# zhouxian/act3d-chained-diffuser

Hardware: AMD Instinct MI355X
Metric: train samples/sec (Act3D keypose fwd+bwd+AdamW step) (higher is better)
Workload: dtype fp16 / bf16 MFMA on two-part operands (x = hi + lo; fp32 accumulate) in attention; fp32-accurate linears (f32 MFMA; bf16x3 MFMA from 4096 rows); bf16 frozen backbone + FPN; 1 GPU; Act3D keypose training step, 18-PerAct-task shapes: 4 cameras 256x256, 3 ghost-point levels, 1000 ghost points (333/level), E=60, frozen synthetic CLIP-RN50-shaped backbone + trainable FPN included in the step; per_gpu_batch_keyframes=64, global_batch=64, parallelism=dp1, hipgraph=True, backbone_prefetch=True

## Files before the change

### act3d-chained-diffuser_amd/csrc/a3d_common.h

```cpp
#pragma once
#include <hip/hip_runtime.h>
#include <stdint.h>
#include <math.h>

#define A3D_OK 0
#define A3D_ERR_ARG (-22)
#define A3D_ERR_LAUNCH (-5)
#define A3D_ERR_NOMEM (-12)

namespace a3d {

void set_error(const char* fmt, ...);
int check_launch(const char* what);
int zero_words(void* p, size_t bytes, hipStream_t s, const char* what);

typedef __attribute__((ext_vector_type(4))) float f32x4;
typedef __attribute__((ext_vector_type(8))) short s16x8;
typedef __attribute__((ext_vector_type(8))) __bf16 bf16x8;
typedef __attribute__((ext_vector_type(4))) short s16x4;

constexpr int HD = 15;
constexpr float LOG2E_F = 1.4426950408889634f;
constexpr int HDP = 16;

__device__ __forceinline__ unsigned short f2bf(float x) {
  unsigned int u = __float_as_uint(x);
  unsigned int r = u + 0x7FFFu + ((u >> 16) & 1u);
  return (unsigned short)(r >> 16);
}
__device__ __forceinline__ unsigned int pk_bf16(float a, float b) {
  typedef __bf16 bf16x2_t __attribute__((ext_vector_type(2)));
  typedef float f32x2_t __attribute__((ext_vector_type(2)));
  return __builtin_bit_cast(unsigned int, __builtin_convertvector(f32x2_t{a, b}, bf16x2_t));
}
__device__ __forceinline__ float bf2f(unsigned short h) {
  return __uint_as_float(((unsigned int)h) << 16);
}
__device__ __forceinline__ void split_bf16(float x, unsigned short& hi, unsigned short& lo) {
  hi = f2bf(x);
  lo = f2bf(x - bf2f(hi));
}

__device__ __forceinline__ void split_bf16_3(float x, unsigned short& hi, unsigned short& lo, unsigned short& lo2) {
  hi = f2bf(x);
  const float r1 = x - bf2f(hi);
  lo = f2bf(r1);
  lo2 = f2bf(r1 - bf2f(lo));
}
constexpr int QKW = 48;
constexpr int VRW = 32;
__device__ __forceinline__ int tile_off(int row, int seg) { return row * 32 + ((seg ^ ((0 - (row >> 3)) & 3)) << 3); }
__device__ __forceinline__ int plane_off(int row, int seg) { return row * 32 + ((seg ^ ((0 - (row >> 2)) & 3)) << 3); }

__device__ __forceinline__ float colmax4(float v) {
  typedef unsigned int u32x2_t __attribute__((ext_vector_type(2)));
  u32x2_t r = __builtin_amdgcn_permlane16_swap(__float_as_uint(v), __float_as_uint(v), false, false);
  v = fmaxf(__uint_as_float(r[0]), __uint_as_float(r[1]));
  r = __builtin_amdgcn_permlane32_swap(__float_as_uint(v), __float_as_uint(v), false, false);
  return fmaxf(__uint_as_float(r[0]), __uint_as_float(r[1]));
}

__device__ __forceinline__ double colsum4(double v) {
  typedef unsigned int u32x2_t __attribute__((ext_vector_type(2)));
  unsigned int lo = (unsigned int)(__double_as_longlong(v) & 0xFFFFFFFFll), hi = (unsigned int)(__double_as_longlong(v) >> 32);
  u32x2_t a = __builtin_amdgcn_permlane16_swap(lo, lo, false, false);
  u32x2_t b = __builtin_amdgcn_permlane16_swap(hi, hi, false, false);
  v = __longlong_as_double(((long long)b[0] << 32) | a[0]) + __longlong_as_double(((long long)b[1] << 32) | a[1]);
  lo = (unsigned int)(__double_as_longlong(v) & 0xFFFFFFFFll);
  hi = (unsigned int)(__double_as_longlong(v) >> 32);
  a = __builtin_amdgcn_permlane32_swap(lo, lo, false, false);
  b = __builtin_amdgcn_permlane32_swap(hi, hi, false, false);
  return __longlong_as_double(((long long)b[0] << 32) | a[0]) + __longlong_as_double(((long long)b[1] << 32) | a[1]);
}

__device__ __forceinline__ f32x4 mfma_bf16_16x16x32(s16x8 a, s16x8 b, f32x4 c) {
  return __builtin_amdgcn_mfma_f32_16x16x32_bf16(__builtin_bit_cast(bf16x8, a),
                                                 __builtin_bit_cast(bf16x8, b), c, 0, 0, 0);
}
__device__ __forceinline__ f32x4 mfma_f32_16x16x4(float a, float b, f32x4 c) {
  return __builtin_amdgcn_mfma_f32_16x16x4f32(a, b, c, 0, 0, 0);
}

__device__ __forceinline__ float wave_sum(float v) {
#pragma unroll
  for (int o = 32; o > 0; o >>= 1) v += __shfl_xor(v, o, 64);
  return v;
}
__device__ __forceinline__ float wave_max(float v) {
#pragma unroll
  for (int o = 32; o > 0; o >>= 1) v = fmaxf(v, __shfl_xor(v, o, 64));
  return v;
}

__device__ __forceinline__ float rope_freq(int k, int E) {
  return expf((float)(2 * k) * (-9.210340371976184f / (float)(E / 3)));
}

__host__ __device__ __forceinline__ void sincos_poly(float x, float* sn, float* cs) {
  const float kf = rintf(x * 0.636619772367581343f);
  float r = fmaf(-kf, 1.57079637050628662109375f, x);
  r = fmaf(-kf, -4.37113900018624283e-8f, r);
  const float z = r * r;
  const float ps = fmaf(fmaf(fmaf(-1.9515295891e-4f, z, 8.3321608736e-3f), z, -1.6666654611e-1f) * z, r, r);
  const float pc = fmaf(fmaf(fmaf(2.443315711809948e-5f, z, -1.388731625493765e-3f), z, 4.166664568298827e-2f), z * z,
                        fmaf(-0.5f, z, 1.0f));
  const int q = (int)kf;
  const float s0 = (q & 1) ? pc : ps, c0 = (q & 1) ? ps : pc;
  *sn = (q & 2) ? -s0 : s0;
  *cs = ((q + 1) & 2) ? -c0 : c0;
}
__host__ __device__ __forceinline__ void fast_sincos(float x, float* sn, float* cs) {
#if defined(A3D_LIBM_SINCOS) && defined(__HIP_DEVICE_COMPILE__)
  sincosf(x, sn, cs);
#else
  if (fabsf(x) >= 200.0f) {
    const double t = (double)x;
    const double k = rint(t * 0.15915494309189535);
    x = (float)fma(-k, 2.4492935982947064e-16, fma(-k, 6.283185307179586, t));
  }
  sincos_poly(x, sn, cs);
#endif
}

__device__ __forceinline__ float add_rn(float a, float b) {
#pragma clang fp contract(off)
  return a + b;
}
__device__ __forceinline__ float sub_rn(float a, float b) {
#pragma clang fp contract(off)
  return a - b;
}
__device__ __forceinline__ float mul_rn(float a, float b) {
#pragma clang fp contract(off)
  return a * b;
}
__device__ __forceinline__ float sqrt_rn(float a) { return __builtin_sqrtf(a); }

__host__ __device__ __forceinline__ void philox4x32_10(uint32_t c0, uint32_t c1, uint32_t c2, uint32_t c3,
                                                       uint32_t k0, uint32_t k1, uint32_t out[4]) {
  for (int r = 0; r < 10; ++r) {
    const uint64_t p0 = (uint64_t)0xD2511F53u * c0;
    const uint64_t p1 = (uint64_t)0xCD9E8D57u * c2;
    const uint32_t n0 = (uint32_t)(p1 >> 32) ^ c1 ^ k0;
    const uint32_t n1 = (uint32_t)p1;
    const uint32_t n2 = (uint32_t)(p0 >> 32) ^ c3 ^ k1;
    const uint32_t n3 = (uint32_t)p0;
    c0 = n0; c1 = n1; c2 = n2; c3 = n3;
    k0 += 0x9E3779B9u; k1 += 0xBB67AE85u;
  }
  out[0] = c0; out[1] = c1; out[2] = c2; out[3] = c3;
}

struct DropKey { uint32_t k0, k1; };
__device__ __forceinline__ DropKey drop_key(const unsigned long long* state) {
  const unsigned long long seed = state[0], offs = state[1];
  const unsigned long long key = seed + offs * 0x9E3779B97F4A7C15ull;
  DropKey k;
  k.k0 = (uint32_t)key;
  k.k1 = (uint32_t)(key >> 32);
  return k;
}
__device__ __forceinline__ uint32_t drop_keep8(DropKey k, uint32_t c0, uint32_t c1, uint32_t c2, uint32_t site,
                                               uint32_t thr16) {
  uint32_t r[4];
  philox4x32_10(c0, c1, c2, site, k.k0, k.k1, r);
  uint32_t bits = 0;
#pragma unroll
  for (int w = 0; w < 4; ++w) {
    bits |= ((r[w] & 0xFFFFu) >= thr16 ? 1u : 0u) << (2 * w);
    bits |= ((r[w] >> 16) >= thr16 ? 1u : 0u) << (2 * w + 1);
  }
  return bits;
}

__device__ __forceinline__ bool xcd_decode(int per_group, int ngroups, int& group, int& within) {
  const int id = blockIdx.x;
  const int xcd = id & 7, slot = id >> 3;
  group = (slot / per_group) * 8 + xcd;
  within = slot % per_group;
  return group < ngroups;
}
static inline int xcd_grid(int ngroups, int per_group) { return ((ngroups + 7) / 8) * 8 * per_group; }

static inline int cdiv(int a, int b) { return (a + b - 1) / b; }

bool conv1x1_deep_serves(int K, int N);
int conv1x1_deep_slabs(size_t M, int K, int N);
int conv1x1_deep_launch(const void* x, const void* w, const float* in_scale, const float* in_shift, int in_relu, void* y, float* partial,
                        size_t M, int K, int N, hipStream_t s);

}
```

### act3d-chained-diffuser_amd/csrc/conv1x1.hip

```cpp
#include "a3d_common.h"
#include "../../include/act3d_hip.h"

namespace a3d {

constexpr int C1_BK = 32;

__device__ __forceinline__ int c1_woff(int row, int seg) { return row * 32 + ((seg ^ (((row >> 1) & 1) | (((row >> 4) & 1) << 1))) << 3); }

struct C1Epilogue { const float* bias; int nbias; const unsigned short* top; int H, W; };
template <int WN, int KS, bool EP = false>
__global__ __launch_bounds__(256, 2) void conv1x1_stream_kernel(const unsigned short* __restrict__ x, const unsigned short* __restrict__ w,
                                                             const float* __restrict__ in_scale, const float* __restrict__ in_shift,
                                                             int in_relu, unsigned short* __restrict__ y, float* __restrict__ partial,
                                                             long long M, int N, C1Epilogue ep) {
  constexpr int WM = 4 / WN, BM = 64 * WM, BN = 64 * WN, K = KS * 32;
  constexpr int XL = BM * 4 / 256;
  constexpr int D = 8 / XL;
  extern __shared__ __attribute__((aligned(16))) unsigned short smem_c1[];
  unsigned short* Ws = smem_c1;
  unsigned short* Xs = Ws + KS * BN * 32;
  float* scS = reinterpret_cast<float*>(Xs + 2 * BM * 32);
  __shared__ float redS[4][64], redQ[4][64];
  const int t = threadIdx.x, lane = t & 63, wave = t >> 6;
  const int li = lane & 15, g = lane >> 4;
  const int wm = wave / WN, wn = wave % WN;
  const int n0 = blockIdx.y * BN;
  const long long mtiles = (M + BM - 1) / BM;
  for (int i = t; i < KS * BN * 4; i += 256) {
    const int ks = i / (BN * 4), rem = i - ks * (BN * 4), row = rem >> 2, seg = rem & 3;
    *reinterpret_cast<uint4*>(&Ws[ks * BN * 32 + c1_woff(row, seg)]) =
        *reinterpret_cast<const uint4*>(w + (size_t)(n0 + row) * K + ks * C1_BK + seg * 8);
  }
  if (in_scale)
    for (int i = t; i < K; i += 256) { scS[i] = in_scale[i]; scS[K + i] = in_shift[i]; }
  float ssum[4][4], ssq[4][4];
#pragma unroll
  for (int a = 0; a < 4; ++a)
#pragma unroll
    for (int r = 0; r < 4; ++r) { ssum[a][r] = 0.f; ssq[a][r] = 0.f; }
  float epb[16];
  if (EP) {
#pragma unroll
    for (int j = 0; j < 16; ++j) {
      const int c = n0 + wn * 64 + g * 16 + j;
      epb[j] = (ep.bias && c < ep.nbias) ? ep.bias[c] : 0.f;
    }
  }
  const long long my_tiles = blockIdx.x < mtiles ? (mtiles - blockIdx.x + gridDim.x - 1) / gridDim.x : 0;
  const long long total = my_tiles * KS;
  auto load = [&](long long s, uint4 (&r)[XL]) {
    const long long m0 = (blockIdx.x + (s / KS) * gridDim.x) * BM;
    const int ks = (int)(s % KS);
#pragma unroll
    for (int i = 0; i < XL; ++i) {
      const int idx = t + i * 256, row = idx >> 2, seg = idx & 3;
      const long long m = m0 + row < M ? m0 + row : M - 1;
      r[i] = *reinterpret_cast<const uint4*>(x + (size_t)m * K + ks * C1_BK + seg * 8);
    }
  };
  const float relu_lo = in_relu ? 0.f : -INFINITY;
  auto stage = [&](int buf, int ks, const uint4 (&r)[XL]) {
#pragma unroll
    for (int i = 0; i < XL; ++i) {
      const int idx = t + i * 256, row = idx >> 2, seg = idx & 3;
      uint4 v = r[i];
      if (in_scale) {
        const int k0 = ks * C1_BK + seg * 8;
        unsigned int u[4] = {v.x, v.y, v.z, v.w};
#pragma unroll
        for (int j = 0; j < 4; ++j) {
          float a = __uint_as_float(u[j] << 16) * scS[k0 + 2 * j] + scS[K + k0 + 2 * j];
          float b = __uint_as_float(u[j] & 0xFFFF0000u) * scS[k0 + 2 * j + 1] + scS[K + k0 + 2 * j + 1];
          a = fmaxf(a, relu_lo);
          b = fmaxf(b, relu_lo);
          u[j] = pk_bf16(a, b);
        }
        v = make_uint4(u[0], u[1], u[2], u[3]);
      }
      *reinterpret_cast<uint4*>(&Xs[buf * BM * 32 + plane_off(row, seg)]) = v;
    }
  };
  if (total > 0) {
    uint4 xr[D][XL];
#pragma unroll
    for (int j = 0; j < D; ++j) load(j < total ? j : total - 1, xr[j]);
    f32x4 acc[4][4];
#pragma unroll
    for (int a = 0; a < 4; ++a)
#pragma unroll
      for (int b = 0; b < 4; ++b) acc[a][b] = f32x4{0.f, 0.f, 0.f, 0.f};
    __syncthreads();
    for (long long s0 = 0; s0 < total; s0 += D) {
#pragma unroll
      for (int j = 0; j < D; ++j) {
        const long long s = s0 + j;
        if (s >= total) break;
        const int ks = (int)(s % KS), buf = (int)(s & 1);
        stage(buf, ks, xr[j]);
        load(s + D < total ? s + D : total - 1, xr[j]);
        __syncthreads();
        s16x8 xa[4], wb[4];
#pragma unroll
        for (int tm = 0; tm < 4; ++tm)
          xa[tm] = *reinterpret_cast<const s16x8*>(&Xs[buf * BM * 32 + plane_off(wm * 64 + tm * 16 + li, g)]);
#pragma unroll
        for (int tn = 0; tn < 4; ++tn)
          wb[tn] = *reinterpret_cast<const s16x8*>(&Ws[ks * BN * 32 + c1_woff(wn * 64 + (li >> 2) * 16 + tn * 4 + (li & 3), g)]);
        uint4 tv[4][2];
        if (EP && ks == KS - 1 && ep.top) {
          const long long m0 = (blockIdx.x + (s / KS) * gridDim.x) * BM;
#pragma unroll
          for (int tm = 0; tm < 4; ++tm) {
            const long long m = m0 + wm * 64 + tm * 16 + li;
            const unsigned int mm = (unsigned int)(m < M ? m : M - 1);
            const unsigned int hq = mm / (unsigned int)ep.W, w_ = mm - hq * (unsigned int)ep.W;
            const unsigned int n_ = hq / (unsigned int)ep.H, h_ = hq - n_ * (unsigned int)ep.H;
            const size_t tr = ((size_t)n_ * (ep.H >> 1) + (h_ >> 1)) * (ep.W >> 1) + (w_ >> 1);
            const uint4* src = reinterpret_cast<const uint4*>(ep.top + tr * N + n0 + wn * 64 + g * 16);
            tv[tm][0] = src[0];
            tv[tm][1] = src[1];
          }
        }
#pragma unroll
        for (int tn = 0; tn < 4; ++tn)
#pragma unroll
          for (int tm = 0; tm < 4; ++tm) acc[tn][tm] = mfma_bf16_16x16x32(wb[tn], xa[tm], acc[tn][tm]);
        if (ks == KS - 1) {
          const long long m0 = (blockIdx.x + (s / KS) * gridDim.x) * BM;
#pragma unroll
          for (int tm = 0; tm < 4; ++tm) {
            const long long m = m0 + wm * 64 + tm * 16 + li;
            const bool ok = m < M;
            unsigned int pk[8];
#pragma unroll
            for (int tn = 0; tn < 4; ++tn) {
#pragma unroll
              for (int r2 = 0; r2 < 2; ++r2) {
                float a0 = acc[tn][tm][2 * r2], a1 = acc[tn][tm][2 * r2 + 1];
                if (EP) {
                  a0 += epb[4 * tn + 2 * r2];
                  a1 += epb[4 * tn + 2 * r2 + 1];
                  if (ep.top) {
                    const uint4 q = tv[tm][tn >> 1];
                    const unsigned int tw = (tn & 1) ? (r2 ? q.w : q.z) : (r2 ? q.y : q.x);
                    a0 += __uint_as_float(tw << 16);
                    a1 += __uint_as_float(tw & 0xFFFF0000u);
                  }
                }
                const unsigned int u = pk_bf16(a0, a1);
                if (!EP && ok) {
                  const float v0 = __uint_as_float(u << 16), v1 = __uint_as_float(u & 0xFFFF0000u);
                  ssum[tn][2 * r2] += v0;
                  ssq[tn][2 * r2] += v0 * v0;
                  ssum[tn][2 * r2 + 1] += v1;
                  ssq[tn][2 * r2 + 1] += v1 * v1;
                }
                pk[2 * tn + r2] = u;
              }
              acc[tn][tm] = f32x4{0.f, 0.f, 0.f, 0.f};
            }
            if (ok) {
              uint4* dst = reinterpret_cast<uint4*>(y + (size_t)m * N + n0 + wn * 64 + g * 16);
              dst[0] = make_uint4(pk[0], pk[1], pk[2], pk[3]);
              dst[1] = make_uint4(pk[4], pk[5], pk[6], pk[7]);
            }
          }
        }
      }
    }
  }
  if (EP || !partial) return;
#pragma unroll
  for (int tn = 0; tn < 4; ++tn)
#pragma unroll
    for (int r = 0; r < 4; ++r) {
      float sv = ssum[tn][r], q = ssq[tn][r];
#pragma unroll
      for (int o = 1; o < 16; o <<= 1) { sv += __shfl_xor(sv, o, 64); q += __shfl_xor(q, o, 64); }
      if (li == 0) { redS[wave][g * 16 + tn * 4 + r] = sv; redQ[wave][g * 16 + tn * 4 + r] = q; }
    }
  __syncthreads();
  for (int i = t; i < BN; i += 256) {
    const int wn_i = i >> 6, c = i & 63;
    float sv = 0.f, q = 0.f;
#pragma unroll
    for (int j = 0; j < WM; ++j) { sv += redS[j * WN + wn_i][c]; q += redQ[j * WN + wn_i][c]; }
    float* p = partial + (size_t)blockIdx.x * 2 * N;
    p[n0 + i] = sv;
    p[N + n0 + i] = q;
  }
}

}

using namespace a3d;

static int c1_wn(int N) { return N >= 256 ? 4 : (N >= 128 ? 2 : 1); }
static size_t c1_stream_lds(int K, int N) {
  const int wn = c1_wn(N), bn = 64 * wn, bm = 64 * (4 / wn);
  return (size_t)(K / 32) * bn * 64 + (size_t)2 * bm * 64 + (size_t)2 * K * sizeof(float);
}
static bool c1_streams(int K, int N) {
  return (K == 64 || K == 128 || K == 256) && (N % 64) == 0 && (N < 256 || (N % 256) == 0) && c1_stream_lds(K, N) <= 96 * 1024;
}
static int c1_slabs(size_t M, int K, int N) {
  const int wn = c1_wn(N);
  const int bm = 64 * (4 / wn);
  const size_t mtiles = (M + bm - 1) / bm;
  const int ntiles = N / (64 * wn);
  const size_t lds = c1_stream_lds(K, N) + 2048;
  const int per_cu = (int)std::max<size_t>(1, std::min<size_t>(2, (160 * 1024) / lds));
  return (int)std::min<size_t>(mtiles, (size_t)std::max(1, 256 * per_cu / ntiles));
}

static int c1_deep_mode = getenv("A3D_CONV1X1_DEEP") ? atoi(getenv("A3D_CONV1X1_DEEP")) : 1;
extern "C" int a3d_conv1x1_deep_mode(int mode) {
  const int prev = c1_deep_mode;
  if (mode >= 0) c1_deep_mode = mode > 0 ? 1 : 0;
  return prev;
}
static bool c1_deep(int K, int N) { return c1_deep_mode != 0 && !c1_streams(K, N) && conv1x1_deep_serves(K, N); }

extern "C" int a3d_conv1x1_streams(int K, int N) { return (K > 0 && N > 0 && (c1_streams(K, N) || c1_deep(K, N))) ? 1 : 0; }

extern "C" int a3d_conv1x1_nslab(size_t M, int K, int N) {
  if (M == 0 || N <= 0 || K <= 0) return 0;
  if (c1_streams(K, N)) return c1_slabs(M, K, N);
  return c1_deep(K, N) ? conv1x1_deep_slabs(M, K, N) : 0;
}

extern "C" int a3d_conv1x1_bn_fwd(const void* x, const void* w, const float* in_scale, const float* in_shift, int in_relu,
                                  void* y, float* partial, size_t M, int K, int N, void* stream) {
  if (!x || !w || !y || M == 0 || K <= 0 || N <= 0 || !(c1_streams(K, N) || c1_deep(K, N)) || (in_scale && !in_shift) ||
      ((((uintptr_t)x | (uintptr_t)w | (uintptr_t)y) & 15) != 0)) {
    set_error("a3d_conv1x1_bn_fwd: bad argument (M=%zu K=%d N=%d; served shapes: K in {64, 128, 256}, N in {64, 128, 256 j}, weight block "
              "+ buffers within 96 KB of LDS (the resident-weight kernel), or K = 64 j in 128 .. 2048 and N = 128 j up to 2048 (the deep-layer "
              "GEMM) -- a3d_conv1x1_streams; 16-byte aligned operands)", M, K, N);
    return A3D_ERR_ARG;
  }
  hipStream_t s = (hipStream_t)stream;
  if (!c1_streams(K, N)) return conv1x1_deep_launch(x, w, in_scale, in_shift, in_relu, y, partial, M, K, N, s);
  const unsigned short* xs = (const unsigned short*)x;
  const unsigned short* ws = (const unsigned short*)w;
  unsigned short* ys = (unsigned short*)y;
  const int slabs = c1_slabs(M, K, N);
  const size_t lds = c1_stream_lds(K, N);
  const dim3 grid(slabs, N >= 256 ? N / 256 : 1);
#define A3D_C1S(WNV, KSV)                                                                                                         \
  do {                                                                                                                           \
    static bool once = false;                                                                                                    \
    if (!once) { (void)hipFuncSetAttribute((const void*)conv1x1_stream_kernel<WNV, KSV>, hipFuncAttributeMaxDynamicSharedMemorySize, 96 * 1024); once = true; } \
    hipLaunchKernelGGL((conv1x1_stream_kernel<WNV, KSV>), grid, dim3(256), lds, s, xs, ws, in_scale, in_shift, in_relu, ys, partial, (long long)M, N, C1Epilogue{nullptr, 0, nullptr, 0, 0}); \
  } while (0)
  const int wn = c1_wn(N), ks = K / 32;
  if (wn == 4 && ks == 2) A3D_C1S(4, 2);
  else if (wn == 4 && ks == 4) A3D_C1S(4, 4);
  else if (wn == 2 && ks == 2) A3D_C1S(2, 2);
  else if (wn == 2 && ks == 4) A3D_C1S(2, 4);
  else if (wn == 2 && ks == 8) A3D_C1S(2, 8);
  else if (wn == 1 && ks == 2) A3D_C1S(1, 2);
  else if (wn == 1 && ks == 4) A3D_C1S(1, 4);
  else if (wn == 1 && ks == 8) A3D_C1S(1, 8);
  else { set_error("a3d_conv1x1_bn_fwd: no streaming instance for K=%d N=%d", K, N); return A3D_ERR_ARG; }
#undef A3D_C1S
  return check_launch("a3d_conv1x1_bn_fwd");
}

extern "C" int a3d_conv1x1_topdown_serves(int K, int N) { return (c1_streams(K, N) && N <= 128) ? 1 : 0; }

extern "C" int a3d_conv1x1_topdown_fwd(const void* x, const void* w, const float* bias, int nbias, const void* top, void* y,
                                       size_t images, int H, int W, int K, int N, void* stream) {
  const size_t M = images * (size_t)H * (size_t)W;
  if (!x || !w || !y || images == 0 || H <= 0 || W <= 0 || K <= 0 || N <= 0 || !a3d_conv1x1_topdown_serves(K, N) || M > 0xFFFFFFFFull ||
      (top && ((H & 1) || (W & 1))) || (bias && (nbias <= 0 || nbias > N)) ||
      ((((uintptr_t)x | (uintptr_t)w | (uintptr_t)y | (uintptr_t)top) & 15) != 0)) {
    set_error("a3d_conv1x1_topdown_fwd: bad argument (images=%zu H=%d W=%d K=%d N=%d nbias=%d; served: K in {64, 128, 256}, N in {64, 128}, "
              "H and W even with a top map, at most 2^32 rows, 0 < nbias <= N with a bias, 16-byte aligned operands)", images, H, W, K, N, nbias);
    return A3D_ERR_ARG;
  }
  hipStream_t s = (hipStream_t)stream;
  const int slabs = c1_slabs(M, K, N);
  const size_t lds = c1_stream_lds(K, N);
  const dim3 grid(slabs, 1);
  const C1Epilogue ep{bias, bias ? nbias : 0, (const unsigned short*)top, H, W};
#define A3D_C1E(WNV, KSV)                                                                                                         \
  do {                                                                                                                           \
    static bool once = false;                                                                                                    \
    if (!once) { (void)hipFuncSetAttribute((const void*)conv1x1_stream_kernel<WNV, KSV, true>, hipFuncAttributeMaxDynamicSharedMemorySize, 96 * 1024); once = true; } \
    hipLaunchKernelGGL((conv1x1_stream_kernel<WNV, KSV, true>), grid, dim3(256), lds, s, (const unsigned short*)x, (const unsigned short*)w, \
                       (const float*)nullptr, (const float*)nullptr, 0, (unsigned short*)y, (float*)nullptr, (long long)M, N, ep);  \
  } while (0)
  const int wn = c1_wn(N), ks = K / 32;
  if (wn == 2 && ks == 2) A3D_C1E(2, 2);
  else if (wn == 2 && ks == 4) A3D_C1E(2, 4);
  else if (wn == 2 && ks == 8) A3D_C1E(2, 8);
  else if (wn == 1 && ks == 2) A3D_C1E(1, 2);
  else if (wn == 1 && ks == 4) A3D_C1E(1, 4);
  else if (wn == 1 && ks == 8) A3D_C1E(1, 8);
  else { set_error("a3d_conv1x1_topdown_fwd: no streaming instance for K=%d N=%d", K, N); return A3D_ERR_ARG; }
#undef A3D_C1E
  return check_launch("a3d_conv1x1_topdown_fwd");
}
```

### act3d-chained-diffuser_amd/csrc/conv1x1_deep.hip

```cpp
#include "a3d_common.h"
#include "../../include/act3d_hip.h"

namespace a3d {

constexpr int CD_BM = 128, CD_BN = 128, CD_BK = 64;

__device__ __forceinline__ int cd_xoff(int row, int seg) { return row * 64 + ((seg ^ ((row >> 1) & 7)) << 3); }
__device__ __forceinline__ int cd_woff(int row, int seg) { return row * 64 + ((seg ^ ((((row >> 4) & 3) << 1) | ((row >> 1) & 1))) << 3); }

__device__ __forceinline__ unsigned int cd_norm2(unsigned int u, const float* scS, int K, int k, float relu_lo) {
  float a = __uint_as_float(u << 16) * scS[k] + scS[K + k];
  float b = __uint_as_float(u & 0xFFFF0000u) * scS[k + 1] + scS[K + k + 1];
  return pk_bf16(fmaxf(a, relu_lo), fmaxf(b, relu_lo));
}

__device__ __forceinline__ void cd_compute(const unsigned short* Xb, const unsigned short* Wb, const int (&xo)[2][4], const int (&wo)[2][4],
                                           f32x4 (&acc)[4][4]) {
#pragma unroll
  for (int h = 0; h < 2; ++h) {
    s16x8 xa[4], wb[4];
#pragma unroll
    for (int i = 0; i < 4; ++i) {
      xa[i] = *reinterpret_cast<const s16x8*>(&Xb[xo[h][i]]);
      wb[i] = *reinterpret_cast<const s16x8*>(&Wb[wo[h][i]]);
    }
#pragma unroll
    for (int tn = 0; tn < 4; ++tn)
#pragma unroll
      for (int tm = 0; tm < 4; ++tm) acc[tn][tm] = mfma_bf16_16x16x32(wb[tn], xa[tm], acc[tn][tm]);
  }
}

__device__ __forceinline__ void cd_epilogue(f32x4 (&acc)[4][4], float (&ssum)[4][4], float (&ssq)[4][4], unsigned short* __restrict__ y,
                                            long long m0, long long M, int N, int n0, int wm, int wn, int li, int g) {
#pragma unroll
  for (int tm = 0; tm < 4; ++tm) {
    const long long m = m0 + wm * 64 + tm * 16 + li;
    const bool ok = m < M;
    unsigned int pk[8];
#pragma unroll
    for (int tn = 0; tn < 4; ++tn) {
#pragma unroll
      for (int r2 = 0; r2 < 2; ++r2) {
        const unsigned int u = pk_bf16(acc[tn][tm][2 * r2], acc[tn][tm][2 * r2 + 1]);
        const float v0 = ok ? __uint_as_float(u << 16) : 0.f, v1 = ok ? __uint_as_float(u & 0xFFFF0000u) : 0.f;
        ssum[tn][2 * r2] += v0;
        ssq[tn][2 * r2] += v0 * v0;
        ssum[tn][2 * r2 + 1] += v1;
        ssq[tn][2 * r2 + 1] += v1 * v1;
        pk[2 * tn + r2] = u;
      }
      acc[tn][tm] = f32x4{0.f, 0.f, 0.f, 0.f};
    }
    if (ok) {
      uint4* dst = reinterpret_cast<uint4*>(y + (size_t)m * N + n0 + wn * 64 + g * 16);
      dst[0] = make_uint4(pk[0], pk[1], pk[2], pk[3]);
      dst[1] = make_uint4(pk[4], pk[5], pk[6], pk[7]);
    }
  }
}

template <bool XFORM>
__global__ __launch_bounds__(256, 2) void conv1x1_deep_kernel(const unsigned short* __restrict__ x, const unsigned short* __restrict__ w,
                                                            const float* __restrict__ in_scale, const float* __restrict__ in_shift,
                                                            int in_relu, unsigned short* __restrict__ y, float* __restrict__ partial,
                                                            long long M, int N, int K) {
  extern __shared__ __attribute__((aligned(16))) unsigned short smem_cd[];
  unsigned short* Xs = smem_cd;
  unsigned short* Ws = Xs + 2 * CD_BM * CD_BK;
  float* scS = reinterpret_cast<float*>(Ws + 2 * CD_BN * CD_BK);
  const int t = threadIdx.x, lane = t & 63, wave = t >> 6;
  const int li = lane & 15, g = lane >> 4;
  const int wm = wave >> 1, wn = wave & 1;
  const int n0 = blockIdx.y * CD_BN;
  const int KS = K / CD_BK;
  const long long mtiles = (M + CD_BM - 1) / CD_BM;
  if (XFORM)
    for (int i = t; i < K; i += 256) { scS[i] = in_scale[i]; scS[K + i] = in_shift[i]; }
  float ssum[4][4], ssq[4][4];
#pragma unroll
  for (int a = 0; a < 4; ++a)
#pragma unroll
    for (int r = 0; r < 4; ++r) { ssum[a][r] = 0.f; ssq[a][r] = 0.f; }
  const long long my_tiles = blockIdx.x < mtiles ? (mtiles - blockIdx.x + gridDim.x - 1) / gridDim.x : 0;
  const long long total = my_tiles * KS;
  const int srow = t >> 3, sseg = t & 7;
  long long l_m0 = (long long)blockIdx.x * CD_BM;
  int l_ks = 0;
  const float relu_lo = in_relu ? 0.f : -INFINITY;
#define CD_LOAD1(P, i)                                                                                                \
  {                                                                                                                   \
    const long long m_ = l_m0 + srow + 32 * i < M ? l_m0 + srow + 32 * i : M - 1;    \
    P##x##i = *reinterpret_cast<const uint4*>(x + (size_t)m_ * K + l_ks * CD_BK + sseg * 8);                          \
    P##w##i = *reinterpret_cast<const uint4*>(w + (size_t)(n0 + srow + 32 * i) * K + l_ks * CD_BK + sseg * 8);        \
  }
#define CD_LOAD(P)                                                                                                    \
  do {                                                                                                                \
    CD_LOAD1(P, 0) CD_LOAD1(P, 1) CD_LOAD1(P, 2) CD_LOAD1(P, 3)                                                       \
    if (l_left > 1) { --l_left; if (++l_ks == KS) { l_ks = 0; l_m0 += (long long)gridDim.x * CD_BM; } }               \
  } while (0)
#define CD_STAGE1(P, i)                                                                                               \
  {                                                                                                                   \
    uint4 v = P##x##i;                                                                                                \
    if (XFORM) {                                                                                                      \
      const int k0 = ks * CD_BK + sseg * 8;                                                                           \
      unsigned int u0 = v.x, u1 = v.y, u2 = v.z, u3 = v.w;                                                            \
      u0 = cd_norm2(u0, scS, K, k0 + 0, relu_lo); u1 = cd_norm2(u1, scS, K, k0 + 2, relu_lo);                         \
      u2 = cd_norm2(u2, scS, K, k0 + 4, relu_lo); u3 = cd_norm2(u3, scS, K, k0 + 6, relu_lo);                         \
      v = make_uint4(u0, u1, u2, u3);                                                                                 \
    }                                                                                                                 \
    *reinterpret_cast<uint4*>(&Xs[buf * CD_BM * CD_BK + cd_xoff(srow + 32 * i, sseg)]) = v;                           \
    *reinterpret_cast<uint4*>(&Ws[buf * CD_BN * CD_BK + cd_woff(srow + 32 * i, sseg)]) = P##w##i;                     \
  }
#define CD_STAGE(P) CD_STAGE1(P, 0) CD_STAGE1(P, 1) CD_STAGE1(P, 2) CD_STAGE1(P, 3)
  int xo[2][4], wo[2][4];
#pragma unroll
  for (int h = 0; h < 2; ++h)
#pragma unroll
    for (int i = 0; i < 4; ++i) {
      xo[h][i] = cd_xoff(wm * 64 + i * 16 + li, h * 4 + g);
      wo[h][i] = cd_woff(wn * 64 + (li >> 2) * 16 + i * 4 + (li & 3), h * 4 + g);
    }
  if (total > 0) {
    uint4 ax0, ax1, ax2, ax3, aw0, aw1, aw2, aw3, bx0, bx1, bx2, bx3, bw0, bw1, bw2, bw3;
    long long l_left = total;
    CD_LOAD(a);
    CD_LOAD(b);
    long long c_m0 = (long long)blockIdx.x * CD_BM;
    int ks = 0;
    f32x4 acc[4][4];
#pragma unroll
    for (int a = 0; a < 4; ++a)
#pragma unroll
      for (int b = 0; b < 4; ++b) acc[a][b] = f32x4{0.f, 0.f, 0.f, 0.f};
    __syncthreads();
#define CD_STEP(P, BUF)                                                                                               \
    {                                                                                                                 \
      constexpr int buf = BUF;                                                                                        \
      CD_STAGE(P)                                                                                                     \
      CD_LOAD(P);                                                                                \
      __syncthreads();                                             \
      cd_compute(Xs + buf * CD_BM * CD_BK, Ws + buf * CD_BN * CD_BK, xo, wo, acc);                                    \
      if (ks == KS - 1) cd_epilogue(acc, ssum, ssq, y, c_m0, M, N, n0, wm, wn, li, g);                                \
      if (++ks == KS) { ks = 0; c_m0 += (long long)gridDim.x * CD_BM; }                                               \
    }
    for (long long s = 0; s < total; s += 2) {
      CD_STEP(a, 0)
      if (s + 1 < total) CD_STEP(b, 1)
    }
#undef CD_STEP
  }
  if (!partial) return;
  __syncthreads();
  float* redS = reinterpret_cast<float*>(Xs);
  float* redQ = redS + 4 * 64;
#pragma unroll
  for (int tn = 0; tn < 4; ++tn)
#pragma unroll
    for (int r = 0; r < 4; ++r) {
      float sv = ssum[tn][r], q = ssq[tn][r];
#pragma unroll
      for (int o = 1; o < 16; o <<= 1) { sv += __shfl_xor(sv, o, 64); q += __shfl_xor(q, o, 64); }
      if (li == 0) { redS[wave * 64 + g * 16 + tn * 4 + r] = sv; redQ[wave * 64 + g * 16 + tn * 4 + r] = q; }
    }
  __syncthreads();
  if (t < CD_BN) {
    const int wn_i = t >> 6, c = t & 63;
    const float sv = redS[(0 * 2 + wn_i) * 64 + c] + redS[(1 * 2 + wn_i) * 64 + c];
    const float q = redQ[(0 * 2 + wn_i) * 64 + c] + redQ[(1 * 2 + wn_i) * 64 + c];
    float* p = partial + (size_t)blockIdx.x * 2 * N;
    p[n0 + t] = sv;
    p[N + n0 + t] = q;
  }
}

#undef CD_LOAD
#undef CD_LOAD1
#undef CD_STAGE1
#undef CD_STAGE

}

using namespace a3d;

bool a3d::conv1x1_deep_serves(int K, int N) { return K >= 128 && K <= 2048 && (K % CD_BK) == 0 && N >= 128 && N <= 2048 && (N % CD_BN) == 0; }
static size_t cd_lds(int K, bool xform) { return (size_t)2 * (CD_BM + CD_BN) * CD_BK * 2 + (xform ? (size_t)2 * K * sizeof(float) : 0); }

int a3d::conv1x1_deep_slabs(size_t M, int K, int N) {
  (void)K;
  const size_t mtiles = (M + CD_BM - 1) / CD_BM;
  const int nblocks = N / CD_BN;
  return (int)std::min<size_t>(mtiles, (size_t)std::max(1, 512 / nblocks));
}

int a3d::conv1x1_deep_launch(const void* x, const void* w, const float* in_scale, const float* in_shift, int in_relu, void* y, float* partial,
                             size_t M, int K, int N, hipStream_t s) {
  if (in_scale && K > 1024) { set_error("a3d_conv1x1_bn_fwd: the folded BatchNorm-apply of the deep-layer kernel serves K <= 1024 (K=%d)", K); return A3D_ERR_ARG; }
  static bool once = false;
  if (!once) {
    (void)hipFuncSetAttribute((const void*)conv1x1_deep_kernel<false>, hipFuncAttributeMaxDynamicSharedMemorySize, 80 * 1024);
    (void)hipFuncSetAttribute((const void*)conv1x1_deep_kernel<true>, hipFuncAttributeMaxDynamicSharedMemorySize, 80 * 1024);
    once = true;
  }
  const dim3 grid(conv1x1_deep_slabs(M, K, N), N / CD_BN);
  if (in_scale)
    hipLaunchKernelGGL(conv1x1_deep_kernel<true>, grid, dim3(256), cd_lds(K, true), s, (const unsigned short*)x, (const unsigned short*)w,
                       in_scale, in_shift, in_relu, (unsigned short*)y, partial, (long long)M, N, K);
  else
    hipLaunchKernelGGL(conv1x1_deep_kernel<false>, grid, dim3(256), cd_lds(K, false), s, (const unsigned short*)x, (const unsigned short*)w,
                       in_scale, in_shift, in_relu, (unsigned short*)y, partial, (long long)M, N, K);
  return check_launch("a3d_conv1x1_bn_fwd(deep)");
}
```

### act3d-chained-diffuser_amd/csrc/vision.hip

```cpp
#include "a3d_common.h"
#include "../../include/act3d_hip.h"

namespace a3d {

__global__ __launch_bounds__(256) void bn_stats_kernel(const uint4* __restrict__ x, float* __restrict__ partial,
                                                       size_t rows, int C, int CG, int nslab) {
  __shared__ float red[256 * 16];
  const int tpr = CG >> 3;
  const int nsub = 256 / tpr;
  const int cp = threadIdx.x % tpr, rsub = threadIdx.x / tpr;
  const int C8 = C >> 3;
  const int cvec = blockIdx.y * tpr + cp;
  const size_t chunk_rows = (size_t)nsub * 8;
  const size_t nchunk = (rows + chunk_rows - 1) / chunk_rows;
  float s[8], q[8];
#pragma unroll
  for (int j = 0; j < 8; ++j) { s[j] = 0.f; q[j] = 0.f; }
  auto accum = [&](const uint4& v) {
    const unsigned int w[4] = {v.x, v.y, v.z, v.w};
#pragma unroll
    for (int j = 0; j < 4; ++j) {
      const float a = __uint_as_float(w[j] << 16), b = __uint_as_float(w[j] & 0xFFFF0000u);
      s[2 * j] += a; q[2 * j] += a * a;
      s[2 * j + 1] += b; q[2 * j + 1] += b * b;
    }
  };
  auto load = [&](size_t ch, uint4 (&v)[8]) {
    const size_t r = ch * chunk_rows + rsub;
#pragma unroll
    for (int u = 0; u < 8; ++u) {
      const size_t ru = r + (size_t)u * nsub;
      const uint4 t = x[(ru < rows ? ru : rows - 1) * C8 + cvec];
      v[u] = ru < rows ? t : make_uint4(0, 0, 0, 0);
    }
  };
  uint4 cur[8], nxt[8];
  size_t ch = blockIdx.x;
  if (ch < nchunk) load(ch, cur);
  while (ch < nchunk) {
    const size_t nch = ch + nslab;
    if (nch < nchunk) load(nch, nxt);
#pragma unroll
    for (int u = 0; u < 8; ++u) accum(cur[u]);
#pragma unroll
    for (int u = 0; u < 8; ++u) cur[u] = nxt[u];
    ch = nch;
  }
#pragma unroll
  for (int j = 0; j < 8; ++j) { red[threadIdx.x * 16 + j] = s[j]; red[threadIdx.x * 16 + 8 + j] = q[j]; }
  __syncthreads();
  for (int o = threadIdx.x; o < 2 * CG; o += 256) {
    const int which = o / CG, c = o - which * CG;
    const int tp = c >> 3, j = c & 7;
    float acc = 0.f;
    for (int u = 0; u < nsub; ++u) acc += red[(u * tpr + tp) * 16 + which * 8 + j];
    partial[(size_t)blockIdx.x * 2 * C + (size_t)which * C + blockIdx.y * CG + c] = acc;
  }
}

__global__ __launch_bounds__(1024) void bn_finalize_kernel(const float* __restrict__ partial, int nslab, double rows, int C,
                                                           float eps, float momentum, const float* __restrict__ gamma,
                                                           const float* __restrict__ beta, float* __restrict__ running_mean,
                                                           float* __restrict__ running_var, float* __restrict__ scale,
                                                           float* __restrict__ shift, int train) {
  __shared__ double rs[16][16], rq[16][16];
  const int cx = threadIdx.x & 15, sg = threadIdx.x >> 4, wave = threadIdx.x >> 6;
  const int c = blockIdx.x * 16 + cx;
  double s = 0.0, q = 0.0;
  if (train && c < C) {
    int i = sg;
    double s1 = 0.0, q1 = 0.0;
    for (; i + 64 < nslab; i += 128) {
      s += (double)partial[(size_t)i * 2 * C + c];
      q += (double)partial[(size_t)i * 2 * C + C + c];
      s1 += (double)partial[(size_t)(i + 64) * 2 * C + c];
      q1 += (double)partial[(size_t)(i + 64) * 2 * C + C + c];
    }
    if (i < nslab) {
      s += (double)partial[(size_t)i * 2 * C + c];
      q += (double)partial[(size_t)i * 2 * C + C + c];
    }
    s += s1;
    q += q1;
  }
  s = colsum4(s);
  q = colsum4(q);
  if ((threadIdx.x & 63) < 16) { rs[wave][cx] = s; rq[wave][cx] = q; }
  __syncthreads();
  if (sg != 0 || c >= C) return;
  double mean, var;
  if (train) {
    s = 0.0; q = 0.0;
#pragma unroll
    for (int u = 0; u < 16; ++u) { s += rs[u][cx]; q += rq[u][cx]; }
    mean = s / rows;
    var = q / rows - mean * mean;
    if (var < 0.0) var = 0.0;
    if (running_mean) {
      const double unb = rows > 1.0 ? var * rows / (rows - 1.0) : var;
      running_mean[c] = (float)((1.0 - momentum) * running_mean[c] + momentum * mean);
      running_var[c] = (float)((1.0 - momentum) * running_var[c] + momentum * unb);
    }
  } else {
    mean = running_mean[c];
    var = running_var[c];
  }
  const float inv = (float)(1.0 / sqrt(var + (double)eps));
  const float sc = (gamma ? gamma[c] : 1.f) * inv;
  scale[c] = sc;
  shift[c] = (beta ? beta[c] : 0.f) - (float)mean * sc;
}

__device__ __forceinline__ unsigned int pack2(float a, float b) {
  typedef __attribute__((ext_vector_type(2))) float f2;
  typedef __attribute__((ext_vector_type(2))) __bf16 b2;
  return __builtin_bit_cast(unsigned int, __builtin_convertvector((f2){a, b}, b2));
}

__global__ __launch_bounds__(256) void rgb_normalize_kernel(const float* __restrict__ x, const float* __restrict__ mean,
                                                            const float* __restrict__ stdv, unsigned short* __restrict__ y,
                                                            size_t N, size_t HW) {
  const size_t quads = N * HW / 4;
  const float m0 = mean[0], m1 = mean[1], m2 = mean[2], s0 = stdv[0], s1 = stdv[1], s2 = stdv[2];
  for (size_t i = (size_t)blockIdx.x * blockDim.x + threadIdx.x; i < quads; i += (size_t)gridDim.x * blockDim.x) {
    const size_t n = (i * 4) / HW, p = (i * 4) - n * HW;
    const float* base = x + n * 3 * HW + p;
    const float4 r = *reinterpret_cast<const float4*>(base);
    const float4 g = *reinterpret_cast<const float4*>(base + HW);
    const float4 b = *reinterpret_cast<const float4*>(base + 2 * HW);
    const float rr[4] = {r.x, r.y, r.z, r.w}, gg[4] = {g.x, g.y, g.z, g.w}, bb[4] = {b.x, b.y, b.z, b.w};
    unsigned short o[12];
#pragma unroll
    for (int j = 0; j < 4; ++j) {
      o[3 * j + 0] = f2bf((rr[j] - m0) / s0);
      o[3 * j + 1] = f2bf((gg[j] - m1) / s1);
      o[3 * j + 2] = f2bf((bb[j] - m2) / s2);
    }
    uint2* dst = reinterpret_cast<uint2*>(y + (n * HW + p) * 3);
    dst[0] = make_uint2(o[0] | ((unsigned)o[1] << 16), o[2] | ((unsigned)o[3] << 16));
    dst[1] = make_uint2(o[4] | ((unsigned)o[5] << 16), o[6] | ((unsigned)o[7] << 16));
    dst[2] = make_uint2(o[8] | ((unsigned)o[9] << 16), o[10] | ((unsigned)o[11] << 16));
  }
}

template <bool RBN>
__global__ __launch_bounds__(256) void bn_apply_kernel(const uint4* __restrict__ x, const uint4* __restrict__ res,
                                                       const float* __restrict__ scale, const float* __restrict__ shift,
                                                       const float* __restrict__ rscale, const float* __restrict__ rshift,
                                                       uint4* __restrict__ y, size_t nvec, int C8, int relu) {
  const bool pow2 = (C8 & (C8 - 1)) == 0;
  for (size_t i = (size_t)blockIdx.x * blockDim.x + threadIdx.x; i < nvec; i += (size_t)gridDim.x * blockDim.x) {
    const int c = (pow2 ? (int)((unsigned int)i & (unsigned int)(C8 - 1)) : (int)(i % C8)) * 8;
    const uint4 v = x[i];
    uint4 rv = make_uint4(0, 0, 0, 0);
    if (res) rv = res[i];
    const unsigned int vw[4] = {v.x, v.y, v.z, v.w};
    const unsigned int rw[4] = {rv.x, rv.y, rv.z, rv.w};
    unsigned int ow[4];
#pragma unroll
    for (int j = 0; j < 4; ++j) {
      float a = __uint_as_float(vw[j] << 16) * scale[c + 2 * j] + shift[c + 2 * j];
      float b = __uint_as_float(vw[j] & 0xFFFF0000u) * scale[c + 2 * j + 1] + shift[c + 2 * j + 1];
      if (res) {
        float ra = __uint_as_float(rw[j] << 16), rb = __uint_as_float(rw[j] & 0xFFFF0000u);
        if (RBN) {
          ra = ra * rscale[c + 2 * j] + rshift[c + 2 * j];
          rb = rb * rscale[c + 2 * j + 1] + rshift[c + 2 * j + 1];
        }
        a += ra;
        b += rb;
      }
      if (relu) { a = fmaxf(a, 0.f); b = fmaxf(b, 0.f); }
      ow[j] = pack2(a, b);
    }
    y[i] = make_uint4(ow[0], ow[1], ow[2], ow[3]);
  }
}

__global__ __launch_bounds__(256) void bn_apply_pool2_kernel(const uint4* __restrict__ x, const uint4* __restrict__ res,
                                                             const float* __restrict__ scale, const float* __restrict__ shift,
                                                             uint4* __restrict__ y_full, uint4* __restrict__ y_pool, int N,
                                                             int H, int W, int C8, int relu) {
  const int Ho = H >> 1, Wo = W >> 1;
  const size_t nout = (size_t)N * Ho * Wo * C8;
  const bool p2 = (C8 & (C8 - 1)) == 0 && (Wo & (Wo - 1)) == 0;
  const int c8_sh = 31 - __clz(C8), wo_sh = 31 - __clz(Wo);
  for (unsigned int i = blockIdx.x * blockDim.x + threadIdx.x; i < (unsigned int)nout; i += gridDim.x * blockDim.x) {
    int c8, wo;
    unsigned int pix;
    if (p2) {
      c8 = (int)(i & (unsigned int)(C8 - 1));
      pix = i >> c8_sh;
      wo = (int)(pix & (unsigned int)(Wo - 1));
      pix >>= wo_sh;
    } else {
      c8 = (int)(i % (unsigned int)C8);
      pix = i / (unsigned int)C8;
      wo = (int)(pix % (unsigned int)Wo);
      pix /= (unsigned int)Wo;
    }
    const int ho = (int)(pix % (unsigned int)Ho);
    const int n = (int)(pix / (unsigned int)Ho);
    const int c = c8 * 8;
    float sc[8], sh[8];
#pragma unroll
    for (int j = 0; j < 8; ++j) { sc[j] = scale ? scale[c + j] : 1.f; sh[j] = scale ? shift[c + j] : 0.f; }
    float acc[8];
#pragma unroll
    for (int j = 0; j < 8; ++j) acc[j] = 0.f;
#pragma unroll
    for (int dy = 0; dy < 2; ++dy) {
#pragma unroll
      for (int dx = 0; dx < 2; ++dx) {
        const size_t src = (((size_t)n * H + 2 * ho + dy) * W + 2 * wo + dx) * C8 + c8;
        const uint4 v = x[src];
        uint4 rv = make_uint4(0, 0, 0, 0);
        if (res) rv = res[src];
        const unsigned int vw[4] = {v.x, v.y, v.z, v.w};
        const unsigned int rw[4] = {rv.x, rv.y, rv.z, rv.w};
        unsigned int ow[4];
#pragma unroll
        for (int j = 0; j < 4; ++j) {
          float a = __uint_as_float(vw[j] << 16) * sc[2 * j] + sh[2 * j];
          float b = __uint_as_float(vw[j] & 0xFFFF0000u) * sc[2 * j + 1] + sh[2 * j + 1];
          if (res) {
            a += __uint_as_float(rw[j] << 16);
            b += __uint_as_float(rw[j] & 0xFFFF0000u);
          }
          if (relu) { a = fmaxf(a, 0.f); b = fmaxf(b, 0.f); }
          ow[j] = pack2(a, b);
          acc[2 * j] += __uint_as_float(ow[j] << 16);
          acc[2 * j + 1] += __uint_as_float(ow[j] & 0xFFFF0000u);
        }
        if (y_full) y_full[src] = make_uint4(ow[0], ow[1], ow[2], ow[3]);
      }
    }
    y_pool[i] = make_uint4(pack2(acc[0] * 0.25f, acc[1] * 0.25f), pack2(acc[2] * 0.25f, acc[3] * 0.25f),
                           pack2(acc[4] * 0.25f, acc[5] * 0.25f), pack2(acc[6] * 0.25f, acc[7] * 0.25f));
  }
}

__device__ __forceinline__ void bf16x4_to_f32(uint2 a, float (&o)[4]) {
  o[0] = __uint_as_float(a.x << 16); o[1] = __uint_as_float(a.x & 0xFFFF0000u);
  o[2] = __uint_as_float(a.y << 16); o[3] = __uint_as_float(a.y & 0xFFFF0000u);
}
__global__ __launch_bounds__(256) void upsample2_add_fwd_kernel(const uint2* __restrict__ lat, const uint2* __restrict__ top,
                                                                const float* __restrict__ bias, int nbias,
                                                                uint2* __restrict__ y, int N, int H, int W, int C4) {
  const size_t total = (size_t)N * H * W * C4;
  const int Ht = H >> 1, Wt = W >> 1;
  const bool p2 = (C4 & (C4 - 1)) == 0 && (W & (W - 1)) == 0 && (H & (H - 1)) == 0;
  const int c_sh = 31 - __clz(C4), w_sh = 31 - __clz(W), h_sh = 31 - __clz(H);
  for (size_t i = (size_t)blockIdx.x * blockDim.x + threadIdx.x; i < total; i += (size_t)gridDim.x * blockDim.x) {
    int c, w, h, n;
    if (p2) {
      c = (int)((unsigned int)i & (unsigned int)(C4 - 1));
      const size_t pix = i >> c_sh;
      w = (int)((unsigned int)pix & (unsigned int)(W - 1));
      h = (int)((unsigned int)(pix >> w_sh) & (unsigned int)(H - 1));
      n = (int)(pix >> (w_sh + h_sh));
    } else {
      c = (int)(i % C4);
      size_t pix = i / C4;
      w = (int)(pix % W);
      pix /= W;
      h = (int)(pix % H);
      n = (int)(pix / H);
    }
    float a[4], t[4] = {0.f, 0.f, 0.f, 0.f};
    bf16x4_to_f32(lat[i], a);
    if (top) bf16x4_to_f32(top[(((size_t)n * Ht + (h >> 1)) * Wt + (w >> 1)) * C4 + c], t);
    if (bias) {
#pragma unroll
      for (int j = 0; j < 4; ++j) a[j] += (c * 4 + j < nbias) ? bias[c * 4 + j] : 0.f;
    }
    y[i] = make_uint2(pack2(a[0] + t[0], a[1] + t[1]), pack2(a[2] + t[2], a[3] + t[3]));
  }
}
__global__ __launch_bounds__(256) void upsample2_add_bwd_kernel(const uint2* __restrict__ dy, uint2* __restrict__ dtop,
                                                                float* __restrict__ bias_partial, int N, int H, int W, int C4) {
  __shared__ float red[256 * 4];
  const int Ht = H >> 1, Wt = W >> 1;
  const size_t total = (size_t)N * Ht * Wt * C4;
  float cs[4] = {0.f, 0.f, 0.f, 0.f};
  const bool p2 = (C4 & (C4 - 1)) == 0 && (Wt & (Wt - 1)) == 0 && (Ht & (Ht - 1)) == 0;
  const int c_sh = 31 - __clz(C4), w_sh = 31 - __clz(Wt), h_sh = 31 - __clz(Ht);
  for (size_t i = (size_t)blockIdx.x * blockDim.x + threadIdx.x; i < total; i += (size_t)gridDim.x * blockDim.x) {
    int c, wt, ht, n;
    if (p2) {
      c = (int)((unsigned int)i & (unsigned int)(C4 - 1));
      const size_t pix = i >> c_sh;
      wt = (int)((unsigned int)pix & (unsigned int)(Wt - 1));
      ht = (int)((unsigned int)(pix >> w_sh) & (unsigned int)(Ht - 1));
      n = (int)(pix >> (w_sh + h_sh));
    } else {
      c = (int)(i % C4);
      size_t pix = i / C4;
      wt = (int)(pix % Wt);
      pix /= Wt;
      ht = (int)(pix % Ht);
      n = (int)(pix / Ht);
    }
    float acc[4] = {0.f, 0.f, 0.f, 0.f};
#pragma unroll
    for (int dyy = 0; dyy < 2; ++dyy)
#pragma unroll
      for (int dx = 0; dx < 2; ++dx) {
        float v[4];
        bf16x4_to_f32(dy[(((size_t)n * H + 2 * ht + dyy) * W + 2 * wt + dx) * C4 + c], v);
#pragma unroll
        for (int j = 0; j < 4; ++j) acc[j] += v[j];
      }
    if (dtop) dtop[i] = make_uint2(pack2(acc[0], acc[1]), pack2(acc[2], acc[3]));
#pragma unroll
    for (int j = 0; j < 4; ++j) cs[j] += acc[j];
  }
  if (bias_partial) {
#pragma unroll
    for (int j = 0; j < 4; ++j) red[threadIdx.x * 4 + j] = cs[j];
    __syncthreads();
    for (int o = threadIdx.x; o < 4 * C4; o += 256) {
      const int c = o >> 2, j = o & 3;
      float a = 0.f;
      for (int u = c; u < 256; u += C4) a += red[u * 4 + j];
      bias_partial[(size_t)blockIdx.x * 4 * C4 + o] = a;
    }
  }
}

__global__ __launch_bounds__(1024) void colsum_reduce_kernel(const float* __restrict__ partial, int nrow, int C, float* __restrict__ out,
                                                            int nout) {
  __shared__ float red[16][64];
  const int cl = threadIdx.x & 63, rg = threadIdx.x >> 6;
  const int c = blockIdx.x * 64 + cl;
  float a[8];
#pragma unroll
  for (int u = 0; u < 8; ++u) a[u] = 0.f;
  if (c < C) {
    int i = rg;
    for (; i + 7 * 16 < nrow; i += 8 * 16) {
#pragma unroll
      for (int u = 0; u < 8; ++u) a[u] += partial[(size_t)(i + u * 16) * C + c];
    }
    for (; i < nrow; i += 16) a[0] += partial[(size_t)i * C + c];
  }
  red[rg][cl] = ((a[0] + a[1]) + (a[2] + a[3])) + ((a[4] + a[5]) + (a[6] + a[7]));
  __syncthreads();
  if (rg == 0 && c < nout) {
    float s = 0.f;
#pragma unroll
    for (int u = 0; u < 16; ++u) s += red[u][cl];
    out[c] += s;
  }
}

__global__ __launch_bounds__(256) void colsum_rows_kernel(const float* __restrict__ src, int B, int S, int k, int ld, int C,
                                                          float* __restrict__ partial) {
  __shared__ float red[256];
  const int cl = threadIdx.x & 63, rg = threadIdx.x >> 6;
  const int c = blockIdx.y * 64 + cl;
  const size_t total = (size_t)B * k;
  float a = 0.f;
  if (c < C) {
    for (size_t r = (size_t)blockIdx.x * 4 + rg; r < total; r += (size_t)gridDim.x * 4) {
      const size_t b = r / k, s = r - b * k;
      a += src[(b * S + s) * ld + c];
    }
  }
  red[threadIdx.x] = a;
  __syncthreads();
  if (threadIdx.x < 64 && c < C)
    partial[(size_t)blockIdx.x * C + c] = (red[cl] + red[64 + cl]) + (red[128 + cl] + red[192 + cl]);
}

}

using namespace a3d;

static int bn_channel_group(int C) { return C < 256 ? C : 256; }

extern "C" int a3d_bn_nslab(size_t rows, int C) {
  if (C < 8) return 1;
  const int CG = bn_channel_group(C);
  const size_t chunk_rows = (size_t)(256 / (CG / 8)) * 8;
  size_t n = 2048 / (size_t)(C / CG);
  const size_t nchunk = (rows + chunk_rows - 1) / chunk_rows;
  if (n > nchunk) n = nchunk;
  if (n > 1024) n = 1024;
  if (n < 1) n = 1;
  return (int)n;
}

extern "C" int a3d_bn_stats(const void* x, float* partial, size_t rows, int C, int nslab, void* stream) {
  const int CG = bn_channel_group(C);
  if (!x || !partial || rows == 0 || C < 8 || (C % 8) != 0 || C > 2048 || (256 % (CG / 8)) != 0 || (C % CG) != 0 || nslab < 1 ||
      (((uintptr_t)x) & 15)) {
    set_error("a3d_bn_stats: bad argument (C=%d must be 8 * a divisor of 256 or a multiple of 256, nslab=%d)", C, nslab);
    return A3D_ERR_ARG;
  }
  hipLaunchKernelGGL(bn_stats_kernel, dim3(nslab, C / CG), dim3(256), 0, (hipStream_t)stream, (const uint4*)x, partial, rows, C, CG,
                     nslab);
  return check_launch("a3d_bn_stats");
}

extern "C" int a3d_bn_finalize(const float* partial, int nslab, size_t rows, int C, float eps, float momentum,
                               const float* gamma, const float* beta, float* running_mean, float* running_var,
                               float* scale, float* shift, int train, void* stream) {
  if (C <= 0 || !scale || !shift || (train && !partial) || (!train && (!running_mean || !running_var))) {
    set_error("a3d_bn_finalize: bad argument");
    return A3D_ERR_ARG;
  }
  hipLaunchKernelGGL(bn_finalize_kernel, dim3(cdiv(C, 16)), dim3(1024), 0, (hipStream_t)stream, partial, nslab, (double)rows,
                     C, eps, momentum, gamma, beta, running_mean, running_var, scale, shift, train);
  return check_launch("a3d_bn_finalize");
}

static int g_bn_grid_cap = getenv("A3D_BN_GRID") ? std::max(64, atoi(getenv("A3D_BN_GRID"))) : 16384;
static int bn_grid_cap() { return g_bn_grid_cap; }
extern "C" int a3d_bn_grid_cap(int cap) {
  const int prev = g_bn_grid_cap;
  if (cap > 0) g_bn_grid_cap = std::max(64, cap);
  return prev;
}

extern "C" int a3d_bn_apply(const void* x, const void* residual, const float* res_scale, const float* res_shift, const float* scale,
                            const float* shift, void* y, size_t rows, int C, int relu, void* stream) {
  if (!x || !scale || !shift || !y || rows == 0 || C <= 0 || (C % 8) != 0 || (res_scale && (!res_shift || !residual)) ||
      ((((uintptr_t)x) | ((uintptr_t)y) | ((uintptr_t)residual)) & 15)) {
    set_error("a3d_bn_apply: bad argument (C=%d must be a multiple of 8, pointers 16-byte aligned, res_scale needs res_shift and a residual)", C);
    return A3D_ERR_ARG;
  }
  const size_t nvec = rows * (size_t)(C / 8);
  const int grid = (int)std::min<size_t>((nvec + 255) / 256, (size_t)bn_grid_cap());
  if (res_scale)
    hipLaunchKernelGGL(bn_apply_kernel<true>, dim3(grid), dim3(256), 0, (hipStream_t)stream, (const uint4*)x, (const uint4*)residual,
                       scale, shift, res_scale, res_shift, (uint4*)y, nvec, C / 8, relu);
  else
    hipLaunchKernelGGL(bn_apply_kernel<false>, dim3(grid), dim3(256), 0, (hipStream_t)stream, (const uint4*)x, (const uint4*)residual,
                       scale, shift, (const float*)nullptr, (const float*)nullptr, (uint4*)y, nvec, C / 8, relu);
  return check_launch("a3d_bn_apply");
}

extern "C" int a3d_bn_apply_pool2(const void* x, const void* residual, const float* scale, const float* shift, void* y_full,
                                  void* y_pool, int N, int H, int W, int C, int relu, void* stream) {
  if (!x || !y_pool || (scale && !shift) || N <= 0 || H <= 0 || W <= 0 || (H & 1) || (W & 1) || C <= 0 || (C % 8) != 0 ||
      ((((uintptr_t)x) | ((uintptr_t)y_pool) | ((uintptr_t)y_full) | ((uintptr_t)residual)) & 15)) {
    set_error("a3d_bn_apply_pool2: bad argument (H=%d W=%d must be even, C=%d a multiple of 8, pointers 16-byte aligned)", H,
              W, C);
    return A3D_ERR_ARG;
  }
  const size_t nout = (size_t)N * (H / 2) * (W / 2) * (C / 8);
  if (nout >= ((size_t)1 << 31)) { set_error("a3d_bn_apply_pool2: map too large (%zu 16-byte outputs)", nout); return A3D_ERR_ARG; }
  const int grid = (int)std::min<size_t>((nout + 255) / 256, (size_t)bn_grid_cap());
  hipLaunchKernelGGL(bn_apply_pool2_kernel, dim3(grid), dim3(256), 0, (hipStream_t)stream, (const uint4*)x,
                     (const uint4*)residual, scale, shift, (uint4*)y_full, (uint4*)y_pool, N, H, W, C / 8, relu);
  return check_launch("a3d_bn_apply_pool2");
}

static int check_up2(const char* fn, const void* a, const void* b, const void* c , int N, int H, int W, int C) {
  if (!a || !b || N <= 0 || H <= 0 || W <= 0 || (H & 1) || (W & 1) || C <= 0 || (C % 4) != 0 ||
      ((((uintptr_t)a) | ((uintptr_t)b) | ((uintptr_t)c)) & 7)) {
    set_error("%s: bad argument (H=%d W=%d must be even, C=%d a multiple of 4, pointers 8-byte aligned)", fn, H, W, C);
    return A3D_ERR_ARG;
  }
  return A3D_OK;
}

extern "C" int a3d_upsample2_add_fwd(const void* lat, const void* top, const float* bias, int nbias, void* y, int N, int H, int W,
                                     int C, void* stream) {
  int rc = check_up2("a3d_upsample2_add_fwd", lat, y, top, N, H, W, C);
  if (rc) return rc;
  if (bias && (nbias <= 0 || nbias > C)) { set_error("a3d_upsample2_add_fwd: %d bias entries for %d channels", nbias, C); return A3D_ERR_ARG; }
  const size_t total = (size_t)N * H * W * (C / 4);
  const int grid = (int)std::min<size_t>((total + 255) / 256, 16384);
  hipLaunchKernelGGL(upsample2_add_fwd_kernel, dim3(grid), dim3(256), 0, (hipStream_t)stream, (const uint2*)lat,
                     (const uint2*)top, bias, nbias, (uint2*)y, N, H, W, C / 4);
  return check_launch("a3d_upsample2_add_fwd");
}

static int up2_bwd_grid(int N, int H, int W, int C) {
  const size_t total = (size_t)N * (H / 2) * (W / 2) * (C / 4);
  return (int)std::min<size_t>((total + 255) / 256, 2048);
}
extern "C" size_t a3d_upsample2_add_bwd_ws_floats(int N, int H, int W, int C) {
  if (N <= 0 || H <= 0 || W <= 0 || C <= 0) return 0;
  return (size_t)up2_bwd_grid(N, H, W, C) * C;
}

extern "C" int a3d_upsample2_add_bwd(const void* dy, void* dtop, float* dbias, int nbias, float* ws, int N, int H, int W, int C,
                                     void* stream) {
  int rc = check_up2("a3d_upsample2_add_bwd", dy, dy, dtop, N, H, W, C);
  if (rc) return rc;
  if (!dtop && !dbias) { set_error("a3d_upsample2_add_bwd: nothing to compute (dtop and dbias are both null)"); return A3D_ERR_ARG; }
  if (dbias && (!ws || (256 % (C / 4)) != 0 || nbias <= 0 || nbias > C)) {
    set_error("a3d_upsample2_add_bwd: the bias gradient needs a workspace, C / 4 = %d dividing 256 and 0 < nbias <= C", C / 4);
    return A3D_ERR_ARG;
  }
  const int grid = up2_bwd_grid(N, H, W, C);
  hipLaunchKernelGGL(upsample2_add_bwd_kernel, dim3(grid), dim3(256), 0, (hipStream_t)stream, (const uint2*)dy, (uint2*)dtop,
                     dbias ? ws : nullptr, N, H, W, C / 4);
  rc = check_launch("a3d_upsample2_add_bwd");
  if (rc || !dbias) return rc;
  hipLaunchKernelGGL(colsum_reduce_kernel, dim3(cdiv(C, 64)), dim3(1024), 0, (hipStream_t)stream, ws, grid, C, dbias, nbias);
  return check_launch("a3d_upsample2_add_bwd(bias)");
}

extern "C" size_t a3d_colsum_rows_ws_floats(int B, int k, int C) {
  if (B <= 0 || k <= 0 || C <= 0) return 0;
  const size_t nblk = std::min<size_t>(((size_t)B * k + 63) / 64, 1024);
  return nblk * C;
}

extern "C" int a3d_colsum_rows(const float* src, int B, int S, int k, int ld, int C, float* out, int nout, float* ws, void* stream) {
  if (!src || !out || !ws || B <= 0 || S <= 0 || k <= 0 || k > S || C <= 0 || ld < C || nout <= 0 || nout > C) {
    set_error("a3d_colsum_rows: bad argument (B=%d S=%d k=%d ld=%d C=%d nout=%d; k <= S, nout <= C <= ld)", B, S, k, ld, C, nout);
    return A3D_ERR_ARG;
  }
  const int nblk = (int)(a3d_colsum_rows_ws_floats(B, k, C) / C);
  hipLaunchKernelGGL(colsum_rows_kernel, dim3(nblk, cdiv(C, 64)), dim3(256), 0, (hipStream_t)stream, src, B, S, k, ld, C, ws);
  int rc = check_launch("a3d_colsum_rows");
  if (rc) return rc;
  hipLaunchKernelGGL(colsum_reduce_kernel, dim3(cdiv(C, 64)), dim3(1024), 0, (hipStream_t)stream, ws, nblk, C, out, nout);
  return check_launch("a3d_colsum_rows(reduce)");
}

extern "C" int a3d_rgb_normalize_nhwc_bf16(const float* x, const float* mean, const float* stdv, void* y, size_t N, int H, int W,
                                           void* stream) {
  const size_t HW = (size_t)H * W;
  if (!x || !mean || !stdv || !y || N == 0 || H <= 0 || W <= 0 || (HW % 4) != 0 || ((((uintptr_t)x) & 15) != 0) ||
      ((((uintptr_t)y) & 7) != 0)) {
    set_error("a3d_rgb_normalize_nhwc_bf16: bad argument (H * W must be a multiple of 4, x 16-byte aligned)");
    return A3D_ERR_ARG;
  }
  const size_t quads = N * HW / 4;
  hipLaunchKernelGGL(rgb_normalize_kernel, dim3((int)std::min<size_t>((quads + 255) / 256, 16384)), dim3(256), 0,
                     (hipStream_t)stream, x, mean, stdv, (unsigned short*)y, N, HW);
  return check_launch("a3d_rgb_normalize_nhwc_bf16");
}
```

### act3d-chained-diffuser_amd/engine.py

```python
import os

import torch
import torch.distributed as dist

from . import lib as L

NO_DECAY = ["bias", "LayerNorm.weight", "LayerNorm.bias"]


def _is_no_decay(name):
    return any(nd in name for nd in NO_DECAY)


def discover_active_parameters(model, run_fwd_bwd):
    for p in model.parameters():
        p.grad = None
    run_fwd_bwd()
    active = [n for n, p in model.named_parameters() if p.requires_grad and p.grad is not None]
    for p in model.parameters():
        p.grad = None
    return active


class FlatParams:

    def __init__(self, model, active_names=None, late_prefixes=("feature_pyramid",)):
        named = [(n, p) for n, p in model.named_parameters() if p.requires_grad]
        if active_names is not None:
            keep = set(active_names)
            named = [(n, p) for n, p in named if n in keep]
        is_late = lambda n: any(pre in n for pre in late_prefixes)
        segs = [[], [], [], []]
        for n, p in named:
            nd, late = _is_no_decay(n), is_late(n)
            segs[0 if (nd and not late) else 1 if (nd and late) else 2 if late else 3].append((n, p))
        self.order = [x for s in segs for x in s]
        every = [n for n, _ in model.named_parameters()]
        self.torch_groups = [[n for n in every if _is_no_decay(n)], [n for n in every if not _is_no_decay(n)]]
        self.torch_index = {n: i for i, n in enumerate(self.torch_groups[0] + self.torch_groups[1])}
        sizes = [sum(p.numel() for _, p in s) for s in segs]
        self.n = sum(sizes)
        self.n_nodecay = sizes[0] + sizes[1]
        self.late_range = (sizes[0], sizes[0] + sizes[1] + sizes[2])
        dev = self.order[0][1].device
        self.flat = torch.empty(self.n, device=dev, dtype=torch.float32)
        self.grad = torch.zeros(self.n, device=dev, dtype=torch.float32)
        self.slices = {}
        off = 0
        with torch.no_grad():
            for n, p in self.order:
                k = p.numel()
                self.flat[off:off + k].copy_(p.detach().reshape(-1))
                p.data = self.flat[off:off + k].view(p.shape)
                p.grad = self.grad[off:off + k].view(p.shape)
                self.slices[n] = (off, off + k)
                off += k

    def rebind_grads(self):
        for n, p in self.order:
            a, b = self.slices[n]
            p.grad = self.grad[a:b].view(p.shape)

    def zero_grad(self):
        self.grad.zero_()
        for n, p in self.order:
            if p.grad is None or p.grad.data_ptr() != self.grad.data_ptr() + self.slices[n][0] * 4:
                self.rebind_grads()
                break


class FlatAdamW:

    def __init__(self, flat, lr=1e-4, betas=(0.9, 0.999), eps=1e-8, weight_decay=5e-4):
        self.flat, self.betas, self.eps, self.weight_decay = flat, betas, eps, weight_decay
        self.exp_avg = torch.zeros_like(flat.flat)
        self.exp_avg_sq = torch.zeros_like(flat.flat)
        self.step_count = torch.zeros(1, device=flat.flat.device, dtype=torch.float32)
        self.seg_off = torch.tensor([flat.slices[n][0] for n, _ in flat.order] + [flat.n], dtype=torch.int64, device=flat.flat.device)
        self.seg_state = torch.zeros((len(flat.order), 4), device=flat.flat.device, dtype=torch.float32)
        self.param_groups = [{"lr": lr, "weight_decay": 0.0}, {"lr": lr, "weight_decay": weight_decay}]

    @property
    def lr(self):
        return self.param_groups[0]["lr"]

    @lr.setter
    def lr(self, value):
        for g in self.param_groups:
            g["lr"] = float(value)

    def zero_grad(self, set_to_none=False):
        self.flat.zero_grad()

    def step(self, grad_scale=1.0):
        f = self.flat
        L.call("a3d_adamw_step", f.flat.data_ptr(), f.grad.data_ptr(), self.exp_avg.data_ptr(),
               self.exp_avg_sq.data_ptr(), self.step_count.data_ptr(), self.seg_off.data_ptr(), self.seg_state.data_ptr(),
               len(f.order), f.n, f.n_nodecay, float(self.lr),
               self.betas[0], self.betas[1], self.eps, 0.0, float(self.weight_decay), float(grad_scale), L.stream())

    @property
    def param_steps(self):
        return self.seg_state[:, 0]

    def reset_state(self):
        self.exp_avg.zero_(); self.exp_avg_sq.zero_(); self.step_count.zero_(); self.seg_state.zero_()

    def state_dict(self):
        f = self.flat
        state = {}
        steps = self.param_steps.detach().cpu()
        for (n, p), st in zip(f.order, steps):
            if float(st) <= 0:
                continue
            a, b = f.slices[n]
            state[f.torch_index[n]] = {"step": st.clone().reshape(()), "exp_avg": self.exp_avg[a:b].detach().clone().view(p.shape),
                                       "exp_avg_sq": self.exp_avg_sq[a:b].detach().clone().view(p.shape)}
        groups, off = [], 0
        for names, wd in zip(f.torch_groups, (0.0, self.weight_decay)):
            groups.append({"lr": self.lr, "betas": tuple(self.betas), "eps": self.eps, "weight_decay": wd,
                           "amsgrad": False, "maximize": False, "foreach": None, "capturable": False,
                           "differentiable": False, "fused": None, "decoupled_weight_decay": True,
                           "params": list(range(off, off + len(names)))})
            off += len(names)
        return {"state": state, "param_groups": groups}

    def load_state_dict(self, sd):
        f = self.flat
        if not isinstance(sd, dict) or "state" not in sd or "param_groups" not in sd:
            raise ValueError("optimizer state: expected torch.optim.AdamW's {'state', 'param_groups'} layout")
        sizes = [len(g["params"]) for g in sd["param_groups"]]
        if sizes != [len(g) for g in f.torch_groups]:
            raise ValueError("optimizer state: parameter groups of sizes %s do not match this model's %s "
                             "(reference grouping, engine.py:89-102)" % (sizes, [len(g) for g in f.torch_groups]))
        by_index = {i: n for n, i in f.torch_index.items()}
        seg_of = {n: i for i, (n, _) in enumerate(f.order)}
        steps = torch.zeros(len(f.order), dtype=torch.float32)
        loaded = []
        for idx, st in sd["state"].items():
            n = by_index.get(int(idx))
            if n is None:
                raise ValueError("optimizer state: index %r is not a parameter of this model" % (idx,))
            if n not in f.slices:
                continue
            a, b = f.slices[n]
            if st["exp_avg"].numel() != b - a:
                raise ValueError("optimizer state of %s has %d elements, the parameter %d" % (n, st["exp_avg"].numel(), b - a))
            loaded.append((a, b, st))
            steps[seg_of[n]] = float(st["step"])
        self.reset_state()
        for a, b, st in loaded:
            self.exp_avg[a:b].copy_(st["exp_avg"].reshape(-1))
            self.exp_avg_sq[a:b].copy_(st["exp_avg_sq"].reshape(-1))
        self.seg_state[:, 0].copy_(steps)
        self.step_count.fill_(float(steps.max()) if len(loaded) else 0.0)
        self.lr = sd["param_groups"][0].get("lr", self.lr)


def get_optimizer(model, lr=1e-4, active_names=None):
    flat = FlatParams(model, active_names)
    return flat, FlatAdamW(flat, lr=lr)


DP_ONESHOT = os.environ.get("A3D_DP_ONESHOT", "0") == "1"


class FlatDataParallel:

    def __init__(self, flat, process_group=None, overlap=True, model=None):
        self.flat = flat
        self.model = model
        self.pg = process_group
        self.world = dist.get_world_size(process_group) if dist.is_initialized() else 1
        self.overlap = overlap and flat.flat.is_cuda and not DP_ONESHOT
        self._pending = []
        self._side = torch.cuda.Stream() if self.overlap else None
        self._early_done = False
        self._begun = False
        self._armed = True

    def broadcast_parameters(self, src=0):
        if self.world == 1:
            return
        dist.broadcast(self.flat.flat, src=src, group=self.pg)
        if self.model is not None:
            flat_ptrs = {p.data_ptr() for _, p in self.flat.order}
            for name, t in self.model.state_dict().items():
                if t.data_ptr() in flat_ptrs:
                    continue
                if t.is_contiguous():
                    dist.broadcast(t, src=src, group=self.pg)
                else:
                    c = t.contiguous()
                    dist.broadcast(c, src=src, group=self.pg)
                    t.copy_(c)

    def _segments(self):
        a, b = self.flat.late_range
        return [(0, a), (b, self.flat.n)], (a, b)

    def arm(self, on=True):
        self._armed = bool(on)

    def hot_path_done(self):
        if self.world == 1 or not self.overlap or not self._armed or self._early_done:
            return
        hot, _ = self._segments()
        ev = torch.cuda.Event()
        ev.record(torch.cuda.current_stream())
        self._side.wait_event(ev)
        with torch.cuda.stream(self._side):
            for a, b in hot:
                if b > a:
                    self._pending.append(dist.all_reduce(self.flat.grad[a:b], op=dist.ReduceOp.SUM, group=self.pg,
                                                         async_op=True))
        self._early_done = True

    def begin_sync(self):
        if self.world == 1 or self._begun:
            return
        hot, late = self._segments()
        todo = [late] if self._early_done else [(0, self.flat.n)]
        if self._side is not None:
            ev = torch.cuda.Event()
            ev.record(torch.cuda.current_stream())
            self._side.wait_event(ev)
            with torch.cuda.stream(self._side):
                for a, b in todo:
                    if b > a:
                        self._pending.append(dist.all_reduce(self.flat.grad[a:b], op=dist.ReduceOp.SUM, group=self.pg, async_op=True))
        else:
            for a, b in todo:
                if b > a:
                    dist.all_reduce(self.flat.grad[a:b], op=dist.ReduceOp.SUM, group=self.pg)
        self._begun = True

    def finish_sync(self):
        if self.world == 1:
            return 1.0
        for w in self._pending:
            w.wait()
        if self._side is not None:
            torch.cuda.current_stream().wait_stream(self._side)
        self._pending, self._early_done, self._begun = [], False, False
        return 1.0 / self.world

    def sync_gradients(self):
        if self.world == 1:
            return 1.0
        self.begin_sync()
        return self.finish_sync()


def _split_backward(tokens, run_hot, on_hot_done):
    from .ops import TokenMap
    uniq, leaves = {}, []
    for t in tokens:
        tm = TokenMap.of(t)
        if id(tm.tokens) not in uniq:
            uniq[id(tm.tokens)] = (tm.tokens, tm.leaf())
        leaf = uniq[id(tm.tokens)][1]
        leaves.append(leaf if isinstance(t, TokenMap) else leaf.tokens)
    loss = run_hot(leaves)
    loss.backward()
    if on_hot_done is not None:
        on_hot_done()
    pairs = [(t, l.tokens.grad) for t, l in uniq.values() if t.requires_grad and l.tokens.grad is not None]
    if pairs:
        torch.autograd.backward([t for t, _ in pairs], [g for _, g in pairs])
    return loss.detach()


def fwd_bwd_keypose(model, criterion, sample, use_gt_sampling=True, on_hot_done=None):
    maps = sample.get("backbone_maps")
    tokens = model.compute_visual_tokens(sample["rgbs"]) if maps is None else model.compute_visual_tokens(sample["rgbs"], maps=maps)

    def hot(leaves):
        out = model(sample["rgbs"], sample["pcds"], sample["instr"], sample["curr_gripper"],
                    gt_action=sample["action"] if use_gt_sampling else None, visual_features=leaves)
        return sum(criterion.compute_loss(out, sample).values())

    return _split_backward(tokens, hot, on_hot_done)


def fwd_bwd_trajectory(model, criterion, sample, on_hot_done=None):
    maps = sample.get("backbone_maps")
    head = model.prediction_head
    tokens = head.encode_images(sample["rgbs"], None) if maps is None else head.encode_images(sample["rgbs"], None, maps=maps)
    multi = isinstance(tokens, (list, tuple))

    kw = {k: sample[k] for k in ("noise", "timesteps") if k in sample}

    def hot(leaves):
        return criterion.compute_loss(model(sample["trajectory"], sample["trajectory_mask"], sample["rgbs"], sample["pcds"],
                                            sample["instr"], sample["curr_gripper"], sample["action"],
                                            visual_tokens=list(leaves) if multi else leaves[0], **kw))

    return _split_backward(list(tokens) if multi else [tokens], hot, on_hot_done)


def _finish_step(optimizer, ddp, step_id, accumulate_grad_batches):
    if step_id % accumulate_grad_batches == accumulate_grad_batches - 1:
        scale = ddp.sync_gradients() if ddp is not None else 1.0
        optimizer.step(grad_scale=scale) if isinstance(optimizer, FlatAdamW) else optimizer.step()


def train_one_step(model, criterion, optimizer, step_id, sample, ddp=None, accumulate_grad_batches=1,
                   use_ground_truth_position_for_sampling_train=True):
    if step_id % accumulate_grad_batches == 0:
        optimizer.zero_grad()
    last = step_id % accumulate_grad_batches == accumulate_grad_batches - 1
    if ddp is not None:
        ddp.arm(last)
    loss = fwd_bwd_keypose(model, criterion, sample, use_ground_truth_position_for_sampling_train,
                           None if ddp is None else ddp.hot_path_done)
    _finish_step(optimizer, ddp, step_id, accumulate_grad_batches)
    return loss


def train_one_step_trajectory(model, criterion, optimizer, step_id, sample, ddp=None, accumulate_grad_batches=1):
    if step_id % accumulate_grad_batches == 0:
        optimizer.zero_grad()
    last = step_id % accumulate_grad_batches == accumulate_grad_batches - 1
    if ddp is not None:
        ddp.arm(last)
    loss = fwd_bwd_trajectory(model, criterion, sample, None if ddp is None else ddp.hot_path_done)
    _finish_step(optimizer, ddp, step_id, accumulate_grad_batches)
    return loss


class JointStep:

    def __init__(self, kp_model, kp_criterion, kp_optimizer, tr_model, tr_criterion, tr_optimizer, kp_ddp=None, tr_ddp=None,
                 use_ground_truth_position_for_sampling_train=True):
        self.kp = (kp_model, kp_criterion, kp_optimizer, kp_ddp)
        self.tr = (tr_model, tr_criterion, tr_optimizer, tr_ddp)
        self.use_gt = use_ground_truth_position_for_sampling_train

    def __call__(self, kp_sample, tr_sample):
        km, kc, ko, kd = self.kp
        tm, tc, to, td = self.tr
        ko.zero_grad()
        to.zero_grad()
        if kd is not None:
            kd.arm(True)
        loss_k = fwd_bwd_keypose(km, kc, kp_sample, self.use_gt, None if kd is None else kd.hot_path_done)
        if kd is not None:
            kd.begin_sync()
        if td is not None:
            td.arm(True)
        loss_t = fwd_bwd_trajectory(tm, tc, tr_sample, None if td is None else td.hot_path_done)
        if td is not None:
            td.begin_sync()
        ko.step(grad_scale=kd.finish_sync() if kd is not None else 1.0)
        to.step(grad_scale=td.finish_sync() if td is not None else 1.0)
        return loss_k, loss_t


def save_checkpoint(path, model, optimizer, step_id, best_loss=None):
    weight = {"module." + k: v.detach().clone() for k, v in model.state_dict().items()}
    torch.save({"weight": weight, "optimizer": optimizer.state_dict(), "iter": step_id + 1, "best_loss": best_loss}, path)


def load_checkpoint(path, model, optimizer=None, strict=True):
    d = torch.load(path, map_location="cpu", weights_only=False)
    weight = {(k[7:] if k.startswith("module.") else k): v for k, v in d["weight"].items()}
    res = model.load_state_dict(weight, strict=False)
    if strict and (res.missing_keys or res.unexpected_keys):
        raise RuntimeError("checkpoint %s does not match the model: missing %s, unexpected %s" %
                           (path, res.missing_keys[:5], res.unexpected_keys[:5]))
    if optimizer is not None:
        if "optimizer" not in d:
            raise RuntimeError("checkpoint %s holds no optimizer state" % path)
        optimizer.load_state_dict(d["optimizer"])
    return d.get("iter", 0), d.get("best_loss", None)


PREFETCH_HIPRIO = os.environ.get("A3D_PREFETCH_HIPRIO", "0")
PREFETCH_BN_GRID = int(os.environ.get("A3D_PREFETCH_BN_GRID", "256"))
PREFETCH_CHECK = os.environ.get("A3D_PREFETCH_CHECK", "0") == "1"


class GraphedStep:

    def __init__(self, step_fwd_bwd, optimizer, static_inputs, ddp=None, warmup=3, prefetch=None):
        self.static_inputs = static_inputs
        self.optimizer = optimizer
        self.ddp = ddp
        self.world = ddp.world if ddp is not None else 1
        self.prefetch = prefetch
        split = self.world > 1
        self.parity = 0
        self._primed = False
        sets = 1
        gkw = {}
        if prefetch is not None:
            sets = 2
            self.next_rgbs = static_inputs["rgbs"].clone()
            with torch.no_grad():
                m0 = prefetch(static_inputs["rgbs"])
            self.maps = [m0, {k: torch.empty_like(v) for k, v in m0.items()}]
            self._pf_stream = torch.cuda.Stream(priority=-1) if PREFETCH_HIPRIO == "side" else torch.cuda.Stream()
            if PREFETCH_HIPRIO in ("1", "main"):
                gkw["stream"] = torch.cuda.Stream(priority=-1)
        inputs = [dict(static_inputs) for _ in range(sets)]
        if prefetch is not None:
            for p_ in range(sets):
                inputs[p_]["backbone_maps"] = self.maps[p_]
        call = (lambda p_, cb: step_fwd_bwd(inputs[p_], cb)) if split else (lambda p_, cb: step_fwd_bwd(inputs[p_]))
        s = torch.cuda.Stream()
        s.wait_stream(torch.cuda.current_stream())
        with torch.cuda.stream(s):
            for _ in range(warmup):
                optimizer.zero_grad()
                call(0, ddp.hot_path_done if split else None)
                scale = ddp.sync_gradients() if ddp is not None else 1.0
                optimizer.step(grad_scale=scale)
        torch.cuda.current_stream().wait_stream(s)
        torch.cuda.synchronize()

        def fork(p_):
            if prefetch is None:
                return
            self._pf_stream.wait_stream(torch.cuda.current_stream())
            lib = L.load()
            prev = lib.a3d_bn_grid_cap(PREFETCH_BN_GRID) if PREFETCH_BN_GRID > 0 else 0
            try:
                with torch.cuda.stream(self._pf_stream), torch.no_grad():
                    prefetch(self.next_rgbs, out=self.maps[1 - p_])
            finally:
                if PREFETCH_BN_GRID > 0:
                    lib.a3d_bn_grid_cap(prev)

        def join():
            if prefetch is not None:
                torch.cuda.current_stream().wait_stream(self._pf_stream)

        self.g_fb, self.g_late, self.loss = [], [], []
        self.g_opt = None
        pool = None
        for p_ in range(sets):
            g = torch.cuda.CUDAGraph()
            self.g_fb.append(g)
            if not split:
                with (torch.cuda.graph(g, **gkw) if pool is None else torch.cuda.graph(g, pool=pool, **gkw)):
                    fork(p_)
                    optimizer.zero_grad()
                    self.loss.append(call(p_, None))
                    optimizer.step(grad_scale=1.0)
                    join()
                pool = g.pool()
                continue
            g2 = torch.cuda.CUDAGraph()
            self.g_late.append(g2)
            ctx = {}

            def switch_graphs():
                join()
                ctx["first"].__exit__(None, None, None)
                ctx["second"] = torch.cuda.graph(g2, pool=g.pool() if pool is None else pool, **gkw)
                ctx["second"].__enter__()

            ctx["first"] = torch.cuda.graph(g, **gkw) if pool is None else torch.cuda.graph(g, pool=pool, **gkw)
            ctx["first"].__enter__()
            try:
                fork(p_)
                optimizer.zero_grad()
                self.loss.append(call(p_, switch_graphs))
            finally:
                if "second" not in ctx:
                    join()
                (ctx.get("second") or ctx["first"]).__exit__(None, None, None)
            pool = g.pool()
        if split:
            self.g_opt = torch.cuda.CUDAGraph()
            with torch.cuda.graph(self.g_opt, pool=pool, **gkw):
                optimizer.step(grad_scale=1.0 / self.world)
        self._last = 0

    def launch(self, inputs=None, next_rgbs=None):
        if inputs is not None:
            for k, v in inputs.items():
                if torch.is_tensor(v) and k in self.static_inputs and v.data_ptr() != self.static_inputs[k].data_ptr():
                    self.static_inputs[k].copy_(v, non_blocking=True)
        p_ = 0
        if self.prefetch is not None:
            p_ = self.parity
            if self._primed and PREFETCH_CHECK and not torch.equal(self.static_inputs["rgbs"], self.next_rgbs):
                raise RuntimeError("GraphedStep(prefetch): this launch's images are not the next_rgbs the previous launch was given -- "
                                   "the maps prefetched for it belong to another batch")
            if not self._primed:
                with torch.no_grad():
                    self.prefetch(self.static_inputs["rgbs"], out=self.maps[p_])
                self._primed = True
            src = next_rgbs if next_rgbs is not None else self.static_inputs["rgbs"]
            if src.data_ptr() != self.next_rgbs.data_ptr():
                self.next_rgbs.copy_(src, non_blocking=True)
            self.parity ^= 1
        self._last = p_
        self.g_fb[p_].replay()
        if self.world > 1:
            self.ddp.arm(True)
            self.ddp.hot_path_done()
            self.g_late[p_].replay()
            self.ddp.begin_sync()

    def finish(self):
        if self.world > 1:
            self.ddp.finish_sync()
            self.g_opt.replay()
        return self.loss[self._last]

    def __call__(self, inputs=None, next_rgbs=None):
        self.launch(inputs, next_rgbs)
        return self.finish()


class GraphedJointStep:

    def __init__(self, keypose_step, trajectory_step):
        self.kp, self.tr = keypose_step, trajectory_step

    def __call__(self, kp_sample=None, tr_sample=None):
        self.kp.launch(kp_sample)
        self.tr.launch(tr_sample)
        return self.kp.finish(), self.tr.finish()
```

### act3d-chained-diffuser_amd/lib.py

```python
import ctypes as C
import os

import torch

_PKG_DIR = os.path.dirname(os.path.abspath(__file__))
LIB_PATH = os.path.join(_PKG_DIR, os.path.basename(os.environ.get("A3D_LIB", "libact3d_hip.so")))

_p = C.c_void_p
_i = C.c_int
_f = C.c_float
_z = C.c_size_t
_u64 = C.c_ulonglong



def _struct(name, fields):
    return type(name, (C.Structure,), {"_fields_": [(f, t) for f, t in fields]})


DnHeadParams = _struct("DnHeadParams", [(n, _p) for n in ("enc_w0", "enc_b0", "enc_w1", "enc_b1", "sem", "lang_kv")] +
                       [("S_lang", _i)] + [(n, _p) for n in ("q_w", "q_b", "out_w", "out_b", "ln_g", "ln_b")])
DnCrossParams = _struct("DnCrossParams", [(n, _p) for n in ("sem", "mod", "q_w", "q_b", "freq", "Kf", "Vt")])
DnRestParams = _struct("DnRestParams", [(n, _p) for n in (
    "c_out_w", "c_out_b", "c_ln_g", "c_ln_b", "sem", "s_mod", "s_in_w", "s_in_b", "s_out_w", "s_out_b", "s_ln_g", "s_ln_b", "freq",
    "kmask", "f_mod", "f_w1", "f_b1", "f_w2", "f_b2", "f_ln_g", "f_ln_b")] + [("F", _i)])
DnLayerParams = _struct("DnLayerParams", [("cross", DnCrossParams), ("rest", DnRestParams)])
DnTailParams = _struct("DnTailParams", [(n, _p) for n in (
    "pos_w0", "pos_b0", "pos_w1", "pos_b1", "rot_w0", "rot_b0", "rot_w1", "rot_b1", "noise", "cond_data", "cond_mask", "coef_pos",
    "coef_rot")])

QsParams = _struct("QsParams", [(n, _p) for n in ("wv", "bv", "wo", "bo", "g1", "b1", "w1", "c1", "w2", "c2", "g2", "b2")])
QsGrads = _struct("QsGrads", [(n, _p) for n in ("dwv", "dbv", "dwo", "dbo", "dg1", "db1", "dw1", "dc1", "dw2", "dc2", "dg2", "db2")])

SIGNATURES = {
    "a3d_version": (_i, []),
    "a3d_last_error_string": (C.c_char_p, []),
    "a3d_linear_fwd": (_i, [_p, _i, _p, _i, _p, _p, _i, _p, _i, _i, _i, _i, _i, _i, _p]),
    "a3d_linear_wgrad": (_i, [_p, _i, _p, _i, _p, _i, _p, _i, _i, _i, _p]),
    "a3d_linear_wgrad_ws": (_i, [_p, _i, _p, _i, _p, _i, _p, _i, _i, _i, _p, _z, _p]),
    "a3d_linear_wgrad_ws_bytes": (_z, [_i, _i, _i, _i]),
    "a3d_add_layernorm_fwd": (_i, [_p, _p, _p, _p, _p, _p, _p, _i, _i, _f, _p]),
    "a3d_add_layernorm_bwd": (_i, [_p, _p, _p, _p, _p, _p, _p, _p, _p, _i, _i, _p]),
    "a3d_rope_split_qk": (_i, [_p, _i, _p, _p, _f, _p, _i, _i, _i, _i, _i, _p]),
    "a3d_split_vt": (_i, [_p, _i, _p, _i, _i, _i, _i, _i, _p]),
    "a3d_proj_rope_split": (_i, [_p, _i, _p, _i, _p, _i, _p, _f, _p, _i, _p, _p, _f, _p, _i, _p, _p, _i, _i, _i, _i, _i, _p]),
    "a3d_rope_split": (_i, [_p, _i, _p, _p, _f, _p, _i, _p, _i, _i, _i, _i, _i, _p]),
    "a3d_rope_merge_bwd": (_i, [_p, _i, _p, _p, _f, _p, _i, _i, _i, _i, _i, _i, _p]),
    "a3d_attn_fwd": (_i, [_p, _p, _p, _p, _p, _p, _p, _i, _i, _i, _i, _i, _i, _i, _p]),
    "a3d_attn_fwd_ws_floats": (_z, [_i, _i, _i, _i]),
    "a3d_attn_bwd_bf16": (_i, [_p] * 15 + [_i] * 7 + [_p]),
    "a3d_rope_split16": (_i, [_p, _i, _p, _p, _f, _p, _p, _i, _i, _i, _i, _i, _i, _p]),
    "a3d_proj_rope_split16": (_i, [_p, _i, _p, _i, _p, _i, _p, _f, _p, _p, _i, _p, _f, _p, _p, _i, _p, _i, _i, _i, _i, _i, _p]),
    "a3d_attn16_fwd": (_i, [_p] * 7 + [_i] * 7 + [_p, C.c_uint, _f, _p]),
    "a3d_attn16_fwd_rows": (_i, [_p] * 7 + [_i] * 7 + [_p, C.c_uint, _f, _i, _p]),
    "a3d_conv3x3_tile_count": (_z, [_z, _i, _i]),
    "a3d_conv3x3_dgrad_tiles_ws_ints": (_z, [_z, _i, _i]),
    "a3d_conv3x3_mark_tiles": (_i, [_p, _i, _i, _i, _i, _i, _p, _p]),
    "a3d_conv3x3_dgrad_tiles": (_i, [_p, _p, _p, _p, _p, _z, _i, _i, _p]),
    "a3d_conv3x3_wgrad_tokens_ws_floats": (_z, []),
    "a3d_conv3x3_wgrad_tokens": (_i, [_p, _p, _p, _i, _i, _p, _p, _i, _i, _i, _i, _i, _i, _p]),
    "a3d_attn16_bwd_pack_bytes": (_z, [_i, _i, _i]),
    "a3d_dbg_dn_prof": (_i, [_p]),
    "a3d_attn8_operand_bytes": (_z, [_i, _i, _i]),
    "a3d_attn8_fwd": (_i, [_p] * 8 + [_i] * 7 + [_p]),
    "a3d_attn16_bwd": (_i, [_p] * 16 + [_i] * 7 + [_p, C.c_uint, _f, _p]),
    "a3d_pose_to_signal": (_i, [_p, _p, _p, _i, _i, _p]),
    "a3d_signal_to_pose": (_i, [_p, _p, _p, _i, _i, _p]),
    "a3d_traj_errors": (_i, [_p, _p, _p, _i, _i, _i, _p]),
    "a3d_keypose_errors": (_i, [_p, _p, _p, _p, _i, _p, _i, _i, _i, _p]),
    "a3d_sym_quat_loss": (_i, [_p, _p, _i, _f, _p, _p, _i, _p]),
    "a3d_sq_fwd_ws_floats": (_z, [_i, _i, _i, _i]),
    "a3d_sq_attn_fwd": (_i, [_p, _p, _p, _i, _p, _p, _i, _p, _p, _p, _p, _p, _p, _p, _i, _i, _i, _i, _i, _p]),
    "a3d_sq_bwd_ws_floats": (_z, [_i, _i, _i, _i]),
    "a3d_sq_attn_bwd": (_i, [_p, _p, _p, _i, _p, _p, _i, _p, _p, _p, _p, _p, _p, _p, _p, _p, _i, _p, _p, _i, _p, _i, _i, _i, _i,
                             _i, _p]),
    "a3d_sq_attn_bwd_acc": (_i, [_p, _p, _p, _i, _p, _p, _i, _p, _p, _p, _p, _p, _p, _p, _p, _p, _i, _p, _p, _i, _p, _i, _i, _i, _i,
                                 _i, _i, _p]),
    "a3d_qs_pre_fwd": (_i, [_p, _p, _p, _p, _p, _f, _p, _i, _i, _i, _p]),
    "a3d_qs_pre_bwd": (_i, [_p, _i, _p, _p, _f, _p, _p, _p, _p, _p, _i, _i, _i, _p]),
    "a3d_qs_save_floats": (_z, [_i, _i]),
    "a3d_qs_post_fwd": (_i, [_p, _p, _p, _p, _p, _i, _i, _i, _p]),
    "a3d_qs_post_bwd": (_i, [_p, _p, _p, _p, _p, _p, _p, _p, _p, _i, _i, _i, _p]),
    "a3d_sq_wgrad_reduce": (_i, [_p, _i, _p, _i, _p, _i, _p]),
    "a3d_dn_head": (_i, [_p, _i, _p, _p, _i, _i, _i, _i, _p]),
    "a3d_dn_cross_ws_floats": (_z, [_i, _i, _i]),
    "a3d_dn_cross": (_i, [_p, _p, _i, _p, _p, _i, _i, _i, _i, _i, _i, _i, _p]),
    "a3d_dn_rest": (_i, [_p, _p, _i, _p, _p, _p, _i, _i, _i, _i, _i, _p]),
    "a3d_dn_tail": (_i, [_p, _p, _p, _i, _p, _p, _i, _i, _i, _i, _p]),
    "a3d_dn_persist_splits": (_i, [_i, _i]),
    "a3d_dn_persist_sync_ints": (_z, [_i, _i, _i, _i]),
    "a3d_dn_persist_kvx_floats": (_z, [_i, _i, _i]),
    "a3d_dn_persist_prof": (_i, [_p, _i, _i, _i, _i, _p]),
    "a3d_dn_persist_xbuf_floats": (_z, [_i, _i]),
    "a3d_dn_persist": (_i, [_p, _i, _i, _i, _p, _p, _p, _p, _p, _p, _p, _p] + [_i] * 10 + [_p]),
    "a3d_rope_rows_f32": (_i, [_p, _i, _p, _p, _f, _p, _i, _i, _i, _i, _i, _p]),
    "a3d_dropout": (_i, [_p, _p, _z, _p, C.c_uint, _f, _p]),
    "a3d_dropout_mask": (_i, [_p, _z, _p, C.c_uint, C.c_uint, C.c_uint, _f, _p]),
    "a3d_linear_fwd_drop": (_i, [_p, _i, _p, _i, _p, _p, _i, _p, _i, _i, _i, _i, _i, _i, _p, C.c_uint, _f, _p]),
    "a3d_add_layernorm_bwd_drop": (_i, [_p] * 10 + [_i, _i, _p, C.c_uint, _f, _p]),
    "a3d_attn_fwd_dropout": (_i, [_p, _p, _p, _p, _p, _p, _p, _i, _i, _i, _i, _i, _i, _i, _p, C.c_uint, _f, _p]),
    "a3d_attn_bwd_bf16_dropout": (_i, [_p] * 15 + [_i] * 7 + [_p, C.c_uint, _f, _p]),
    "a3d_pcd_downsample": (_i, [_p, _p, _i, _i, _i, _i, _i, _p]),
    "a3d_knn_topk_ws_bytes": (_z, [_i, _i]),
    "a3d_knn_topk": (_i, [_p, _p, _p, _p, _p, _i, _i, _i, _p]),
    "a3d_traj_nn_topk": (_i, [_p, _i, _p, _p, _p, _p, _i, _i, _i, _p]),
    "a3d_build_context": (_i, [_p, _p, _p, _p, _i, _i, _i, _i, _i, _p]),
    "a3d_build_context_bwd": (_i, [_p, _p, _p, _p, _i, _i, _i, _i, _i, _i, _p]),
    "a3d_build_context_bf16": (_i, [_p, _i, _p, _p, _p, _p, _i, _i, _i, _i, _i, _p]),
    "a3d_colsum_rows_ws_floats": (_z, [_i, _i, _i]),
    "a3d_colsum_rows": (_i, [_p, _i, _i, _i, _i, _i, _p, _i, _p, _p]),
    "a3d_build_context_bwd_bf16": (_i, [_p, _p, _p, _i, _p, _i, _i, _i, _i, _i, _i, _p]),
    "a3d_mask_logits_fwd": (_i, [_p, _p, _p, _i, _i, _i, _p]),
    "a3d_mask_logits_bwd": (_i, [_p, _p, _p, _p, _p, _i, _i, _i, _i, _p]),
    "a3d_argmax_gather": (_i, [_p, _p, _p, _p, _i, _i, _p]),
    "a3d_soft_ce_loss": (_i, [_p, _p, _p, _p, _p, _p, _i, _i, _f, _f, _f, _p]),
    "a3d_elem_loss": (_i, [_p, _p, _i, _i, _f, _p, _p, _p]),
    "a3d_scale_by_scalar": (_i, [_p, _p, _p, _z, _p]),
    "a3d_quat_sigmoid_fwd": (_i, [_p, _p, _p, _i, _p]),
    "a3d_quat_sigmoid_bwd": (_i, [_p, _p, _p, _p, _i, _p]),
    "a3d_ortho6d_sigmoid_fwd": (_i, [_p, _p, _p, _i, _p]),
    "a3d_ortho6d_sigmoid_bwd": (_i, [_p, _p, _p, _p, _i, _p]),
    "a3d_select_row_fwd": (_i, [_p, _p, _p, _i, _i, _i, _p]),
    "a3d_select_row_bwd": (_i, [_p, _p, _p, _i, _i, _i, _p]),
    "a3d_sample_ghost_points": (_i, [_p, _p, _p, _f, _p, _i, _i, _i, _i, _p]),
    "a3d_rng_advance": (_i, [_p, _u64, _p]),
    "a3d_philox4x32_10_host": (None, [_p, _p, _p]),
    "a3d_sincos_host": (None, [_p, _p, _p, _z]),
    "a3d_adamw_step": (_i, [_p, _p, _p, _p, _p, _p, _p, _i, _z, _z, _f, _f, _f, _f, _f, _f, _f, _p]),
    "a3d_dbg_mfma_bf16": (_i, [_p, _p, _p, _p]),
    "a3d_dbg_mfma_f32": (_i, [_p, _p, _p, _p]),
    "a3d_dbg_cvt_pk_bf16": (_i, [_p, _p, _i, _p]),
    "a3d_bn_nslab": (_i, [_z, _i]),
    "a3d_bn_grid_cap": (_i, [_i]),
    "a3d_conv1x1_streams": (_i, [_i, _i]),
    "a3d_conv1x1_nslab": (_i, [_z, _i, _i]),
    "a3d_conv1x1_bn_fwd": (_i, [_p, _p, _p, _p, _i, _p, _p, _z, _i, _i, _p]),
    "a3d_conv1x1_topdown_serves": (_i, [_i, _i]),
    "a3d_conv1x1_topdown_fwd": (_i, [_p, _p, _p, _i, _p, _p, _z, _i, _i, _i, _i, _p]),
    "a3d_conv3x3_serves": (_i, [_i, _i, _i, _i]),
    "a3d_conv1x1_deep_mode": (_i, [_i]),
    "a3d_stem_conv_nslab": (_i, [_z, _i, _i]),
    "a3d_stem_conv_bn_fwd": (_i, [_p, _p, _p, _p, _p, _p, _z, _i, _i, _p]),
    "a3d_conv3x3_nslab": (_i, [_z, _i, _i, _i, _i]),
    "a3d_conv3x3_bn_fwd": (_i, [_p, _p, _p, _p, _i, _p, _p, _z, _i, _i, _i, _i, _p]),
    "a3d_bn_stats": (_i, [_p, _p, _z, _i, _i, _p]),
    "a3d_bn_finalize": (_i, [_p, _i, _z, _i, _f, _f, _p, _p, _p, _p, _p, _p, _i, _p]),
    "a3d_bn_apply": (_i, [_p, _p, _p, _p, _p, _p, _p, _z, _i, _i, _p]),
    "a3d_bn_apply_pool2": (_i, [_p, _p, _p, _p, _p, _p, _i, _i, _i, _i, _i, _p]),
    "a3d_rgb_normalize_nhwc_bf16": (_i, [_p, _p, _p, _p, _z, _i, _i, _p]),
    "a3d_upsample2_add_fwd": (_i, [_p, _p, _p, _i, _p, _i, _i, _i, _i, _p]),
    "a3d_upsample2_add_bwd_ws_floats": (_z, [_i, _i, _i, _i]),
    "a3d_upsample2_add_bwd": (_i, [_p, _p, _p, _i, _p, _i, _i, _i, _i, _p]),
    "a3d_ddpm_add_noise": (_i, [_p, _p, _p, _p, _p, _p, _i, _i, _i, _i, _p]),
    "a3d_ddpm_step": (_i, [_p, _p, _p, _p, _p, _p, _p, _p, _i, _i, _i, _i, _p]),
    "a3d_adaln_fwd": (_i, [_p, _p, _p, _i, _i, _i, _p]),
    "a3d_adaln_bwd": (_i, [_p, _p, _p, _p, _p, _i, _i, _i, _p]),
    "a3d_sinusoidal_emb": (_i, [_p, _p, _i, _i, _p]),
    "a3d_silu_fwd": (_i, [_p, _p, _z, _p]),
    "a3d_silu_bwd": (_i, [_p, _p, _p, _z, _p]),
    "a3d_add_rows": (_i, [_p, _p, _p, _i, _i, _i, _p]),
    "a3d_add_rows_bwd": (_i, [_p, _p, _i, _i, _i, _p]),
    "a3d_resize_crop": (_i, [_p, _p, _p, _i, _i, _i, _i, _f, _f, _p]),
    "a3d_traj_update": (_i, [_p, _p, _p, _i, _i, _i, _p]),
}

_lib = None


def load():
    global _lib
    if _lib is not None:
        return _lib
    if not os.path.exists(LIB_PATH):
        raise RuntimeError(
            "libact3d_hip.so is missing (%s). Build it with `python -c 'import __graft_entry__ as g; g.build()'` "
            "(needs hipcc); there is no CPU fallback." % LIB_PATH)
    lib = C.CDLL(LIB_PATH)
    for name, (res, args) in SIGNATURES.items():
        try:
            fn = getattr(lib, name)
        except AttributeError as e:
            raise RuntimeError("libact3d_hip.so does not export %s (stale build?)" % name) from e
        fn.restype = res
        fn.argtypes = args
    _lib = lib
    return lib


def exported_symbols():
    return list(SIGNATURES.keys())


def last_error():
    s = load().a3d_last_error_string()
    return s.decode() if s else ""


def check(rc, what=""):
    if rc != 0:
        raise RuntimeError("libact3d_hip %s failed with code %d: %s" % (what, rc, last_error()))


def ptr(t):
    if t is None:
        return None
    assert t.is_contiguous(), "libact3d_hip needs contiguous tensors"
    return t.data_ptr()


def stream():
    return torch.cuda.current_stream().cuda_stream


def require_gpu(*tensors):
    for t in tensors:
        if t is not None and not t.is_cuda:
            raise RuntimeError("act3d_amd ops run on an MI355X device tensor; got a %s tensor "
                               "(there is no CPU fallback)" % t.device)


def call(name, *args):
    lib = load()
    rc = getattr(lib, name)(*args)
    if rc != 0:
        raise RuntimeError("%s failed with code %d: %s" % (name, rc, last_error()))
```

### act3d-chained-diffuser_amd/nn.py

```python
import math
import os

import torch
import torch.nn as nn
import torch.nn.functional as F

from . import ops as O


class MultiheadCustomAttention(nn.Module):

    def __init__(self, embed_dim, num_heads, dropout=0.0):
        super().__init__()
        assert embed_dim % num_heads == 0 and embed_dim // num_heads == 15, \
            "the HIP attention kernels are specialised for head_dim 15 (60/4, 120/8), as in both reference models"
        self.embed_dim, self.num_heads, self.dropout = embed_dim, num_heads, dropout
        self.in_proj_weight = nn.Parameter(torch.empty(3 * embed_dim, embed_dim))
        self.in_proj_bias = nn.Parameter(torch.zeros(3 * embed_dim))
        self.out_proj = nn.Linear(embed_dim, embed_dim)
        nn.init.xavier_uniform_(self.in_proj_weight)
        nn.init.constant_(self.out_proj.bias, 0.0)


class RelativeCrossAttentionLayer(nn.Module):
    def __init__(self, embedding_dim, num_heads, dropout=0.0):
        super().__init__()
        self.multihead_attn = MultiheadCustomAttention(embedding_dim, num_heads, dropout=dropout)
        self.norm = nn.LayerNorm(embedding_dim)
        self.num_heads = num_heads

    def forward(self, query, value, query_xyz=None, value_xyz=None, pad_mask=None, sink=None):
        return O.attn_block(query, value, value, query, query_xyz, value_xyz, pad_mask, self.multihead_attn, self.norm,
                            self.num_heads, sink=sink)


class FeedforwardLayer(nn.Module):
    def __init__(self, embedding_dim, hidden_dim, dropout=0.0):
        super().__init__()
        self.linear1 = nn.Linear(embedding_dim, hidden_dim)
        self.linear2 = nn.Linear(hidden_dim, embedding_dim)
        self.norm = nn.LayerNorm(embedding_dim)
        for p in self.parameters():
            if p.dim() > 1:
                nn.init.xavier_uniform_(p)

    def forward(self, x):
        return O.mlp(x, self.linear1, self.linear2, self.norm)


class RelativeCrossAttentionModule(nn.Module):
    def __init__(self, embedding_dim, num_attn_heads, num_layers):
        super().__init__()
        self.attn_layers = nn.ModuleList(
            [RelativeCrossAttentionLayer(embedding_dim, num_attn_heads) for _ in range(num_layers)])
        self.ffw_layers = nn.ModuleList([FeedforwardLayer(embedding_dim, embedding_dim) for _ in range(num_layers)])

    def forward(self, query, value, query_xyz=None, value_xyz=None):
        output = []
        sink = getattr(value, "_a3d_sink", None)
        for attn, ffw in zip(self.attn_layers, self.ffw_layers):
            mha = attn.multihead_attn
            if O.query_layer_applicable(query, value, mha.embed_dim, attn.num_heads, ffw.linear1.out_features):
                query = O.QueryLayerFn.apply(query, value, query_xyz, value_xyz, mha.in_proj_weight, mha.in_proj_bias,
                                             mha.out_proj.weight, mha.out_proj.bias, attn.norm.weight, attn.norm.bias,
                                             ffw.linear1.weight, ffw.linear1.bias, ffw.linear2.weight, ffw.linear2.bias,
                                             ffw.norm.weight, ffw.norm.bias, attn.num_heads, sink)
            else:
                query = ffw(attn(query, value, query_xyz, value_xyz, sink=sink))
            output.append(query)
        return output


class AdaLN(nn.Module):
    def __init__(self, embedding_dim):
        super().__init__()
        self.modulation = nn.Sequential(nn.SiLU(), nn.Linear(embedding_dim, 2 * embedding_dim, bias=True))
        nn.init.constant_(self.modulation[-1].weight, 0)
        nn.init.constant_(self.modulation[-1].bias, 0)

    def forward(self, x, silu_t):
        return O.AdaLNFn.apply(x, O.linear(silu_t, self.modulation[1]))


class ParallelAttentionLayer(nn.Module):

    def __init__(self, d_model=256, dropout=0.1, n_heads=8, pre_norm=False, self_attention1=True,
                 self_attention2=False, cross_attention1=True, cross_attention2=False, apply_ffn=True,
                 slot_attention12=False, slot_attention21=False, rotary_pe=False, use_adaln=False):
        super().__init__()
        if pre_norm or self_attention2 or cross_attention2 or slot_attention12 or slot_attention21 or not cross_attention1:
            raise NotImplementedError("only the seq1 / post-norm configuration of ParallelAttentionLayer is on the hot "
                                      "path (SURVEY §8a-12); other options are not implemented")
        self.self_attention1, self.apply_ffn, self.rotary_pe = self_attention1, apply_ffn, rotary_pe
        self.n_heads, self.dropout_p = n_heads, dropout
        self.site_base = O.site_id("parallel_attention_layer")
        if self_attention1:
            self.adaln_1 = AdaLN(d_model) if use_adaln else None
            self.sa1 = MultiheadCustomAttention(d_model, n_heads, dropout=dropout)
            self.norm_1 = nn.LayerNorm(d_model)
        self.adaln_12 = AdaLN(d_model) if use_adaln else None
        self.cross_12 = MultiheadCustomAttention(d_model, n_heads, dropout=dropout)
        self.norm_12 = nn.LayerNorm(d_model)
        self.adaln_ff1 = AdaLN(d_model) if use_adaln else None
        self.ffn_12 = nn.Sequential(nn.Linear(d_model, 4 * d_model), nn.ReLU(), nn.Dropout(dropout),
                                    nn.Linear(4 * d_model, d_model), nn.Dropout(dropout))
        self.norm_122 = nn.LayerNorm(d_model)

    def forward(self, seq1, seq1_key_padding_mask, seq2, seq1_xyz=None, seq2_xyz=None, seq1_sem_pos=None, silu_t=None,
                drop=None):
        if self.training and self.dropout_p > 0 and drop is None:
            raise RuntimeError("ParallelAttentionLayer in training mode with dropout=%g needs the forward pass's DropCtx "
                               "(DiffusionHead.begin_dropout())" % self.dropout_p)
        if drop is not None and (not self.training or self.dropout_p <= 0):
            drop = None
        sb = self.site_base
        rope = self.rotary_pe
        q1 = seq1 if seq1_sem_pos is None else O.AddRowsFn.apply(seq1, seq1_sem_pos)
        qa = self.adaln_12(q1, silu_t) if (self.adaln_12 is not None and silu_t is not None) else q1
        seq1 = O.attn_block(qa, seq2, seq2, seq1, seq1_xyz if rope else None, seq2_xyz if rope else None, None,
                            self.cross_12, self.norm_12, self.n_heads, drop=drop, site=sb, sink=getattr(seq2, "_a3d_sink", None))
        if self.self_attention1:
            q1 = seq1 if seq1_sem_pos is None else O.AddRowsFn.apply(seq1, seq1_sem_pos)
            if self.adaln_1 is not None and silu_t is not None:
                qk, vv = self.adaln_1(q1, silu_t), self.adaln_1(seq1, silu_t)
            else:
                qk, vv = q1, seq1
            seq1 = O.attn_block(qk, qk, vv, seq1, seq1_xyz if rope else None, seq1_xyz if rope else None,
                                seq1_key_padding_mask, self.sa1, self.norm_1, self.n_heads, drop=drop, site=sb + 2)
        if self.apply_ffn:
            y = self.adaln_ff1(seq1, silu_t) if (self.adaln_ff1 is not None and silu_t is not None) else seq1
            seq1 = O.mlp(y, self.ffn_12[0], self.ffn_12[3], self.norm_122, drop=drop, site_hidden=sb + 4, site_out=sb + 5)
        return seq1


class ParallelAttention(nn.Module):
    def __init__(self, num_layers=1, **kw):
        super().__init__()
        self.layers = nn.ModuleList([ParallelAttentionLayer(**kw) for _ in range(num_layers)])

    def forward(self, seq1, seq1_key_padding_mask, seq2, **kw):
        for layer in self.layers:
            seq1 = layer(seq1, seq1_key_padding_mask, seq2, **kw)
        return seq1


class _Upsample2AddFn(torch.autograd.Function):

    @staticmethod
    def forward(ctx, lat, top, bias):
        N, C, H, W = lat.shape
        y = torch.empty_like(lat)
        O.L.call("a3d_upsample2_add_fwd", lat.data_ptr(), None if top is None else top.data_ptr(),
                 None if bias is None else bias.data_ptr(), 0 if bias is None else bias.numel(), y.data_ptr(), N, H, W, C,
                 O.L.stream())
        ctx.bias = bias
        ctx.has_top = top is not None
        return y

    @staticmethod
    def backward(ctx, dy):
        dy, dtop = _top_down_backward(dy, ctx.bias, ctx.has_top and ctx.needs_input_grad[1])
        return (dy if ctx.needs_input_grad[0] else None), dtop, None


def _top_down_backward(dy, bias, want_top):
    N, C, H, W = dy.shape
    want_bias = bias is not None and bias.requires_grad
    dtop = None
    if want_top or want_bias:
        dy = dy.contiguous(memory_format=torch.channels_last)
        if want_top:
            dtop = torch.empty((N, C, H // 2, W // 2), device=dy.device, dtype=dy.dtype, memory_format=torch.channels_last)
        ws = gb = None
        if want_bias:
            ws = torch.empty((O.L.load().a3d_upsample2_add_bwd_ws_floats(N, H, W, C),), device=dy.device, dtype=torch.float32)
            gb = O.grad_buf(bias)
        O.L.call("a3d_upsample2_add_bwd", dy.data_ptr(), None if dtop is None else dtop.data_ptr(),
                 None if gb is None else gb.data_ptr(), 0 if gb is None else gb.numel(), None if ws is None else ws.data_ptr(),
                 N, H, W, C, O.L.stream())
    return dy, dtop


FUSED_FPN_LATERAL = os.environ.get("A3D_FPN_LATERAL", "1") not in ("0", "", "off")
FUSED_FPN_OUT3X3 = os.environ.get("A3D_FPN_OUT3X3", "1") not in ("0", "", "off")


class _LateralTopDownFn(torch.autograd.Function):

    @staticmethod
    def forward(ctx, x, w, bias, top):
        N, K, H, W = x.shape
        Co = w.shape[0]
        w16 = w.detach().to(torch.bfloat16).reshape(Co, K).contiguous()
        y = torch.empty((N, Co, H, W), device=x.device, dtype=torch.bfloat16, memory_format=torch.channels_last)
        O.L.call("a3d_conv1x1_topdown_fwd", x.data_ptr(), w16.data_ptr(), None if bias is None else bias.data_ptr(),
                 0 if bias is None else bias.numel(), None if top is None else top.data_ptr(), y.data_ptr(), N, H, W, K, Co, O.L.stream())
        ctx.save_for_backward(x, w16)
        ctx.bias = bias
        ctx.has_top = top is not None
        return y

    @staticmethod
    def backward(ctx, dy):
        x, w16 = ctx.saved_tensors
        dy, dtop = _top_down_backward(dy, ctx.bias, ctx.has_top and ctx.needs_input_grad[3])
        need_x, need_w = ctx.needs_input_grad[0], ctx.needs_input_grad[1]
        dx = dw = None
        if need_x or need_w:
            dy = dy.contiguous(memory_format=torch.channels_last)
            w4 = w16.view(w16.shape[0], w16.shape[1], 1, 1)
            dx, dw, _ = torch.ops.aten.convolution_backward(dy, x, w4, None, (1, 1), (0, 0), (1, 1), False, (0, 0), 1, (need_x, need_w, False))
        return dx, (None if dw is None else dw.float()), None, dtop


def _fused_lateral_ok(x, Co, last):
    cl = torch.channels_last
    return bool(FUSED_FPN_LATERAL and x.is_cuda and x.dtype == torch.bfloat16 and x.dim() == 4 and x.is_contiguous(memory_format=cl)
                and O.L.load().a3d_conv1x1_topdown_serves(x.shape[1], Co)
                and (last is None or (last.dtype == torch.bfloat16 and last.is_contiguous(memory_format=cl) and last.shape[1] == Co
                                      and x.shape[-2] == 2 * last.shape[-2] and x.shape[-1] == 2 * last.shape[-1])))


def _fused_top_down_ok(lat, last, with_bias=False):
    cl = torch.channels_last
    ok = (lat.is_cuda and lat.dtype == torch.bfloat16 and lat.shape[1] % 4 == 0 and lat.shape[-2] % 2 == 0 and lat.shape[-1] % 2 == 0
          and lat.is_contiguous(memory_format=cl))
    if last is not None:
        ok = ok and (last.dtype == torch.bfloat16 and lat.shape[-2] == 2 * last.shape[-2] and lat.shape[-1] == 2 * last.shape[-1]
                     and last.is_contiguous(memory_format=cl))
    if with_bias:
        ok = ok and 256 % (lat.shape[1] // 4) == 0
    return ok


def fpn_top_down(lat, last, bias=None):
    if _fused_top_down_ok(lat, last, bias is not None):
        return _Upsample2AddFn.apply(lat, last, bias)
    if bias is not None:
        lat = lat + F.pad(bias, (0, lat.shape[1] - bias.numel())).to(lat.dtype).view(1, -1, 1, 1)
    return lat if last is None else lat + F.interpolate(last, size=lat.shape[-2:], mode="nearest")


class _LayerConv3x3Fn(torch.autograd.Function):

    @staticmethod
    def forward(ctx, x, w, cc):
        w16 = w.to(x.dtype)
        if (FUSED_FPN_OUT3X3 and x.is_cuda and x.dtype == torch.bfloat16 and x.is_contiguous(memory_format=torch.channels_last)
                and O.L.load().a3d_conv3x3_serves(x.shape[1], w16.shape[0], x.shape[2], x.shape[3])):
            w16 = w16.contiguous(memory_format=torch.channels_last)
            y = torch.empty((x.shape[0], w16.shape[0], x.shape[2], x.shape[3]), device=x.device, dtype=torch.bfloat16,
                            memory_format=torch.channels_last)
            O.L.call("a3d_conv3x3_bn_fwd", x.data_ptr(), w16.data_ptr(), None, None, 0, y.data_ptr(), None, x.shape[0], x.shape[2], x.shape[3],
                     x.shape[1], w16.shape[0], O.L.stream())
        else:
            y = F.conv2d(x, w16, None, padding=1)
        ctx.save_for_backward(x, w16)
        ctx.cc = cc
        cc.x, cc.dw, cc.dense = x, None, False
        cc.mask, cc.ntok = None, 0
        if O.SPARSE_FPN_DGRAD and ctx.needs_input_grad[0] and O.L.load().a3d_conv3x3_tile_count(x.shape[0], x.shape[2], x.shape[3]) > 0 \
                and x.shape[2] // 8 <= 255 and x.shape[3] // 32 <= 255:
            cc.mask = torch.zeros((O.L.load().a3d_conv3x3_tile_count(x.shape[0], x.shape[2], x.shape[3]),), device=x.device, dtype=torch.uint8)
        return y

    @staticmethod
    def backward(ctx, dy):
        x, w16 = ctx.saved_tensors
        cc = ctx.cc
        sparse = cc.dw is not None and not cc.dense
        need_x, need_w = ctx.needs_input_grad[0], ctx.needs_input_grad[1]
        dx = dw = None
        N, _, H, W = x.shape
        sparse_x = (need_x and sparse and cc.mask is not None and 0 < cc.ntok <= O.SPARSE_FPN_DGRAD_MAX * N * H * W and dy.dtype == torch.bfloat16)
        if sparse_x:
            dy = dy.contiguous(memory_format=torch.channels_last)
            wt = w16.flip(2, 3).permute(1, 2, 3, 0).contiguous()
            dx = torch.empty_like(x, memory_format=torch.channels_last)
            ws = torch.empty((O.L.load().a3d_conv3x3_dgrad_tiles_ws_ints(N, H, W),), device=x.device, dtype=torch.int32)
            O.L.call("a3d_conv3x3_dgrad_tiles", dy.data_ptr(), wt.data_ptr(), cc.mask.data_ptr(), ws.data_ptr(), dx.data_ptr(), N, H, W, O.L.stream())
            need_x = False
        if need_x or (need_w and not sparse):
            dy = dy.contiguous(memory_format=torch.channels_last)
            dxl, dw, _ = torch.ops.aten.convolution_backward(dy, x, w16, None, (1, 1), (1, 1), (1, 1), False, (0, 0), 1,
                                                             (need_x, need_w and not sparse, False))
            if need_x:
                dx = dxl
        if need_w and sparse:
            dw = cc.dw.permute(2, 3, 0, 1).contiguous()
        cc.dw, cc.mask = None, None
        return dx, (None if dw is None else dw.float()), None


class FeaturePyramidNetwork(nn.Module):

    def __init__(self, in_channels_list, out_channels):
        super().__init__()
        self.inner_blocks = nn.ModuleList([nn.Sequential(nn.Conv2d(c, out_channels, 1)) for c in in_channels_list])
        self.layer_blocks = nn.ModuleList(
            [nn.Sequential(nn.Conv2d(out_channels, out_channels, 3, padding=1)) for _ in in_channels_list])
        for m in self.modules():
            if isinstance(m, nn.Conv2d):
                nn.init.kaiming_uniform_(m.weight, a=1)
                nn.init.constant_(m.bias, 0)

    def forward(self, feats, needed=None, pad_to=None, defer_output_bias=None, sparse_ncam=None):
        names = list(feats.keys())
        xs = list(feats.values())
        C = self.inner_blocks[0][0].out_channels
        pad = 0 if pad_to is None else max(0, pad_to - C)

        def conv(m, x, wpad, with_bias, **kw):
            w = F.pad(m.weight, wpad) if pad else m.weight
            b = None
            if with_bias:
                b = F.pad(m.bias, (0, pad)) if pad else m.bias
            return F.conv2d(x, w, b, **kw)

        def inner(i, x, last):
            m = self.inner_blocks[i][0]
            wpad = (0, 0, 0, 0, 0, 0, 0, pad)
            Co = C + pad
            bf16 = x.dtype == torch.bfloat16 or (torch.is_autocast_enabled() and torch.get_autocast_gpu_dtype() == torch.bfloat16)
            fuse = (x.is_cuda and bf16 and Co % 4 == 0 and 256 % (Co // 4) == 0 and x.shape[-1] % 2 == 0 and x.shape[-2] % 2 == 0
                    and (last is None or (x.shape[-2] == 2 * last.shape[-2] and x.shape[-1] == 2 * last.shape[-1])))
            if not fuse:
                lat = conv(m, x, wpad, True)
                return lat if last is None else fpn_top_down(lat, last)
            if _fused_lateral_ok(x, Co, last):
                return _LateralTopDownFn.apply(x, F.pad(m.weight, wpad) if pad else m.weight, m.bias, last)
            return fpn_top_down(conv(m, x, wpad, False), last, m.bias)

        out_bias, out_ctx = {}, {}

        def layer(i, x):
            m = self.layer_blocks[i][0]
            defer = defer_output_bias and x.is_cuda
            if defer:
                out_bias[names[i]] = m.bias
            if (defer and sparse_ncam and O.SPARSE_FPN_WGRAD and C + pad == 64 and x.dtype == torch.bfloat16 and x.shape[1] == 64
                    and x.is_contiguous(memory_format=torch.channels_last) and x.shape[0] % sparse_ncam == 0):
                cc = O.SparseConvCtx(sparse_ncam)
                out_ctx[names[i]] = cc
                w = F.pad(m.weight, (0, 0, 0, 0, 0, pad, 0, pad)) if pad else m.weight
                return _LayerConv3x3Fn.apply(x, w, cc)
            return conv(m, x, (0, 0, 0, 0, 0, pad, 0, pad), not defer, padding=1)

        last = inner(len(xs) - 1, xs[-1], None)
        out = {}
        lowest = min(names.index(n) for n in needed) if needed is not None else 0
        if needed is None or names[-1] in needed:
            out[names[-1]] = layer(len(xs) - 1, last)
        for i in range(len(xs) - 2, lowest - 1, -1):
            last = inner(i, xs[i], last)
            if needed is None or names[i] in needed:
                out[names[i]] = layer(i, last)
        if defer_output_bias is None:
            return out
        return (out, out_bias, out_ctx) if sparse_ncam else (out, out_bias)


class _Bottleneck(nn.Module):
    expansion = 4

    def __init__(self, inplanes, planes, stride=1):
        super().__init__()
        self.conv1 = nn.Conv2d(inplanes, planes, 1, bias=False)
        self.bn1 = nn.BatchNorm2d(planes)
        self.conv2 = nn.Conv2d(planes, planes, 3, padding=1, bias=False)
        self.bn2 = nn.BatchNorm2d(planes)
        self.avgpool = nn.AvgPool2d(stride) if stride > 1 else nn.Identity()
        self.conv3 = nn.Conv2d(planes, planes * 4, 1, bias=False)
        self.bn3 = nn.BatchNorm2d(planes * 4)
        self.downsample = None
        if stride > 1 or inplanes != planes * 4:
            self.downsample = nn.Sequential(nn.AvgPool2d(stride), nn.Conv2d(inplanes, planes * 4, 1, bias=False),
                                            nn.BatchNorm2d(planes * 4))

    def forward(self, x):
        out = F.relu(self.bn1(self.conv1(x)))
        out = F.relu(self.bn2(self.conv2(out)))
        out = self.bn3(self.conv3(self.avgpool(out)))
        return F.relu(out + (x if self.downsample is None else self.downsample(x)))


class SyntheticCLIPResNet50(nn.Module):

    def __init__(self, width=64, layers=(3, 4, 6, 3)):
        super().__init__()
        self.conv1 = nn.Conv2d(3, width // 2, 3, stride=2, padding=1, bias=False)
        self.bn1 = nn.BatchNorm2d(width // 2)
        self.conv2 = nn.Conv2d(width // 2, width // 2, 3, padding=1, bias=False)
        self.bn2 = nn.BatchNorm2d(width // 2)
        self.conv3 = nn.Conv2d(width // 2, width, 3, padding=1, bias=False)
        self.bn3 = nn.BatchNorm2d(width)
        self.avgpool = nn.AvgPool2d(2)
        self._inplanes = width
        self.layer1 = self._make_layer(width, layers[0])
        self.layer2 = self._make_layer(width * 2, layers[1], stride=2)
        self.layer3 = self._make_layer(width * 4, layers[2], stride=2)
        self.layer4 = self._make_layer(width * 8, layers[3], stride=2)

    def _make_layer(self, planes, blocks, stride=1):
        layers = [_Bottleneck(self._inplanes, planes, stride)]
        self._inplanes = planes * 4
        for _ in range(1, blocks):
            layers.append(_Bottleneck(self._inplanes, planes))
        return nn.Sequential(*layers)

    def forward(self, x):
        x = F.relu(self.bn1(self.conv1(x)))
        x = F.relu(self.bn2(self.conv2(x)))
        x0 = F.relu(self.bn3(self.conv3(x)))
        x1 = self.layer1(self.avgpool(x0))
        x2 = self.layer2(x1)
        x3 = self.layer3(x2)
        x4 = self.layer4(x3)
        return {"res1": x0, "res2": x1, "res3": x2, "res4": x3, "res5": x4}


class ClipNormalize(nn.Module):

    def __init__(self):
        super().__init__()
        self.register_buffer("mean", torch.tensor([0.48145466, 0.4578275, 0.40821073]).view(1, 3, 1, 1), persistent=False)
        self.register_buffer("std", torch.tensor([0.26862954, 0.26130258, 0.27577711]).view(1, 3, 1, 1), persistent=False)

    def forward(self, x):
        return (x - self.mean) / self.std


def load_synthetic_clip():
    return SyntheticCLIPResNet50(), ClipNormalize()


def bn_scale_shift(x, bn, partial=None):
    N, C, H, W = x.shape
    rows = N * H * W
    dev = x.device
    st = O.L.stream()
    scale = torch.empty((2, C), device=dev, dtype=torch.float32)
    train = 1 if bn.training else 0
    nslab = 1
    if train and partial is None:
        nslab = O.L.load().a3d_bn_nslab(rows, C)
        partial = torch.empty((nslab, 2, C), device=dev, dtype=torch.float32)
        O.L.call("a3d_bn_stats", x.data_ptr(), partial.data_ptr(), rows, C, nslab, st)
    elif train:
        nslab = partial.shape[0]
    O.L.call("a3d_bn_finalize", None if not train else partial.data_ptr(), nslab, rows, C, float(bn.eps),
             float(bn.momentum if bn.momentum is not None else 0.1), bn.weight.data_ptr(), bn.bias.data_ptr(),
             bn.running_mean.data_ptr(), bn.running_var.data_ptr(), scale[0].data_ptr(), scale[1].data_ptr(), train, st)
    return scale


def conv1x1_bn(x, conv, in_scale=None, in_relu=False, want_stats=True):
    N, K, H, W = x.shape
    Cout = conv.weight.shape[0]
    assert x.dtype == torch.bfloat16 and x.is_contiguous(memory_format=torch.channels_last)
    assert conv.kernel_size == (1, 1) and conv.stride == (1, 1) and conv.bias is None and conv.weight.dtype == torch.bfloat16
    M = N * H * W
    w2 = conv.weight.reshape(Cout, K)
    assert w2.is_contiguous()
    y = torch.empty((N, Cout, H, W), device=x.device, dtype=torch.bfloat16, memory_format=torch.channels_last)
    partial = None
    if want_stats:
        partial = torch.empty((O.L.load().a3d_conv1x1_nslab(M, K, Cout), 2, Cout), device=x.device, dtype=torch.float32)
    O.L.call("a3d_conv1x1_bn_fwd", x.data_ptr(), w2.data_ptr(), None if in_scale is None else in_scale[0].data_ptr(),
             None if in_scale is None else in_scale[1].data_ptr(), 1 if in_relu else 0, y.data_ptr(),
             None if partial is None else partial.data_ptr(), M, K, Cout, O.L.stream())
    return y, partial


def conv3x3_serves(x, conv):
    return bool(conv.kernel_size == (3, 3) and conv.stride == (1, 1) and conv.padding == (1, 1) and conv.dilation == (1, 1) and
                conv.groups == 1 and conv.bias is None and conv.weight.dtype == torch.bfloat16 and x.dtype == torch.bfloat16 and
                O.L.load().a3d_conv3x3_serves(x.shape[1], conv.weight.shape[0], x.shape[2], x.shape[3]))


def conv3x3_bn(x, conv, in_scale=None, in_relu=False, want_stats=True):
    N, Cin, H, W = x.shape
    Cout = conv.weight.shape[0]
    assert x.is_contiguous(memory_format=torch.channels_last) and conv3x3_serves(x, conv)
    wt = conv.weight
    assert wt.is_contiguous(memory_format=torch.channels_last)
    y = torch.empty((N, Cout, H, W), device=x.device, dtype=torch.bfloat16, memory_format=torch.channels_last)
    partial = None
    if want_stats:
        partial = torch.empty((O.L.load().a3d_conv3x3_nslab(N, H, W, Cin, Cout), 2, Cout), device=x.device, dtype=torch.float32)
    O.L.call("a3d_conv3x3_bn_fwd", x.data_ptr(), wt.data_ptr(), None if in_scale is None else in_scale[0].data_ptr(),
             None if in_scale is None else in_scale[1].data_ptr(), 1 if in_relu else 0, y.data_ptr(),
             None if partial is None else partial.data_ptr(), N, H, W, Cin, Cout, O.L.stream())
    return y, partial


FUSED_STEM = os.environ.get("A3D_FUSED_STEM", "1") == "1"


def stem_serves(x, conv, normalize):
    return bool(FUSED_STEM and x.is_cuda and x.dtype == torch.float32 and x.dim() == 4 and x.shape[1] == 3 and x.is_contiguous() and
                isinstance(normalize, ClipNormalize) and isinstance(conv, nn.Conv2d) and conv.in_channels == 3 and conv.out_channels == 32 and
                conv.kernel_size == (3, 3) and conv.stride == (2, 2) and conv.padding == (1, 1) and conv.bias is None and
                conv.weight.dtype == torch.bfloat16 and O.L.load().a3d_stem_conv_nslab(x.shape[0], x.shape[2], x.shape[3]) > 0)


def stem_conv_bn(x, conv, normalize, want_stats=True):
    N, _, H, W = x.shape
    w2 = conv.weight.reshape(32, 27)
    if not w2.is_contiguous():
        w2 = conv.weight.contiguous().reshape(32, 27)
    y = torch.empty((N, 32, H // 2, W // 2), device=x.device, dtype=torch.bfloat16, memory_format=torch.channels_last)
    partial = None
    if want_stats:
        partial = torch.empty((O.L.load().a3d_stem_conv_nslab(N, H, W), 2, 32), device=x.device, dtype=torch.float32)
    O.L.call("a3d_stem_conv_bn_fwd", x.data_ptr(), normalize.mean.reshape(-1).contiguous().data_ptr(),
             normalize.std.reshape(-1).contiguous().data_ptr(), w2.data_ptr(), y.data_ptr(), None if partial is None else partial.data_ptr(),
             N, H, W, O.L.stream())
    return y, partial


def bn_act(x, bn, relu=True, residual=None, pool=False, keep_full=True, partial=None, residual_scale=None, out=None):
    N, C, H, W = x.shape
    if out is not None:
        assert out.shape == x.shape and out.dtype == x.dtype and out.is_contiguous(memory_format=torch.channels_last)
    assert x.dtype == torch.bfloat16 and x.is_contiguous(memory_format=torch.channels_last)
    if residual is not None:
        assert residual.shape == x.shape and residual.dtype == x.dtype and \
            residual.is_contiguous(memory_format=torch.channels_last)
    rows = N * H * W
    dev = x.device
    st = O.L.stream()
    sc_ptr = sh_ptr = None
    if bn is not None:
        scale = bn_scale_shift(x, bn, partial)
        sc_ptr, sh_ptr = scale[0].data_ptr(), scale[1].data_ptr()
    res_ptr = None if residual is None else residual.data_ptr()
    if not pool:
        y = out if out is not None else torch.empty_like(x)
        O.L.call("a3d_bn_apply", x.data_ptr(), res_ptr, None if residual_scale is None else residual_scale[0].data_ptr(),
                 None if residual_scale is None else residual_scale[1].data_ptr(), sc_ptr, sh_ptr, y.data_ptr(), rows, C,
                 1 if relu else 0, st)
        return y
    assert residual_scale is None, "the pooled apply takes a materialised residual"
    y = (out if out is not None else torch.empty_like(x)) if keep_full else None
    yp = torch.empty((N, C, H // 2, W // 2), device=dev, dtype=x.dtype, memory_format=torch.channels_last)
    O.L.call("a3d_bn_apply_pool2", x.data_ptr(), res_ptr, sc_ptr, sh_ptr, None if y is None else y.data_ptr(), yp.data_ptr(),
             N, H, W, C, 1 if relu else 0, st)
    return y, yp


def _pool2_ok(m, t):
    return isinstance(m, nn.AvgPool2d) and m.kernel_size in (2, (2, 2)) and t.shape[-1] % 2 == 0 and t.shape[-2] % 2 == 0


def fused_frozen_backbone_forward(bb, x, stem=None, out=None):
    conv = lambda m, t: F.conv2d(t, m.weight, None, m.stride, m.padding)
    fuse3 = FUSED_CONV3X3
    o_ = (lambda k: None) if out is None else (lambda k, _maps=out: _maps[k])

    def conv3(m, t, bn_in, p_in, want_stats):
        if fuse3 and conv3x3_serves(t, m):
            return conv3x3_bn(t, m, in_scale=bn_scale_shift(t, bn_in, p_in), in_relu=True, want_stats=want_stats)
        return conv(m, bn_act(t, bn_in, partial=p_in)), None

    c1, p1 = stem if stem is not None else (conv(bb.conv1, x), None)
    c2, p2 = conv3(bb.conv2, c1, bb.bn1, p1, bb.bn2.training)
    c3, p3 = conv3(bb.conv3, c2, bb.bn2, p2, bb.bn3.training)
    if _pool2_ok(bb.avgpool, c3):
        x0, x = bn_act(c3, bb.bn3, pool=True, partial=p3, out=o_("res1"))
    else:
        x0 = bn_act(c3, bb.bn3, partial=p3, out=o_("res1"))
        x = bb.avgpool(x0)
    outs = [x0]
    bns = [bb.bn1, bb.bn2, bb.bn3]
    blocks = [blk for layer in (bb.layer1, bb.layer2, bb.layer3, bb.layer4) for blk in layer]
    last_of_layer = {id(layer[-1]) for layer in (bb.layer1, bb.layer2, bb.layer3, bb.layer4)}
    x_pooled = None
    fuse = FUSED_CONV1X1

    def fused_ok(m, t):
        return bool(fuse and m.kernel_size == (1, 1) and m.stride == (1, 1) and
                    O.L.load().a3d_conv1x1_streams(t.shape[1], m.weight.shape[0]))

    def conv1(m, t, **kw):
        if fused_ok(m, t):
            return conv1x1_bn(t, m, **kw)
        return conv(m, t), None

    for bi, blk in enumerate(blocks):
        c1, p1 = conv1(blk.conv1, x, want_stats=blk.bn1.training)
        c2, p2 = conv3(blk.conv2, c1, blk.bn1, p1, blk.bn2.training)
        no_pool = isinstance(blk.avgpool, nn.Identity) or (isinstance(blk.avgpool, nn.AvgPool2d) and blk.avgpool.kernel_size in (1, (1, 1)))
        if no_pool and fused_ok(blk.conv3, c2):
            o3, p3 = conv1x1_bn(c2, blk.conv3, in_scale=bn_scale_shift(c2, blk.bn2, p2), in_relu=True, want_stats=blk.bn3.training)
        else:
            if _pool2_ok(blk.avgpool, c2):
                out = bn_act(c2, blk.bn2, pool=True, keep_full=False, partial=p2)[1]
            else:
                out = blk.avgpool(bn_act(c2, blk.bn2, partial=p2))
            o3, p3 = conv1(blk.conv3, out, want_stats=blk.bn3.training)
        if blk.downsample is not None:
            dpool = blk.downsample[0]
            if x_pooled is not None:
                xin = x_pooled
            elif _pool2_ok(dpool, x):
                xin = bn_act(x, None, relu=False, pool=True, keep_full=False)[1]
            elif isinstance(dpool, nn.AvgPool2d) and dpool.kernel_size in (1, (1, 1)):
                xin = x
            else:
                xin = dpool(x)
            cd, pd = conv1(blk.downsample[1], xin, want_stats=blk.downsample[2].training)
            bns.append(blk.downsample[2])
        nxt = blocks[bi + 1] if bi + 1 < len(blocks) else None
        want_pooled = nxt is not None and nxt.downsample is not None and _pool2_ok(nxt.downsample[0], o3)
        idn_scale = None
        if blk.downsample is None:
            idn = x
        elif FOLD_DOWNSAMPLE_BN and not want_pooled:
            idn, idn_scale = cd, bn_scale_shift(cd, blk.downsample[2], pd)
        else:
            idn = bn_act(cd, blk.downsample[2], relu=False, partial=pd)
        o_x = o_("res%d" % (len(outs) + 1)) if id(blk) in last_of_layer else None
        if want_pooled:
            x, x_pooled = bn_act(o3, blk.bn3, relu=True, residual=idn, pool=True, partial=p3, out=o_x)
        else:
            x, x_pooled = bn_act(o3, blk.bn3, relu=True, residual=idn, partial=p3, residual_scale=idn_scale, out=o_x), None
        bns += [blk.bn1, blk.bn2, blk.bn3]
        if id(blk) in last_of_layer:
            outs.append(x)
    if bb.training:
        torch._foreach_add_([b.num_batches_tracked for b in bns], 1)
    return dict(zip(["res1", "res2", "res3", "res4", "res5"], outs))


FUSED_BN = os.environ.get("A3D_FUSED_BN", "1") == "1"
FOLD_DOWNSAMPLE_BN = os.environ.get("A3D_FOLD_DS_BN", "1") not in ("0", "", "off")
FUSED_CONV1X1 = os.environ.get("A3D_FUSED_CONV1X1", "1") not in ("0", "", "off")
FUSED_CONV3X3 = os.environ.get("A3D_FUSED_CONV3X3", "1") not in ("0", "", "off")


def normalize_to_nhwc_bf16(x, normalize):
    x = x.float().contiguous()
    N, _, H, W = x.shape
    y = torch.empty((N, 3, H, W), device=x.device, dtype=torch.bfloat16, memory_format=torch.channels_last)
    O.L.call("a3d_rgb_normalize_nhwc_bf16", x.data_ptr(), normalize.mean.data_ptr(), normalize.std.data_ptr(), y.data_ptr(), N, H, W,
             O.L.stream())
    return y


def run_frozen_backbone(backbone, x, dtype, keep_dtype=False, normalize=None, out=None):
    def deliver(feats):
        if out is None:
            return feats
        for k, v in feats.items():
            if v.data_ptr() != out[k].data_ptr():
                out[k].copy_(v)
        return out
    fused = FUSED_BN and x.is_cuda and dtype == torch.bfloat16 and isinstance(backbone, SyntheticCLIPResNet50)
    if normalize is not None and not (fused and isinstance(normalize, ClipNormalize) and (x.shape[-1] * x.shape[-2]) % 4 == 0):
        x = normalize(x).contiguous(memory_format=torch.channels_last)
        normalize = None
    if dtype == torch.float32:
        return deliver(backbone(x))
    if getattr(backbone, "_conv_dtype", None) != dtype:
        for m in backbone.modules():
            if isinstance(m, nn.Conv2d):
                m.to(dtype)
                m.weight.data = m.weight.data.contiguous(memory_format=torch.channels_last)
        backbone._conv_dtype = dtype
    if fused:
        if normalize is not None and stem_serves(x, backbone.conv1, normalize):
            feats = fused_frozen_backbone_forward(backbone, None, stem=stem_conv_bn(x, backbone.conv1, normalize, want_stats=backbone.bn1.training),
                                                  out=out if keep_dtype else None)
        else:
            xb = normalize_to_nhwc_bf16(x, normalize) if normalize is not None else x.to(dtype).contiguous(memory_format=torch.channels_last)
            feats = fused_frozen_backbone_forward(backbone, xb, out=out if keep_dtype else None)
    else:
        feats = backbone(x.to(dtype))
    return deliver(feats if keep_dtype else {k: v.float() for k, v in feats.items()})
```

### include/act3d_hip.h

```cpp
#ifndef ACT3D_HIP_H
#define ACT3D_HIP_H
#include <stddef.h>
#include <stdint.h>
#ifdef __cplusplus
extern "C" {
#endif

int a3d_version(void);
const char* a3d_last_error_string(void);

int a3d_linear_fwd(const float* X, int ldx, const float* W, int ldw, const float* bias, float* Y, int ldy,
                   const float* mask, int ldm, int M, int N, int K, int act, int w_transposed, void* stream);
int a3d_linear_wgrad(const float* dY, int lddy, const float* X, int ldx, float* dW, int lddw, float* db, int M,
                     int N, int K, void* stream);
size_t a3d_linear_wgrad_ws_bytes(int M, int N, int K, int has_bias);
int a3d_linear_wgrad_ws(const float* dY, int lddy, const float* X, int ldx, float* dW, int lddw, float* db, int M,
                        int N, int K, float* ws, size_t ws_bytes, void* stream);
int a3d_add_layernorm_fwd(const float* A, const float* R, const float* gamma, const float* beta, float* Y,
                          float* mean, float* rstd, int M, int E, float eps, void* stream);
int a3d_add_layernorm_bwd(const float* A, const float* R, const float* gamma, const float* mean, const float* rstd,
                          const float* dY, float* dS, float* dgamma, float* dbeta, int M, int E, void* stream);

int a3d_rope_split_qk(const float* Y, int ldy, const float* xyz, const float* freq, float scale, void* dst, int B,
                      int N, int Npad, int E, int H, void* stream);
int a3d_split_vt(const float* Y, int ldy, void* dst, int B, int N, int Npad, int E, int H, void* stream);
int a3d_rope_split(const float* Y, int ldy, const float* xyz, const float* freq, float scale, void* rows_out,
                   int rows_width, void* planes_out, int B, int N, int Npad, int E, int H, void* stream);
int a3d_proj_rope_split(const float* X, int ldx, const float* W, int ldw, const float* bias, int K, const float* xyz0,
                        float scale0, void* rows0, int rows0_width, void* planes0, const float* xyz1, float scale1,
                        void* rows1, int rows1_width, void* planes1, const float* freq, int B, int N, int Npad, int E,
                        int H, void* stream);
int a3d_rope_merge_bwd(const float* dR, int nsplit, const float* xyz, const float* freq, float scale, float* dY,
                       int ldy, int B, int N, int Npad, int E, int H, void* stream);

int a3d_attn_fwd(const void* Qs, const void* Ks, const void* Vt, const unsigned char* kmask, float* O, float* LSE,
                 float* ws, int B, int H, int Lq, int Lqp, int S, int Sp, int nsplit, void* stream);
size_t a3d_attn_fwd_ws_floats(int B, int H, int Lqp, int nsplit);
int a3d_attn_bwd_bf16(const void* Qs, const void* Qt, const void* Ks, const void* Kt, const void* Vs,
                      const unsigned char* kmask, const float* O, const float* dO, const float* LSE, void* dOs,
                      void* dOt, float* D, float* dQp, float* dK, float* dV, int B, int H, int Lq, int Lqp, int S,
                      int Sp, int nsplit, void* stream);

int a3d_dropout(const float* x, float* y, size_t n, const unsigned long long* drop_state, unsigned int site, float p,
                void* stream);
int a3d_linear_fwd_drop(const float* X, int ldx, const float* W, int ldw, const float* bias, float* Y, int ldy,
                        const float* mask, int ldm, int M, int N, int K, int act, int w_transposed,
                        const unsigned long long* drop_state, unsigned int site, float p, void* stream);
int a3d_add_layernorm_bwd_drop(const float* A, const float* R, const float* gamma, const float* mean, const float* rstd,
                               const float* dY, float* dS, float* dS_drop, float* dgamma, float* dbeta, int M, int E,
                               const unsigned long long* drop_state, unsigned int site, float p, void* stream);
int a3d_dropout_mask(unsigned char* out, size_t n, const unsigned long long* drop_state, unsigned int c2, unsigned int c1,
                     unsigned int site, float p, void* stream);
int a3d_rope_split16(const float* Y, int ldy, const float* xyz, const float* freq, float scale, void* rows_out,
                     void* planes_out, int plane_parts, int B, int N, int Npad, int E, int H, void* stream);
int a3d_proj_rope_split16(const float* X, int ldx, const float* W, int ldw, const float* bias, int K, const float* xyz0,
                          float scale0, void* rows0, void* planes0, int parts0, const float* xyz1, float scale1, void* rows1,
                          void* planes1, int parts1, const float* freq, int B, int N, int Npad, int E, int H, void* stream);
int a3d_attn16_fwd(const void* Qr, const void* Kr, const void* Vp, const unsigned char* kmask, float* O, float* LSE2,
                   float* ws, int B, int H, int Lq, int Lqp, int S, int Sp, int nsplit,
                   const unsigned long long* drop_state, unsigned int drop_site, float drop_p, void* stream);
int a3d_attn16_fwd_rows(const void* Qr, const void* Kr, const void* Vr, const unsigned char* kmask, float* O, float* LSE2,
                        float* ws, int B, int H, int Lq, int Lqp, int S, int Sp, int nsplit,
                        const unsigned long long* drop_state, unsigned int drop_site, float drop_p, int nograd, void* stream);
size_t a3d_attn16_bwd_pack_bytes(int B, int H, int Lqp);
int a3d_attn16_bwd(const void* Qr, const void* Qp, const void* Kr, const void* Kp, const void* Vr,
                   const unsigned char* kmask, const float* O, const float* dO, const float* LSE2, void* dOr, void* pack,
                   float* D, int* rexp, float* dQp, float* dK, float* dV, int B, int H, int Lq, int Lqp, int S, int Sp,
                   int nsplit, const unsigned long long* drop_state, unsigned int drop_site, float drop_p, void* stream);

size_t a3d_attn8_operand_bytes(int B, int H, int Sp);
int a3d_attn8_fwd(const void* Qr, const void* Kr, const void* Vp, void* ops8, const unsigned char* kmask, float* O,
                  float* LSE2, float* ws, int B, int H, int Lq, int Lqp, int S, int Sp, int nsplit, void* stream);

int a3d_attn_fwd_dropout(const void* Qs, const void* Ks, const void* Vt, const unsigned char* kmask, float* O, float* LSE,
                         float* ws, int B, int H, int Lq, int Lqp, int S, int Sp, int nsplit,
                         const unsigned long long* drop_state, unsigned int site, float p, void* stream);
int a3d_attn_bwd_bf16_dropout(const void* Qs, const void* Qt, const void* Ks, const void* Kt, const void* Vs,
                              const unsigned char* kmask, const float* O, const float* dO, const float* LSE, void* dOs,
                              void* dOt, float* D, float* dQp, float* dK, float* dV, int B, int H, int Lq, int Lqp, int S,
                              int Sp, int nsplit, const unsigned long long* drop_state, unsigned int site, float p,
                              void* stream);

size_t a3d_sq_fwd_ws_floats(int B, int H, int E, int nsplit);
int a3d_sq_attn_fwd(const float* X, const float* xyz, const float* Wk, int ldw, const float* bk, const float* Wv, int ldwv,
                    const float* bv, const float* qrot, const float* freq, float* ws, float* xbar, float* lse, float* o, int B,
                    int S, int E, int H, int nsplit, void* stream);
size_t a3d_sq_bwd_ws_floats(int B, int H, int E, int nsplit);
int a3d_sq_attn_bwd(const float* X, const float* xyz, const float* Wk, int ldw, const float* bk, const float* Wv, int ldwv,
                    const float* qrot, const float* freq, const float* xbar, const float* lse, const float* dO, float* ws,
                    float* dX, float* dqp, float* dWk, int lddwk, float* dbk, float* dWv, int lddwv, float* dbv, int B, int S,
                    int E, int H, int nsplit, void* stream);
int a3d_sq_attn_bwd_acc(const float* X, const float* xyz, const float* Wk, int ldw, const float* bk, const float* Wv, int ldwv,
                        const float* qrot, const float* freq, const float* xbar, const float* lse, const float* dO, float* ws,
                        float* dX, float* dqp, float* dWk, int lddwk, float* dbk, float* dWv, int lddwv, float* dbv, int B, int S,
                        int E, int H, int nsplit, int accumulate_dX, void* stream);
int a3d_sq_wgrad_reduce(const float* partial, int nsplit, float* dW, int lddw, float* db, int E, void* stream);

int a3d_pcd_downsample(const float* pcd, float* out_xyz, int B, int C, int Hin, int Win, int factor, void* stream);
size_t a3d_knn_topk_ws_bytes(int B, int N);
int a3d_knn_topk(const float* pos, const float* xyz, void* ws, long long* idx_out, float* dist_out, int B, int N,
                 int k, void* stream);
int a3d_traj_nn_topk(const float* traj_xyz, int L, const float* xyz, void* ws, long long* idx_out, float* dist_out, int B,
                     int N, int k, void* stream);
int a3d_build_context(const float* feat, const long long* idx, const float* extra, float* ctx, int B, int Npts,
                      int k, int X, int W, void* stream);
int a3d_build_context_bwd(const float* dctx, const long long* idx, float* dfeat, float* dextra, int B, int Npts,
                          int k, int X, int W, int accumulate, void* stream);

int a3d_build_context_bf16(const void* feat, int ldf, const long long* idx, const float* extra, const float* bias, float* ctx,
                           int B, int Npts, int k, int X, int W, void* stream);
int a3d_build_context_bwd_bf16(const float* dctx, const long long* idx, void* dfeat, int ldf, float* dextra, int B,
                               int Npts, int k, int X, int W, int accumulate, void* stream);
size_t a3d_conv3x3_wgrad_tokens_ws_floats(void);
int a3d_conv3x3_wgrad_tokens(const void* X, const long long* idx, const float* G, int g_rows, int E, float* ws, float* dW,
                             int accumulate, int B, int k, int ncam, int H, int W, void* stream);
size_t a3d_conv3x3_tile_count(size_t images, int H, int W);
size_t a3d_conv3x3_dgrad_tiles_ws_ints(size_t images, int H, int W);
int a3d_conv3x3_mark_tiles(const long long* idx, int B, int k, int ncam, int H, int W, unsigned char* mask, void* stream);
int a3d_conv3x3_dgrad_tiles(const void* dy, const void* wt, const unsigned char* mask, int* ws, void* dx, size_t images, int H, int W,
                            void* stream);
size_t a3d_colsum_rows_ws_floats(int B, int k, int C);
int a3d_colsum_rows(const float* src, int B, int S, int k, int ld, int C, float* out, int nout, float* ws, void* stream);

int a3d_mask_logits_fwd(const float* q, const float* F, float* out, int B, int Ng, int E, void* stream);
int a3d_mask_logits_bwd(const float* q, const float* F, const float* dlog, float* dF, float* dq, int B, int Ng,
                        int E, int accumulate_dF, void* stream);
int a3d_argmax_gather(const float* logits, const float* ghost, long long* top_idx, float* pos, int B, int Ng,
                      void* stream);
int a3d_soft_ce_loss(const float* ghost, const float* gt, const float* logits, float* loss_b, float* loss,
                     float* dlogits, int B, int Ng, float spread, float label_smoothing, float coeff, void* stream);
int a3d_elem_loss(const float* pred, const float* target, int n, int kind, float coeff, float* loss, float* grad,
                  void* stream);
int a3d_scale_by_scalar(const float* x, const float* scalar, float* y, size_t n, void* stream);
int a3d_quat_sigmoid_fwd(const float* pred, float* rot, float* grip, int B, void* stream);
int a3d_quat_sigmoid_bwd(const float* pred, const float* drot, const float* dgrip, float* dpred, int B, void* stream);
int a3d_ortho6d_sigmoid_fwd(const float* pred, float* rot, float* grip, int B, void* stream);
int a3d_ortho6d_sigmoid_bwd(const float* pred, const float* drot, const float* dgrip, float* dpred, int B, void* stream);
int a3d_select_row_fwd(const float* x, const long long* idx, float* y, int B, int N, int W, void* stream);
int a3d_select_row_bwd(const float* dy, const long long* idx, float* dx, int B, int N, int W, void* stream);
int a3d_sample_ghost_points(const unsigned long long* state, const float* bounds, const float* anchor, float radius,
                            float* out, int B, int Ng, int level, int max_attempts, void* stream);
int a3d_rng_advance(unsigned long long* state, unsigned long long n, void* stream);
void a3d_philox4x32_10_host(const uint32_t ctr[4], const uint32_t key[2], uint32_t out[4]);
void a3d_sincos_host(const float* x, float* sn, float* cs, size_t n);
int a3d_adamw_step(float* p, const float* g, float* m, float* v, float* step, const long long* seg_off, float* seg_state,
                   int nseg, size_t n, size_t n_nodecay, float lr, float beta1, float beta2, float eps, float wd_nodecay,
                   float wd_decay, float grad_scale, void* stream);

typedef struct {
  const float *wv, *bv;
  const float *wo, *bo;
  const float *g1, *b1;
  const float *w1, *c1, *w2, *c2;
  const float *g2, *b2;
} a3d_qs_params;
typedef struct {
  float *dwv, *dbv, *dwo, *dbo, *dg1, *db1, *dw1, *dc1, *dw2, *dc2, *dg2, *db2;
} a3d_qs_grads;
int a3d_qs_pre_fwd(const float* x, const float* wq, const float* bq, const float* xyz, const float* freq, float scale, float* qrot,
                   int B, int E, int H, void* stream);
int a3d_qs_pre_bwd(const float* dqp, int nsplit, const float* xyz, const float* freq, float scale, const float* x, const float* wq,
                   float* dwq, float* dbq, float* dx, int B, int E, int H, void* stream);
size_t a3d_qs_save_floats(int B, int E);
int a3d_qs_post_fwd(const float* xbar, const float* resid, const a3d_qs_params* p, float* save, float* y, int B, int E, int H,
                    void* stream);
int a3d_qs_post_bwd(const float* dy, const float* resid, const float* xbar, const float* save, const a3d_qs_params* p,
                    const a3d_qs_grads* gr, float* dxbar, float* cD, float* dresid, int B, int E, int H, void* stream);

int a3d_ddpm_add_noise(const float* x0, const float* noise, const long long* t, const float* acp_pos,
                       const float* acp_rot, float* out, int B, int L, int D, int npos, void* stream);
int a3d_ddpm_step(const float* model_out, const float* sample, const float* noise, const float* cond_data,
                  const unsigned char* cond_mask, const float* coef_pos, const float* coef_rot, float* out, int rows,
                  int D, int npos, int t, void* stream);
int a3d_adaln_fwd(const float* x, const float* mod, float* y, int B, int L, int E, void* stream);
int a3d_adaln_bwd(const float* x, const float* mod, const float* dy, float* dx, float* dmod, int B, int L, int E,
                  void* stream);
int a3d_sinusoidal_emb(const float* x, float* out, int n, int E, void* stream);
int a3d_silu_fwd(const float* x, float* y, size_t n, void* stream);
int a3d_silu_bwd(const float* x, const float* dy, float* dx, size_t n, void* stream);
int a3d_add_rows(const float* x, const float* r, float* y, int B, int L, int E, void* stream);
int a3d_add_rows_bwd(const float* dy, float* dr, int B, int L, int E, void* stream);
int a3d_traj_update(const float* traj, const float* upd, float* out, int rows, int D, int npos, void* stream);

int a3d_pose_to_signal(const float* pose, const float* bounds, float* out, int n, int extra, void* stream);
int a3d_signal_to_pose(const float* signal, const float* bounds, float* out, int n, int extra, void* stream);
int a3d_traj_errors(const float* pred, const float* gt, float* cols, int B, int L, int D, void* stream);
int a3d_keypose_errors(const float* pos, const float* rot, const float* grip, const float* gt, int ldgt, float* cols, int B,
                       int nlev, int symmetric, void* stream);
int a3d_sym_quat_loss(const float* q, const float* gt, int ldgt, float coeff, float* loss, float* grad, int B, void* stream);

typedef struct {
  const float *enc_w0, *enc_b0, *enc_w1, *enc_b1;
  const float* sem;
  const float* lang_kv;
  int S_lang;
  const float *q_w, *q_b, *out_w, *out_b, *ln_g, *ln_b;
} a3d_dn_head_params;
typedef struct {
  const float* sem;
  const float* mod;
  const float *q_w, *q_b;
  const float* freq;
  const void* Kf;
  const unsigned short* Vt;
} a3d_dn_cross_params;
typedef struct {
  const float *c_out_w, *c_out_b, *c_ln_g, *c_ln_b;
  const float* sem;
  const float *s_mod, *s_in_w, *s_in_b, *s_out_w, *s_out_b, *s_ln_g, *s_ln_b;
  const float* freq;
  const unsigned char* kmask;
  const float *f_mod, *f_w1, *f_b1, *f_w2, *f_b2, *f_ln_g, *f_ln_b;
  int F;
} a3d_dn_rest_params;
typedef struct {
  const float *pos_w0, *pos_b0, *pos_w1, *pos_b1, *rot_w0, *rot_b0, *rot_w1, *rot_b1;
  const float *noise, *cond_data;
  const unsigned char* cond_mask;
  const float *coef_pos, *coef_rot;
} a3d_dn_tail_params;
int a3d_dn_head(const float* traj, int D, const a3d_dn_head_params* p, float* x_out, int B, int L, int E, int H, void* stream);
size_t a3d_dn_cross_ws_floats(int B, int H, int nsplit);
int a3d_dn_cross(const float* x, const float* traj, int D, const a3d_dn_cross_params* p, float* ws, int B, int L, int E,
                 int H, int S, int Sp, int nsplit, void* stream);
int a3d_dn_rest(const float* x_in, const float* traj, int D, const float* ws, const a3d_dn_rest_params* p, float* x_out,
                int B, int L, int E, int H, int nsplit, void* stream);
int a3d_dn_tail(const float* pos_feats, const float* rot_feats, const float* traj, int D, const a3d_dn_tail_params* p,
                float* traj_out, int B, int L, int E, int t_step, void* stream);
typedef struct {
  a3d_dn_cross_params cross;
  a3d_dn_rest_params rest;
} a3d_dn_layer_params;
int a3d_dn_persist_splits(int H, int nsplit);
size_t a3d_dn_persist_kvx_floats(int B, int L, int E);
size_t a3d_dn_persist_xbuf_floats(int B, int L);
int a3d_dn_persist_prof(const int* sync, int B, int L, int n_layers, int nsteps, long long* out256);
size_t a3d_dn_persist_sync_ints(int B, int L, int n_layers, int nsteps);
int a3d_dn_persist(const a3d_dn_layer_params* layers_dev, int n_traj, int n_pos, int n_rot, const a3d_dn_head_params* head,
                   const a3d_dn_tail_params* tail, float* traj, float* qbuf, float* part, float* kvx, float* xbuf, int* sync, int B,
                   int L, int D, int E, int H, int S, int Sp, int nsplit, int t_first, int nsteps, void* stream);
int a3d_dbg_dn_prof(long long* out18);
int a3d_rope_rows_f32(const float* Y, int ldy, const float* xyz, const float* freq, float scale, float* out, int B, int N,
                      int Npad, int E, int H, void* stream);

int a3d_bn_nslab(size_t rows, int C);
int a3d_bn_stats(const void* x, float* partial , size_t rows, int C, int nslab, void* stream);
int a3d_bn_finalize(const float* partial, int nslab, size_t rows, int C, float eps, float momentum, const float* gamma,
                    const float* beta, float* running_mean, float* running_var, float* scale, float* shift, int train,
                    void* stream);
int a3d_bn_apply(const void* x, const void* residual, const float* res_scale, const float* res_shift, const float* scale,
                 const float* shift, void* y, size_t rows, int C, int relu, void* stream);
int a3d_bn_apply_pool2(const void* x, const void* residual, const float* scale, const float* shift, void* y_full,
                       void* y_pool, int N, int H, int W, int C, int relu, void* stream);
int a3d_bn_grid_cap(int cap);
int a3d_upsample2_add_fwd(const void* lat, const void* top, const float* bias, int nbias, void* y, int N, int H, int W, int C,
                          void* stream);
size_t a3d_upsample2_add_bwd_ws_floats(int N, int H, int W, int C);
int a3d_upsample2_add_bwd(const void* dy, void* dtop, float* dbias, int nbias, float* ws, int N, int H, int W, int C,
                          void* stream);

int a3d_rgb_normalize_nhwc_bf16(const float* x, const float* mean, const float* stdv, void* y, size_t N, int H, int W,
                                void* stream);

int a3d_dbg_mfma_bf16(const void* A16x32, const void* B32x16, float* D16x16, void* stream);
int a3d_dbg_mfma_f32(const float* A16x4, const float* B4x16, float* D16x16, void* stream);
int a3d_dbg_cvt_pk_bf16(const float* in, void* out, int npairs, void* stream);

int a3d_conv1x1_streams(int K, int N);
int a3d_conv1x1_nslab(size_t M, int K, int N);
int a3d_conv1x1_bn_fwd(const void* x, const void* w, const float* in_scale, const float* in_shift, int in_relu, void* y,
                       float* partial, size_t M, int K, int N, void* stream);
int a3d_conv1x1_topdown_serves(int K, int N);
int a3d_conv1x1_topdown_fwd(const void* x, const void* w, const float* bias, int nbias, const void* top, void* y, size_t images,
                            int H, int W, int K, int N, void* stream);
int a3d_conv1x1_deep_mode(int mode);
int a3d_stem_conv_nslab(size_t images, int H, int W);
int a3d_stem_conv_bn_fwd(const float* rgb, const float* mean, const float* stdv, const void* w, void* y, float* partial, size_t images,
                         int H, int W, void* stream);

int a3d_conv3x3_serves(int Cin, int Cout, int H, int W);
int a3d_conv3x3_nslab(size_t images, int H, int W, int Cin, int Cout);
int a3d_conv3x3_bn_fwd(const void* x, const void* w, const float* in_scale, const float* in_shift, int in_relu, void* y,
                       float* partial, size_t images, int H, int W, int Cin, int Cout, void* stream);

int a3d_resize_crop(const float* src, float* dst, const int* params, int frames, int planes, int H, int W, float scale,
                    float shift, void* stream);

#ifdef __cplusplus
}
#endif
#endif
```

Before: 3494 samples/s.

## Fuse bottleneck block output BN+residual+ReLU into next block's conv1x1 load

Adds a conv1x1 variant that reads the raw conv3 output and the residual, applies BN scale/shift, adds the optionally BN-folded residual, applies ReLU while staging into LDS, and writes the activated block output once from the blockIdx.y==0 column. The separate bn_act pass over each block output in the ResNet backbone is skipped whenever the next block's conv1 shape is served (256->64 or 512->128 via the deep kernel). This is meant to cut one read-write pass and one kernel launch per block. It costs extra residual loads and registers inside the GEMM staging loop. Prefetch runs keep the unfused path by default, and the prefetch BN grid cap now defaults to the CU count instead of 256.

```diff
diff --git a/act3d-chained-diffuser_amd/csrc/a3d_common.h b/act3d-chained-diffuser_amd/csrc/a3d_common.h
--- a/act3d-chained-diffuser_amd/csrc/a3d_common.h
+++ b/act3d-chained-diffuser_amd/csrc/a3d_common.h
@@ -32,6 +32,22 @@
   typedef __bf16 bf16x2_t __attribute__((ext_vector_type(2)));
   typedef float f32x2_t __attribute__((ext_vector_type(2)));
   return __builtin_bit_cast(unsigned int, __builtin_convertvector(f32x2_t{a, b}, bf16x2_t));
+}
+__device__ __forceinline__ unsigned int bn_res_act2(unsigned int v, unsigned int r, float s0, float s1, float h0, float h1, bool has_res,
+                                                    bool res_bn, float rs0, float rs1, float rh0, float rh1, bool relu) {
+  float a = fmaf(__uint_as_float(v << 16), s0, h0);
+  float b = fmaf(__uint_as_float(v & 0xFFFF0000u), s1, h1);
+  if (has_res) {
+    float ra = __uint_as_float(r << 16), rb = __uint_as_float(r & 0xFFFF0000u);
+    if (res_bn) {
+      ra = fmaf(ra, rs0, rh0);
+      rb = fmaf(rb, rs1, rh1);
+    }
+    a += ra;
+    b += rb;
+  }
+  if (relu) { a = fmaxf(a, 0.f); b = fmaxf(b, 0.f); }
+  return pk_bf16(a, b);
 }
 __device__ __forceinline__ float bf2f(unsigned short h) {
   return __uint_as_float(((unsigned int)h) << 16);
@@ -188,5 +204,10 @@
 int conv1x1_deep_slabs(size_t M, int K, int N);
 int conv1x1_deep_launch(const void* x, const void* w, const float* in_scale, const float* in_shift, int in_relu, void* y, float* partial,
                         size_t M, int K, int N, hipStream_t s);
-
-}
+struct C1Residual { const unsigned short* res; const float* rscale; const float* rshift; unsigned short* x_out; };
+bool conv1x1_deep_res_serves(int K, int N);
+int conv1x1_deep_res_launch(const void* x_raw, const float* scale, const float* shift, const void* residual, const float* res_scale,
+                            const float* res_shift, int relu, const void* w, void* x_act_out, void* y, float* partial, size_t M, int K, int N,
+                            hipStream_t s);
+
+}
diff --git a/act3d-chained-diffuser_amd/csrc/conv1x1.hip b/act3d-chained-diffuser_amd/csrc/conv1x1.hip
--- a/act3d-chained-diffuser_amd/csrc/conv1x1.hip
+++ b/act3d-chained-diffuser_amd/csrc/conv1x1.hip
@@ -8,11 +8,11 @@
 __device__ __forceinline__ int c1_woff(int row, int seg) { return row * 32 + ((seg ^ (((row >> 1) & 1) | (((row >> 4) & 1) << 1))) << 3); }
 
 struct C1Epilogue { const float* bias; int nbias; const unsigned short* top; int H, W; };
-template <int WN, int KS, bool EP = false>
+template <int WN, int KS, bool EP = false, int RES = 0>
 __global__ __launch_bounds__(256, 2) void conv1x1_stream_kernel(const unsigned short* __restrict__ x, const unsigned short* __restrict__ w,
                                                              const float* __restrict__ in_scale, const float* __restrict__ in_shift,
                                                              int in_relu, unsigned short* __restrict__ y, float* __restrict__ partial,
-                                                             long long M, int N, C1Epilogue ep) {
+                                                             long long M, int N, C1Epilogue ep, C1Residual rz) {
   constexpr int WM = 4 / WN, BM = 64 * WM, BN = 64 * WN, K = KS * 32;
   constexpr int XL = BM * 4 / 256;
   constexpr int D = 8 / XL;
@@ -33,6 +33,9 @@
   }
   if (in_scale)
     for (int i = t; i < K; i += 256) { scS[i] = in_scale[i]; scS[K + i] = in_shift[i]; }
+  constexpr bool res_bn = RES == 2;
+  if (res_bn)
+    for (int i = t; i < K; i += 256) { scS[2 * K + i] = rz.rscale[i]; scS[3 * K + i] = rz.rshift[i]; }
   float ssum[4][4], ssq[4][4];
 #pragma unroll
   for (int a = 0; a < 4; ++a)
@@ -48,7 +51,7 @@
   }
   const long long my_tiles = blockIdx.x < mtiles ? (mtiles - blockIdx.x + gridDim.x - 1) / gridDim.x : 0;
   const long long total = my_tiles * KS;
-  auto load = [&](long long s, uint4 (&r)[XL]) {
+  auto load = [&](long long s, uint4 (&r)[XL], uint4 (&q)[XL]) {
     const long long m0 = (blockIdx.x + (s / KS) * gridDim.x) * BM;
     const int ks = (int)(s % KS);
 #pragma unroll
@@ -56,15 +59,30 @@
       const int idx = t + i * 256, row = idx >> 2, seg = idx & 3;
       const long long m = m0 + row < M ? m0 + row : M - 1;
       r[i] = *reinterpret_cast<const uint4*>(x + (size_t)m * K + ks * C1_BK + seg * 8);
+      if (RES) q[i] = *reinterpret_cast<const uint4*>(rz.res + (size_t)m * K + ks * C1_BK + seg * 8);
     }
   };
   const float relu_lo = in_relu ? 0.f : -INFINITY;
-  auto stage = [&](int buf, int ks, const uint4 (&r)[XL]) {
+  auto stage = [&](int buf, long long s, int ks, const uint4 (&r)[XL], const uint4 (&q)[XL]) {
 #pragma unroll
     for (int i = 0; i < XL; ++i) {
       const int idx = t + i * 256, row = idx >> 2, seg = idx & 3;
       uint4 v = r[i];
-      if (in_scale) {
+      if (RES) {
+        const int k0 = ks * C1_BK + seg * 8;
+        const unsigned int u[4] = {v.x, v.y, v.z, v.w}, qw[4] = {q[i].x, q[i].y, q[i].z, q[i].w};
+        unsigned int o[4];
+#pragma unroll
+        for (int j = 0; j < 4; ++j) {
+          const int k = k0 + 2 * j;
+          o[j] = bn_res_act2(u[j], qw[j], scS[k], scS[k + 1], scS[K + k], scS[K + k + 1], true, res_bn, res_bn ? scS[2 * K + k] : 0.f,
+                             res_bn ? scS[2 * K + k + 1] : 0.f, res_bn ? scS[3 * K + k] : 0.f, res_bn ? scS[3 * K + k + 1] : 0.f,
+                             in_relu != 0);
+        }
+        v = make_uint4(o[0], o[1], o[2], o[3]);
+        const long long m = (blockIdx.x + (s / KS) * gridDim.x) * BM + row;
+        if (blockIdx.y == 0 && m < M) *reinterpret_cast<uint4*>(rz.x_out + (size_t)m * K + k0) = v;
+      } else if (in_scale) {
         const int k0 = ks * C1_BK + seg * 8;
         unsigned int u[4] = {v.x, v.y, v.z, v.w};
 #pragma unroll
@@ -81,9 +99,9 @@
     }
   };
   if (total > 0) {
-    uint4 xr[D][XL];
-#pragma unroll
-    for (int j = 0; j < D; ++j) load(j < total ? j : total - 1, xr[j]);
+    uint4 xr[D][XL], rr[RES ? D : 1][XL];
+#pragma unroll
+    for (int j = 0; j < D; ++j) load(j < total ? j : total - 1, xr[j], rr[RES ? j : 0]);
     f32x4 acc[4][4];
 #pragma unroll
     for (int a = 0; a < 4; ++a)
@@ -96,8 +114,8 @@
         const long long s = s0 + j;
         if (s >= total) break;
         const int ks = (int)(s % KS), buf = (int)(s & 1);
-        stage(buf, ks, xr[j]);
-        load(s + D < total ? s + D : total - 1, xr[j]);
+        stage(buf, s, ks, xr[j], rr[RES ? j : 0]);
+        load(s + D < total ? s + D : total - 1, xr[j], rr[RES ? j : 0]);
         __syncthreads();
         s16x8 xa[4], wb[4];
 #pragma unroll
@@ -250,7 +268,7 @@
   do {                                                                                                                           \
     static bool once = false;                                                                                                    \
     if (!once) { (void)hipFuncSetAttribute((const void*)conv1x1_stream_kernel<WNV, KSV>, hipFuncAttributeMaxDynamicSharedMemorySize, 96 * 1024); once = true; } \
-    hipLaunchKernelGGL((conv1x1_stream_kernel<WNV, KSV>), grid, dim3(256), lds, s, xs, ws, in_scale, in_shift, in_relu, ys, partial, (long long)M, N, C1Epilogue{nullptr, 0, nullptr, 0, 0}); \
+    hipLaunchKernelGGL((conv1x1_stream_kernel<WNV, KSV>), grid, dim3(256), lds, s, xs, ws, in_scale, in_shift, in_relu, ys, partial, (long long)M, N, C1Epilogue{nullptr, 0, nullptr, 0, 0}, C1Residual{nullptr, nullptr, nullptr, nullptr}); \
   } while (0)
   const int wn = c1_wn(N), ks = K / 32;
   if (wn == 4 && ks == 2) A3D_C1S(4, 2);
@@ -266,6 +284,42 @@
   return check_launch("a3d_conv1x1_bn_fwd");
 }
 
+static bool c1_res_streams(int K, int N) { return K == 256 && N == 64 && c1_streams(K, N); }
+static bool c1_res_deep(int K, int N) { return c1_deep(K, N) && conv1x1_deep_res_serves(K, N); }
+extern "C" int a3d_conv1x1_res_serves(int K, int N) { return (K > 0 && N > 0 && (c1_res_streams(K, N) || c1_res_deep(K, N))) ? 1 : 0; }
+
+extern "C" int a3d_conv1x1_bn_res_fwd(const void* x_raw, const float* scale, const float* shift, const void* residual, const float* res_scale,
+                                      const float* res_shift, int relu, const void* w, void* x_act_out, void* y, float* partial, size_t M,
+                                      int K, int N, void* stream) {
+  if (!x_raw || !scale || !shift || !residual || !w || !x_act_out || !y || M == 0 || K <= 0 || N <= 0 || !a3d_conv1x1_res_serves(K, N) ||
+      ((res_scale != nullptr) != (res_shift != nullptr)) ||
+      ((((uintptr_t)x_raw | (uintptr_t)residual | (uintptr_t)w | (uintptr_t)x_act_out | (uintptr_t)y) & 15) != 0)) {
+    set_error("a3d_conv1x1_bn_res_fwd: bad argument (M=%zu K=%d N=%d; served shapes: a3d_conv1x1_res_serves -- 256 -> 64 and 512 -> 128; "
+              "x_raw, scale, shift, residual, w, x_act_out and y are required, res_scale and res_shift come together, 16-byte aligned operands)",
+              M, K, N);
+    return A3D_ERR_ARG;
+  }
+  hipStream_t s = (hipStream_t)stream;
+  if (!c1_res_streams(K, N))
+    return conv1x1_deep_res_launch(x_raw, scale, shift, residual, res_scale, res_shift, relu, w, x_act_out, y, partial, M, K, N, s);
+  static bool once = false;
+  if (!once) {
+    (void)hipFuncSetAttribute((const void*)conv1x1_stream_kernel<1, 8, false, 1>, hipFuncAttributeMaxDynamicSharedMemorySize, 96 * 1024);
+    (void)hipFuncSetAttribute((const void*)conv1x1_stream_kernel<1, 8, false, 2>, hipFuncAttributeMaxDynamicSharedMemorySize, 96 * 1024);
+    once = true;
+  }
+  const dim3 grid(c1_slabs(M, K, N), 1);
+  const size_t lds = c1_stream_lds(K, N) + (size_t)2 * K * sizeof(float);
+  const C1Residual rz{(const unsigned short*)residual, res_scale, res_shift, (unsigned short*)x_act_out};
+  if (res_scale)
+    hipLaunchKernelGGL((conv1x1_stream_kernel<1, 8, false, 2>), grid, dim3(256), lds, s, (const unsigned short*)x_raw, (const unsigned short*)w,
+                       scale, shift, relu, (unsigned short*)y, partial, (long long)M, N, C1Epilogue{nullptr, 0, nullptr, 0, 0}, rz);
+  else
+    hipLaunchKernelGGL((conv1x1_stream_kernel<1, 8, false, 1>), grid, dim3(256), lds, s, (const unsigned short*)x_raw, (const unsigned short*)w,
+                       scale, shift, relu, (unsigned short*)y, partial, (long long)M, N, C1Epilogue{nullptr, 0, nullptr, 0, 0}, rz);
+  return check_launch("a3d_conv1x1_bn_res_fwd");
+}
+
 extern "C" int a3d_conv1x1_topdown_serves(int K, int N) { return (c1_streams(K, N) && N <= 128) ? 1 : 0; }
 
 extern "C" int a3d_conv1x1_topdown_fwd(const void* x, const void* w, const float* bias, int nbias, const void* top, void* y,
@@ -288,7 +342,8 @@
     static bool once = false;                                                                                                    \
     if (!once) { (void)hipFuncSetAttribute((const void*)conv1x1_stream_kernel<WNV, KSV, true>, hipFuncAttributeMaxDynamicSharedMemorySize, 96 * 1024); once = true; } \
     hipLaunchKernelGGL((conv1x1_stream_kernel<WNV, KSV, true>), grid, dim3(256), lds, s, (const unsigned short*)x, (const unsigned short*)w, \
-                       (const float*)nullptr, (const float*)nullptr, 0, (unsigned short*)y, (float*)nullptr, (long long)M, N, ep);  \
+                       (const float*)nullptr, (const float*)nullptr, 0, (unsigned short*)y, (float*)nullptr, (long long)M, N, ep, \
+                       C1Residual{nullptr, nullptr, nullptr, nullptr});                                                         \
   } while (0)
   const int wn = c1_wn(N), ks = K / 32;
   if (wn == 2 && ks == 2) A3D_C1E(2, 2);
diff --git a/act3d-chained-diffuser_amd/csrc/conv1x1_deep.hip b/act3d-chained-diffuser_amd/csrc/conv1x1_deep.hip
--- a/act3d-chained-diffuser_amd/csrc/conv1x1_deep.hip
+++ b/act3d-chained-diffuser_amd/csrc/conv1x1_deep.hip
@@ -12,6 +12,11 @@
   float a = __uint_as_float(u << 16) * scS[k] + scS[K + k];
   float b = __uint_as_float(u & 0xFFFF0000u) * scS[k + 1] + scS[K + k + 1];
   return pk_bf16(fmaxf(a, relu_lo), fmaxf(b, relu_lo));
+}
+
+__device__ __forceinline__ unsigned int cd_res2(unsigned int u, unsigned int r, const float* scS, int K, int k, bool res_bn, int relu) {
+  return bn_res_act2(u, r, scS[k], scS[k + 1], scS[K + k], scS[K + k + 1], true, res_bn, res_bn ? scS[2 * K + k] : 0.f,
+                     res_bn ? scS[2 * K + k + 1] : 0.f, res_bn ? scS[3 * K + k] : 0.f, res_bn ? scS[3 * K + k + 1] : 0.f, relu != 0);
 }
 
 __device__ __forceinline__ void cd_compute(const unsigned short* Xb, const unsigned short* Wb, const int (&xo)[2][4], const int (&wo)[2][4],
@@ -60,11 +65,11 @@
   }
 }
 
-template <bool XFORM>
+template <bool XFORM, int RES = 0>
 __global__ __launch_bounds__(256, 2) void conv1x1_deep_kernel(const unsigned short* __restrict__ x, const unsigned short* __restrict__ w,
                                                             const float* __restrict__ in_scale, const float* __restrict__ in_shift,
                                                             int in_relu, unsigned short* __restrict__ y, float* __restrict__ partial,
-                                                            long long M, int N, int K) {
+                                                            long long M, int N, int K, C1Residual rz) {
   extern __shared__ __attribute__((aligned(16))) unsigned short smem_cd[];
   unsigned short* Xs = smem_cd;
   unsigned short* Ws = Xs + 2 * CD_BM * CD_BK;
@@ -77,6 +82,9 @@
   const long long mtiles = (M + CD_BM - 1) / CD_BM;
   if (XFORM)
     for (int i = t; i < K; i += 256) { scS[i] = in_scale[i]; scS[K + i] = in_shift[i]; }
+  constexpr bool res_bn = RES == 2;
+  if (res_bn)
+    for (int i = t; i < K; i += 256) { scS[2 * K + i] = rz.rscale[i]; scS[3 * K + i] = rz.rshift[i]; }
   float ssum[4][4], ssq[4][4];
 #pragma unroll
   for (int a = 0; a < 4; ++a)
@@ -92,6 +100,7 @@
   {                                                                                                                   \
     const long long m_ = l_m0 + srow + 32 * i < M ? l_m0 + srow + 32 * i : M - 1;    \
     P##x##i = *reinterpret_cast<const uint4*>(x + (size_t)m_ * K + l_ks * CD_BK + sseg * 8);                          \
+    if (RES) P##r##i = *reinterpret_cast<const uint4*>(rz.res + (size_t)m_ * K + l_ks * CD_BK + sseg * 8);            \
     P##w##i = *reinterpret_cast<const uint4*>(w + (size_t)(n0 + srow + 32 * i) * K + l_ks * CD_BK + sseg * 8);        \
   }
 #define CD_LOAD(P)                                                                                                    \
@@ -102,7 +111,14 @@
 #define CD_STAGE1(P, i)                                                                                               \
   {                                                                                                                   \
     uint4 v = P##x##i;                                                                                                \
-    if (XFORM) {                                                                                                      \
+    if (RES) {                                                                                                        \
+      const int k0 = ks * CD_BK + sseg * 8;                                                                           \
+      const uint4 q = P##r##i;                                                                                        \
+      v = make_uint4(cd_res2(v.x, q.x, scS, K, k0 + 0, res_bn, in_relu), cd_res2(v.y, q.y, scS, K, k0 + 2, res_bn, in_relu), \
+                     cd_res2(v.z, q.z, scS, K, k0 + 4, res_bn, in_relu), cd_res2(v.w, q.w, scS, K, k0 + 6, res_bn, in_relu)); \
+      const long long m_ = c_m0 + srow + 32 * i;                                                                      \
+      if (blockIdx.y == 0 && m_ < M) *reinterpret_cast<uint4*>(rz.x_out + (size_t)m_ * K + k0) = v;  \
+    } else if (XFORM) {                                                                                               \
       const int k0 = ks * CD_BK + sseg * 8;                                                                           \
       unsigned int u0 = v.x, u1 = v.y, u2 = v.z, u3 = v.w;                                                            \
       u0 = cd_norm2(u0, scS, K, k0 + 0, relu_lo); u1 = cd_norm2(u1, scS, K, k0 + 2, relu_lo);                         \
@@ -123,6 +139,7 @@
     }
   if (total > 0) {
     uint4 ax0, ax1, ax2, ax3, aw0, aw1, aw2, aw3, bx0, bx1, bx2, bx3, bw0, bw1, bw2, bw3;
+    uint4 ar0, ar1, ar2, ar3, br0, br1, br2, br3;
     long long l_left = total;
     CD_LOAD(a);
     CD_LOAD(b);
@@ -205,9 +222,33 @@
   const dim3 grid(conv1x1_deep_slabs(M, K, N), N / CD_BN);
   if (in_scale)
     hipLaunchKernelGGL(conv1x1_deep_kernel<true>, grid, dim3(256), cd_lds(K, true), s, (const unsigned short*)x, (const unsigned short*)w,
-                       in_scale, in_shift, in_relu, (unsigned short*)y, partial, (long long)M, N, K);
+                       in_scale, in_shift, in_relu, (unsigned short*)y, partial, (long long)M, N, K, C1Residual{nullptr, nullptr, nullptr, nullptr});
   else
     hipLaunchKernelGGL(conv1x1_deep_kernel<false>, grid, dim3(256), cd_lds(K, false), s, (const unsigned short*)x, (const unsigned short*)w,
-                       in_scale, in_shift, in_relu, (unsigned short*)y, partial, (long long)M, N, K);
+                       in_scale, in_shift, in_relu, (unsigned short*)y, partial, (long long)M, N, K, C1Residual{nullptr, nullptr, nullptr, nullptr});
   return check_launch("a3d_conv1x1_bn_fwd(deep)");
 }
+
+bool a3d::conv1x1_deep_res_serves(int K, int N) { return conv1x1_deep_serves(K, N) && K == 512 && N == CD_BN; }
+
+int a3d::conv1x1_deep_res_launch(const void* x_raw, const float* scale, const float* shift, const void* residual, const float* res_scale,
+                                 const float* res_shift, int relu, const void* w, void* x_act_out, void* y, float* partial, size_t M, int K, int N,
+                                 hipStream_t s) {
+  if (!conv1x1_deep_res_serves(K, N)) { set_error("a3d_conv1x1_bn_res_fwd: the deep-layer kernel does not serve K=%d N=%d", K, N); return A3D_ERR_ARG; }
+  static bool once = false;
+  if (!once) {
+    (void)hipFuncSetAttribute((const void*)conv1x1_deep_kernel<true, 1>, hipFuncAttributeMaxDynamicSharedMemorySize, 80 * 1024);
+    (void)hipFuncSetAttribute((const void*)conv1x1_deep_kernel<true, 2>, hipFuncAttributeMaxDynamicSharedMemorySize, 80 * 1024);
+    once = true;
+  }
+  const dim3 grid(conv1x1_deep_slabs(M, K, N), N / CD_BN);
+  const C1Residual rz{(const unsigned short*)residual, res_scale, res_shift, (unsigned short*)x_act_out};
+  const size_t lds = cd_lds(K, true) + (size_t)2 * K * sizeof(float);
+  if (res_scale)
+    hipLaunchKernelGGL((conv1x1_deep_kernel<true, 2>), grid, dim3(256), lds, s, (const unsigned short*)x_raw, (const unsigned short*)w, scale, shift,
+                       relu, (unsigned short*)y, partial, (long long)M, N, K, rz);
+  else
+    hipLaunchKernelGGL((conv1x1_deep_kernel<true, 1>), grid, dim3(256), lds, s, (const unsigned short*)x_raw, (const unsigned short*)w, scale, shift,
+                       relu, (unsigned short*)y, partial, (long long)M, N, K, rz);
+  return check_launch("a3d_conv1x1_bn_res_fwd(deep)");
+}
diff --git a/act3d-chained-diffuser_amd/csrc/vision.hip b/act3d-chained-diffuser_amd/csrc/vision.hip
--- a/act3d-chained-diffuser_amd/csrc/vision.hip
+++ b/act3d-chained-diffuser_amd/csrc/vision.hip
@@ -159,19 +159,9 @@
     unsigned int ow[4];
 #pragma unroll
     for (int j = 0; j < 4; ++j) {
-      float a = __uint_as_float(vw[j] << 16) * scale[c + 2 * j] + shift[c + 2 * j];
-      float b = __uint_as_float(vw[j] & 0xFFFF0000u) * scale[c + 2 * j + 1] + shift[c + 2 * j + 1];
-      if (res) {
-        float ra = __uint_as_float(rw[j] << 16), rb = __uint_as_float(rw[j] & 0xFFFF0000u);
-        if (RBN) {
-          ra = ra * rscale[c + 2 * j] + rshift[c + 2 * j];
-          rb = rb * rscale[c + 2 * j + 1] + rshift[c + 2 * j + 1];
-        }
-        a += ra;
-        b += rb;
-      }
-      if (relu) { a = fmaxf(a, 0.f); b = fmaxf(b, 0.f); }
-      ow[j] = pack2(a, b);
+      const int k = c + 2 * j;
+      ow[j] = bn_res_act2(vw[j], rw[j], scale[k], scale[k + 1], shift[k], shift[k + 1], res != nullptr, RBN, RBN ? rscale[k] : 0.f,
+                          RBN ? rscale[k + 1] : 0.f, RBN ? rshift[k] : 0.f, RBN ? rshift[k + 1] : 0.f, relu != 0);
     }
     y[i] = make_uint4(ow[0], ow[1], ow[2], ow[3]);
   }
diff --git a/act3d-chained-diffuser_amd/engine.py b/act3d-chained-diffuser_amd/engine.py
--- a/act3d-chained-diffuser_amd/engine.py
+++ b/act3d-chained-diffuser_amd/engine.py
@@ -4,6 +4,7 @@
 import torch.distributed as dist
 
 from . import lib as L
+from . import nn as NN
 
 NO_DECAY = ["bias", "LayerNorm.weight", "LayerNorm.bias"]
 
@@ -377,7 +378,14 @@
 
 
 PREFETCH_HIPRIO = os.environ.get("A3D_PREFETCH_HIPRIO", "0")
-PREFETCH_BN_GRID = int(os.environ.get("A3D_PREFETCH_BN_GRID", "256"))
+PREFETCH_BN_GRID = int(os.environ["A3D_PREFETCH_BN_GRID"]) if "A3D_PREFETCH_BN_GRID" in os.environ else None
+
+
+def prefetch_bn_grid(device=None):
+    if PREFETCH_BN_GRID is not None:
+        return PREFETCH_BN_GRID
+    return int(torch.cuda.get_device_properties(torch.cuda.current_device() if device is None else device).multi_processor_count)
+PREFETCH_FUSED_BLOCK_OUT = os.environ.get("A3D_PREFETCH_FUSED_BLOCK_OUT", "0") not in ("0", "", "off")
 PREFETCH_CHECK = os.environ.get("A3D_PREFETCH_CHECK", "0") == "1"
 
 
@@ -424,12 +432,16 @@
                 return
             self._pf_stream.wait_stream(torch.cuda.current_stream())
             lib = L.load()
-            prev = lib.a3d_bn_grid_cap(PREFETCH_BN_GRID) if PREFETCH_BN_GRID > 0 else 0
+            bn_grid = prefetch_bn_grid(self.next_rgbs.device)
+            prev = lib.a3d_bn_grid_cap(bn_grid) if bn_grid > 0 else 0
+            fused_out = NN.FUSED_BLOCK_OUT
+            NN.FUSED_BLOCK_OUT = fused_out and PREFETCH_FUSED_BLOCK_OUT
             try:
                 with torch.cuda.stream(self._pf_stream), torch.no_grad():
                     prefetch(self.next_rgbs, out=self.maps[1 - p_])
             finally:
-                if PREFETCH_BN_GRID > 0:
+                NN.FUSED_BLOCK_OUT = fused_out
+                if bn_grid > 0:
                     lib.a3d_bn_grid_cap(prev)
 
         def join():
diff --git a/act3d-chained-diffuser_amd/lib.py b/act3d-chained-diffuser_amd/lib.py
--- a/act3d-chained-diffuser_amd/lib.py
+++ b/act3d-chained-diffuser_amd/lib.py
@@ -135,6 +135,8 @@
     "a3d_conv1x1_streams": (_i, [_i, _i]),
     "a3d_conv1x1_nslab": (_i, [_z, _i, _i]),
     "a3d_conv1x1_bn_fwd": (_i, [_p, _p, _p, _p, _i, _p, _p, _z, _i, _i, _p]),
+    "a3d_conv1x1_res_serves": (_i, [_i, _i]),
+    "a3d_conv1x1_bn_res_fwd": (_i, [_p, _p, _p, _p, _p, _p, _i, _p, _p, _p, _p, _z, _i, _i, _p]),
     "a3d_conv1x1_topdown_serves": (_i, [_i, _i]),
     "a3d_conv1x1_topdown_fwd": (_i, [_p, _p, _p, _i, _p, _p, _z, _i, _i, _i, _i, _p]),
     "a3d_conv3x3_serves": (_i, [_i, _i, _i, _i]),
diff --git a/act3d-chained-diffuser_amd/nn.py b/act3d-chained-diffuser_amd/nn.py
--- a/act3d-chained-diffuser_amd/nn.py
+++ b/act3d-chained-diffuser_amd/nn.py
@@ -470,6 +470,29 @@
              None if in_scale is None else in_scale[1].data_ptr(), 1 if in_relu else 0, y.data_ptr(),
              None if partial is None else partial.data_ptr(), M, K, Cout, O.L.stream())
     return y, partial
+
+
+def conv1x1_bn_res(x_raw, scale, residual, residual_scale, conv, relu=True, want_stats=True, out=None):
+    N, K, H, W = x_raw.shape
+    Cout = conv.weight.shape[0]
+    assert x_raw.dtype == torch.bfloat16 and x_raw.is_contiguous(memory_format=torch.channels_last)
+    assert residual.shape == x_raw.shape and residual.dtype == x_raw.dtype and residual.is_contiguous(memory_format=torch.channels_last)
+    assert conv.kernel_size == (1, 1) and conv.stride == (1, 1) and conv.bias is None and conv.weight.dtype == torch.bfloat16
+    if out is not None:
+        assert out.shape == x_raw.shape and out.dtype == x_raw.dtype and out.is_contiguous(memory_format=torch.channels_last)
+    M = N * H * W
+    w2 = conv.weight.reshape(Cout, K)
+    assert w2.is_contiguous()
+    x_act = out if out is not None else torch.empty_like(x_raw)
+    y = torch.empty((N, Cout, H, W), device=x_raw.device, dtype=torch.bfloat16, memory_format=torch.channels_last)
+    partial = None
+    if want_stats:
+        partial = torch.empty((O.L.load().a3d_conv1x1_nslab(M, K, Cout), 2, Cout), device=x_raw.device, dtype=torch.float32)
+    O.L.call("a3d_conv1x1_bn_res_fwd", x_raw.data_ptr(), scale[0].data_ptr(), scale[1].data_ptr(), residual.data_ptr(),
+             None if residual_scale is None else residual_scale[0].data_ptr(),
+             None if residual_scale is None else residual_scale[1].data_ptr(), 1 if relu else 0, w2.data_ptr(), x_act.data_ptr(),
+             y.data_ptr(), None if partial is None else partial.data_ptr(), M, K, Cout, O.L.stream())
+    return y, partial, x_act
 
 
 def conv3x3_serves(x, conv):
@@ -578,20 +601,31 @@
     x_pooled = None
     fuse = FUSED_CONV1X1
 
-    def fused_ok(m, t):
-        return bool(fuse and m.kernel_size == (1, 1) and m.stride == (1, 1) and
+    def fused_ok(m, t, folded=False):
+        return bool(fuse and m.kernel_size == (1, 1) and m.stride == (1, 1) and not (folded and t.shape[1] > 1024) and
                     O.L.load().a3d_conv1x1_streams(t.shape[1], m.weight.shape[0]))
+
+    def res_ok(m, t):
+        return bool(fuse and FUSED_BLOCK_OUT and m.kernel_size == (1, 1) and m.stride == (1, 1) and m.bias is None and
+                    m.weight.dtype == torch.bfloat16 and O.L.load().a3d_conv1x1_res_serves(t.shape[1], m.weight.shape[0]))
 
     def conv1(m, t, **kw):
         if fused_ok(m, t):
             return conv1x1_bn(t, m, **kw)
         return conv(m, t), None
 
+    pending = None
     for bi, blk in enumerate(blocks):
-        c1, p1 = conv1(blk.conv1, x, want_stats=blk.bn1.training)
+        if pending is not None:
+            c1, p1, x = conv1x1_bn_res(*pending[:4], blk.conv1, want_stats=blk.bn1.training, out=pending[4])
+            pending = None
+            if id(blocks[bi - 1]) in last_of_layer:
+                outs.append(x)
+        else:
+            c1, p1 = conv1(blk.conv1, x, want_stats=blk.bn1.training)
         c2, p2 = conv3(blk.conv2, c1, blk.bn1, p1, blk.bn2.training)
         no_pool = isinstance(blk.avgpool, nn.Identity) or (isinstance(blk.avgpool, nn.AvgPool2d) and blk.avgpool.kernel_size in (1, (1, 1)))
-        if no_pool and fused_ok(blk.conv3, c2):
+        if no_pool and fused_ok(blk.conv3, c2, folded=True):
             o3, p3 = conv1x1_bn(c2, blk.conv3, in_scale=bn_scale_shift(c2, blk.bn2, p2), in_relu=True, want_stats=blk.bn3.training)
         else:
             if _pool2_ok(blk.avgpool, c2):
@@ -621,11 +655,14 @@
         else:
             idn = bn_act(cd, blk.downsample[2], relu=False, partial=pd)
         o_x = o_("res%d" % (len(outs) + 1)) if id(blk) in last_of_layer else None
+        bns += [blk.bn1, blk.bn2, blk.bn3]
+        if nxt is not None and not want_pooled and res_ok(nxt.conv1, o3):
+            pending, x, x_pooled = (o3, bn_scale_shift(o3, blk.bn3, p3), idn, idn_scale, o_x), None, None
+            continue
         if want_pooled:
             x, x_pooled = bn_act(o3, blk.bn3, relu=True, residual=idn, pool=True, partial=p3, out=o_x)
         else:
             x, x_pooled = bn_act(o3, blk.bn3, relu=True, residual=idn, partial=p3, residual_scale=idn_scale, out=o_x), None
-        bns += [blk.bn1, blk.bn2, blk.bn3]
         if id(blk) in last_of_layer:
             outs.append(x)
     if bb.training:
@@ -635,6 +672,7 @@
 
 FUSED_BN = os.environ.get("A3D_FUSED_BN", "1") == "1"
 FOLD_DOWNSAMPLE_BN = os.environ.get("A3D_FOLD_DS_BN", "1") not in ("0", "", "off")
+FUSED_BLOCK_OUT = os.environ.get("A3D_FUSED_BLOCK_OUT", "1") not in ("0", "", "off")
 FUSED_CONV1X1 = os.environ.get("A3D_FUSED_CONV1X1", "1") not in ("0", "", "off")
 FUSED_CONV3X3 = os.environ.get("A3D_FUSED_CONV3X3", "1") not in ("0", "", "off")
 
diff --git a/include/act3d_hip.h b/include/act3d_hip.h
--- a/include/act3d_hip.h
+++ b/include/act3d_hip.h
@@ -270,6 +270,10 @@
 int a3d_conv1x1_nslab(size_t M, int K, int N);
 int a3d_conv1x1_bn_fwd(const void* x, const void* w, const float* in_scale, const float* in_shift, int in_relu, void* y,
                        float* partial, size_t M, int K, int N, void* stream);
+int a3d_conv1x1_res_serves(int K, int N);
+int a3d_conv1x1_bn_res_fwd(const void* x_raw, const float* scale, const float* shift, const void* residual, const float* res_scale,
+                           const float* res_shift, int relu, const void* w, void* x_act_out, void* y, float* partial, size_t M, int K,
+                           int N, void* stream);
 int a3d_conv1x1_topdown_serves(int K, int N);
 int a3d_conv1x1_topdown_fwd(const void* x, const void* w, const float* bias, int nbias, const void* top, void* y, size_t images,
                             int H, int W, int K, int N, void* stream);
```

Result: no change. 3492 samples/s (-0.1%).
